# Hitenze/Preconditioned_Additive_Gaussian_Processes_with_Fourier_Acceleration

Hardware: AMD Instinct MI355X
Metric: kernel matvecs/sec + PCG wall-time to 1e-6, n=1e6 d=32 additive, 1/2/4/8 GPU (higher is better)
Workload: dtype f64; 1 GPU; additive NFFT matvec, n=1000000, d=32, 32 x 1-D windows, Gaussian f=1 l=1 mu=0.01 (BASELINE configs[2]); n=1000000, d=32, nwindows=32, parallelism=single

## Files before the change

include/nfft4gp_amd.h:

```cpp
#ifndef NFFT4GP_AMD_H
#define NFFT4GP_AMD_H

#include <stddef.h>

#ifdef __cplusplus
extern "C" {
#endif

#ifndef NFFT4GP_DOUBLE
#define NFFT4GP_DOUBLE double
#endif

#ifndef NFFT4GP_KERNEL_MAX_PARAMS
#define NFFT4GP_KERNEL_MAX_PARAMS 5
#endif

typedef int (*func_kernel)(void *str, NFFT4GP_DOUBLE *data, int n, int ldim, int d, int *permr, int kr,
                           int *permc, int kc, NFFT4GP_DOUBLE **Kp, NFFT4GP_DOUBLE **dKp);
typedef int (*func_solve)(void *precond, int n, NFFT4GP_DOUBLE *x, NFFT4GP_DOUBLE *rhs);
typedef int (*func_symmatvec)(void *matrix, int n, NFFT4GP_DOUBLE alpha, NFFT4GP_DOUBLE *x,
                              NFFT4GP_DOUBLE beta, NFFT4GP_DOUBLE *y);
typedef void (*func_free)(void *str);
typedef int (*func_trace)(void *str, NFFT4GP_DOUBLE **tracesp);
typedef NFFT4GP_DOUBLE (*func_logdet)(void *str);
// ... 158 lines not shown
typedef struct NFFT4GP_PRECOND_NYS_STRUCT
{
   int _k_setup;
   int _own_perm;
   int *_perm;
   int _n;
   int _tits;
   NFFT4GP_DOUBLE _titt;
   NFFT4GP_DOUBLE _tset;
   NFFT4GP_DOUBLE _tlogdet;
   NFFT4GP_DOUBLE _tdvp;
   int _nys_opt;
   int _k;
   NFFT4GP_DOUBLE _eta;
   NFFT4GP_DOUBLE _f2;
   NFFT4GP_DOUBLE *_U;
   NFFT4GP_DOUBLE *_s;
   NFFT4GP_DOUBLE *_work;
   NFFT4GP_DOUBLE *_K;
   NFFT4GP_DOUBLE *_dU;
   NFFT4GP_DOUBLE *_dK;
   pprecond_chol _chol_K11;
   int _dvp_nosolve;
} precond_nys, *pprecond_nys;
int Nfft4GPPrecondNysSolve(void *vnys_mat, int n, NFFT4GP_DOUBLE *x, NFFT4GP_DOUBLE *rhs);
int Nfft4GPAmdPrecondNysMirrorRelease(void *vnys_mat);

void *Nfft4GPAmdPrecondFsaiCreate(void);
void Nfft4GPAmdPrecondFsaiFree(void *str);
void Nfft4GPAmdPrecondFsaiReset(void *str);
void Nfft4GPAmdPrecondFsaiSetLfil(void *str, int lfil);
void Nfft4GPAmdPrecondFsaiSetKernel(void *str, int kernel);
int Nfft4GPAmdPrecondFsaiSetupWithKernel(NFFT4GP_DOUBLE *data, int n, int ldim, int d, func_kernel fkernel,
                                         void *fkernel_params, int require_grad, void *vfsai_mat);
int Nfft4GPAmdPrecondFsaiSetCsr(void *vfsai_mat, int n, const int *ia, const int *ja, const NFFT4GP_DOUBLE *aa,
                                const NFFT4GP_DOUBLE *da);
int Nfft4GPAmdPrecondFsaiCsr(void *vfsai_mat, int *ia, int *ja, NFFT4GP_DOUBLE *aa, NFFT4GP_DOUBLE *da);
int Nfft4GPAmdPrecondFsaiSolve(void *vfsai_mat, int n, NFFT4GP_DOUBLE *x, NFFT4GP_DOUBLE *rhs);
int Nfft4GPAmdPrecondFsaiInvL(void *vfsai_mat, int n, NFFT4GP_DOUBLE *x, NFFT4GP_DOUBLE *rhs);
int Nfft4GPAmdPrecondFsaiInvLT(void *vfsai_mat, int n, NFFT4GP_DOUBLE *x, NFFT4GP_DOUBLE *rhs);
int Nfft4GPAmdPrecondFsaiDvp(void *vfsai_mat, int n, int *mask, NFFT4GP_DOUBLE *x, NFFT4GP_DOUBLE **yp);
int Nfft4GPAmdPrecondFsaiTrace(void *vfsai_mat, NFFT4GP_DOUBLE **tracesp);
NFFT4GP_DOUBLE Nfft4GPAmdPrecondFsaiLogdet(void *vfsai_mat);

void *Nfft4GPAmdFsaiCreate(int n, const int *L_i, const int *L_j, const NFFT4GP_DOUBLE *L_a);
int Nfft4GPAmdFsaiSolve(void *fsai, int n, NFFT4GP_DOUBLE *x, NFFT4GP_DOUBLE *rhs);
void Nfft4GPAmdFsaiFree(void *fsai);

void *Nfft4GPAmdAfnCreate(int n, int k, const int *perm, const NFFT4GP_DOUBLE *L11, const NFFT4GP_DOUBLE *K12,
                          void *fsai_schur);
int Nfft4GPAmdAfnSolve(void *afn, int n, NFFT4GP_DOUBLE *x, NFFT4GP_DOUBLE *rhs);
void Nfft4GPAmdAfnFree(void *afn);
void *Nfft4GPAmdAfnSetup(const NFFT4GP_DOUBLE *data, int n, int ldim, int d, int k, int perm_opt, const int *perm,
                         int schur_lfil, int kernel, void *fkernel_params);
void *Nfft4GPAmdAfnSetupSchur(const NFFT4GP_DOUBLE *data, int n, int ldim, int d, int k, int perm_opt,
                              const int *perm, int schur_opt, int schur_lfil, int kernel, void *fkernel_params);
int Nfft4GPAmdAfnSetOperator(void *afn, void *op);
int Nfft4GPAmdAfnInfo(void *afn, int *k, int *perm, int *ia, int *ja, NFFT4GP_DOUBLE *aa);

int Nfft4GPAmdRankestNysScaled(const NFFT4GP_DOUBLE *data, int n, int ldim, int d, int kernel, void *fkernel_params,
                               int max_rank, int nsample, int nsample_r);
int Nfft4GPAmdRankestDefault(const NFFT4GP_DOUBLE *data, int n, int ldim, int d, int kernel, void *fkernel_params,
                             int max_rank, int nsample, int nsample_r, NFFT4GP_DOUBLE full_tol, int *perm);
int Nfft4GPAmdAfnRankEstimate(const NFFT4GP_DOUBLE *data, int n, int ldim, int d, int max_k, int perm_opt,
                              int nsamples, int kernel, void *fkernel_params, int *perm);
void *Nfft4GPAmdPrecondAFNSetup(const NFFT4GP_DOUBLE *data, int n, int ldim, int d, int max_k, int perm_opt,
                                int schur_opt, int schur_lfil, int nsamples, int kernel, void *fkernel_params,
                                int require_grad);
int Nfft4GPAmdPrecondAFNSolve(void *pre, int n, NFFT4GP_DOUBLE *x, NFFT4GP_DOUBLE *rhs);
int Nfft4GPAmdPrecondAFNInfo(void *pre, int *kind, int *k, void **afn, void **nys);
void Nfft4GPAmdPrecondAFNFree(void *pre);
void *Nfft4GPAmdPrecondAFNCreate(int max_k, int perm_opt, int schur_opt, int schur_lfil, int nsamples);
int Nfft4GPAmdPrecondAFNSetupWithKernel(NFFT4GP_DOUBLE *data, int n, int ldim, int d, func_kernel fkernel,
                                        void *fkernel_params, int require_grad, void *pre);
int Nfft4GPAmdPrecondAFNDvp(void *pre, int n, int *mask, NFFT4GP_DOUBLE *x, NFFT4GP_DOUBLE **yp);
int Nfft4GPAmdPrecondAFNTrace(void *pre, NFFT4GP_DOUBLE **tracesp);
NFFT4GP_DOUBLE Nfft4GPAmdPrecondAFNLogdet(void *pre);
void Nfft4GPAmdPrecondAFNReset(void *pre);

int Nfft4GPAmdSortFps(const NFFT4GP_DOUBLE *data, int n, int ldim, int d, int *k, NFFT4GP_DOUBLE tol, int *perm,
                      NFFT4GP_DOUBLE *dist);

void Nfft4GPAmdSetStream(void *hip_stream);
void *Nfft4GPAmdGetStream(void);
int Nfft4GPAmdDeviceAvailable(void);
const char *Nfft4GPAmdVersion(void);

int Nfft4GPAmdAdditiveLayoutInfo(void *str, long long *out, int nout);

int Nfft4GPAmdTimingEnable(void *str, int enable);
int Nfft4GPAmdSetDeterministic(void *str, int on);
int Nfft4GPAmdSetPrecision(void *str, int bits);
int Nfft4GPAmdTimingQuery(void *str, double *ms, long long *cnt);
int Nfft4GPAmdKernelBench(void *str, int which, int grad, int reps, const NFFT4GP_DOUBLE *x, NFFT4GP_DOUBLE *y,
                          double *ms_avg);

void *Nfft4GPAmdAdditiveShardCreate(NFFT4GP_DOUBLE *data, int n_global, int ldim, int d, int *windows,
                                    int nwindows, int dwindows, int row_begin, int row_end);
int Nfft4GPAmdShardSpread(void *str, const NFFT4GP_DOUBLE *x_local, NFFT4GP_DOUBLE *grid);
int Nfft4GPAmdShardFinish(void *str, const NFFT4GP_DOUBLE *grid, int grad, NFFT4GP_DOUBLE alpha,
                          const NFFT4GP_DOUBLE *x_local, NFFT4GP_DOUBLE beta, NFFT4GP_DOUBLE *y_local);
long long Nfft4GPAmdShardGridSize(void *str);

typedef int (*Nfft4GPAmdAllreduceFn)(void *ctx, NFFT4GP_DOUBLE *d_buf, long long count);
int Nfft4GPAmdCommRcclAvailable(void);
int Nfft4GPAmdCommUniqueId(void *id128);
void *Nfft4GPAmdCommCreateRccl(int rank, int world, const void *id128);
void *Nfft4GPAmdCommCreateCallback(int rank, int world, Nfft4GPAmdAllreduceFn fn, void *ctx,
                                   NFFT4GP_DOUBLE *d_stage, long long capacity);
int Nfft4GPAmdCommAllreduce(void *comm, NFFT4GP_DOUBLE *d_buf, long long count);
void Nfft4GPAmdCommFree(void *comm);
int Nfft4GPAmdCommRanks(void *comm);

int Nfft4GPAmdAdditiveComponentShard(void *str, int nw_global, int own_diag);
void *Nfft4GPAmdDistCreate(void *handle, int kind, void *comm);
void Nfft4GPAmdDistFree(void *dop);
int Nfft4GPAmdDistMatSymv(void *dop, int n, NFFT4GP_DOUBLE alpha, NFFT4GP_DOUBLE *x, NFFT4GP_DOUBLE beta,
                          NFFT4GP_DOUBLE *y);
int Nfft4GPAmdDistCheck(void *dop);
int Nfft4GPAmdDistSetChunks(void *dop, int chunks);
int Nfft4GPAmdDistPeerEnable(void *dop);
int Nfft4GPAmdDistPeerDisable(void *dop);
int Nfft4GPAmdDistPeerActive(void *dop);
int Nfft4GPAmdDistTimingEnable(void *dop, int enable);
int Nfft4GPAmdDistTimingQuery(void *dop, double *ms, long long *cnt);
int Nfft4GPAmdDistGradMatSymv(void *dop, int n, NFFT4GP_DOUBLE alpha, NFFT4GP_DOUBLE *x, NFFT4GP_DOUBLE beta,
                              NFFT4GP_DOUBLE *y);
int Nfft4GPAmdDistGaussianKernel(void *dop, NFFT4GP_DOUBLE *data, int n, int ldim, int d, int *permr, int kr,
                                 int *permc, int kc, NFFT4GP_DOUBLE **Kp, NFFT4GP_DOUBLE **dKp);
int Nfft4GPAmdDistMatern12Kernel(void *dop, NFFT4GP_DOUBLE *data, int n, int ldim, int d, int *permr, int kr,
                                 int *permc, int kc, NFFT4GP_DOUBLE **Kp, NFFT4GP_DOUBLE **dKp);
void *Nfft4GPAmdNysShard(void *nys, int row_begin, int row_end, void *comm);
void *Nfft4GPAmdNysShardSetupAdditive(void *dop, const int *perm, int k, int k11_mode);
int Nfft4GPAmdDistNysSolve(void *dnys, int n, NFFT4GP_DOUBLE *x, NFFT4GP_DOUBLE *rhs);
void Nfft4GPAmdDistNysFree(void *dnys);
int Nfft4GPAmdAfnSetStorage(void *afn, int bits);
int Nfft4GPAmdPrecondAFNSetStorage(void *pre, int bits);
void *Nfft4GPAmdAfnShard(void *afn, int row_begin, int row_end, void *comm);
void *Nfft4GPAmdAfnShardSetup(const NFFT4GP_DOUBLE *data, int n, int ldim, int d, int k, int perm_opt,
                              const int *perm, int schur_opt, int schur_lfil, int kernel, void *fkernel_params,
                              int row_begin, int row_end, void *comm);
int Nfft4GPAmdAfnShardInfo(void *dafn, int *m1, int *m2, long long *k12_doubles, long long *g_nnz);
int Nfft4GPAmdDistAfnSolve(void *dafn, int n, NFFT4GP_DOUBLE *x, NFFT4GP_DOUBLE *rhs);
void Nfft4GPAmdDistAfnFree(void *dafn);

typedef int (*func_matvec)(void *matrix, char trans, int m, int n, NFFT4GP_DOUBLE alpha, NFFT4GP_DOUBLE *x,
                           NFFT4GP_DOUBLE beta, NFFT4GP_DOUBLE *y);
typedef enum
{
   NFFT4GP_OPTIMIZER_UNDEFINED = 0,
   NFFT4GP_OPTIMIZER_ADAM,
   NFFT4GP_OPTIMIZER_NLTGCR
} nfft4gp_optimizer_type;
typedef int (*func_loss)(void *problem, NFFT4GP_DOUBLE *x, NFFT4GP_DOUBLE *lossp, NFFT4GP_DOUBLE *dloss);
typedef int (*func_optimization_step)(void *optimizer);

typedef struct NFFT4GP_OPTIMIZER_ADAM_STRUCT
{
   int _maxits;
   NFFT4GP_DOUBLE _tol;
   func_loss _floss;
   void *_fdata;
   int _n;
   NFFT4GP_DOUBLE _beta1;
   NFFT4GP_DOUBLE _beta2;
   NFFT4GP_DOUBLE _epsilon;
   NFFT4GP_DOUBLE _alpha;
   NFFT4GP_DOUBLE *_m;
   NFFT4GP_DOUBLE *_v;
   NFFT4GP_DOUBLE *_m_hat;
   NFFT4GP_DOUBLE *_v_hat;
   int _nits;
   NFFT4GP_DOUBLE *_loss_history;
   NFFT4GP_DOUBLE *_x_history;
   NFFT4GP_DOUBLE *_grad_history;
   NFFT4GP_DOUBLE *_grad_norm_history;
} optimizer_adam, *poptimizer_adam;

void *Nfft4GPOptimizationAdamCreate(void);
void Nfft4GPOptimizationAdamFree(void *optimizer);
int Nfft4GPOptimizationAdamSetProblem(void *optimizer, func_loss floss, void *fdata, int n);
int Nfft4GPOptimizationAdamSetOptions(void *optimizer, int maxits, NFFT4GP_DOUBLE tol, NFFT4GP_DOUBLE beta1,
                                      NFFT4GP_DOUBLE beta2, NFFT4GP_DOUBLE epsilon, NFFT4GP_DOUBLE alpha);
int Nfft4GPOptimizationAdamInit(void *optimizer, NFFT4GP_DOUBLE *x);
int Nfft4GPOptimizationAdamStep(void *optimizer);

typedef struct NFFT4GP_GP_OPTIMIZER_STRUCT
{
   nfft4gp_optimizer_type _type;
   func_optimization_step _fstep;
   void *_optimizer;
   NFFT4GP_DOUBLE *_dwork;
   NFFT4GP_DOUBLE *_data_train;
   int _data_train_n;
   int _data_train_ldim;
   int _data_train_d;
   NFFT4GP_DOUBLE *_label_train;
   func_kernel _fkernel;
   void *_vfkernel_data;
   func_free _kernel_data_free;
   func_symmatvec _matvec;
   func_symmatvec _dmatvec;
   func_kernel _precond_fkernel;
   void *_precond_vfkernel_data;
   func_free _precond_kernel_data_free;
   precond_kernel_setup _precond_setup;
   func_solve _precond_solve;
   func_trace _precond_trace;
   func_logdet _precond_logdet;
   func_dvp _precond_dvp;
   func_free _precond_reset;
   void *_precond_data;
   int _atol_loss;
   NFFT4GP_DOUBLE _tol_loss;
   int _wsize_loss;
   int _maxits_loss;
   int _nvecs_loss;
   NFFT4GP_DOUBLE *_radamacher_loss;
   nfft4gp_transform_type _transform;
   int *_mask;
   int _print_level_loss;
   NFFT4GP_DOUBLE *_data_predict;
   int _data_predict_n;
   int _data_predict_ldim;
   int _data_predict_d;
   NFFT4GP_DOUBLE *_label_predict;
   func_matvec _matvec_predict;
   int _atol_predict;
   NFFT4GP_DOUBLE _tol_predict;
   int _wsize_predict;
   int _maxits_predict;
   int _print_level_predict;
   int _retuire_std;
} nfft4gp_gp_problem, *pnfft4gp_gp_problem;

void *Nfft4GPGPProblemCreate(void);
void Nfft4GPGPProblemFree(void *gp_problem);
int Nfft4GPGpProblemSetup(void *gp_problem, nfft4gp_optimizer_type type, func_optimization_step fstep, void *optimizer,
                          NFFT4GP_DOUBLE *data_train, int data_train_n, int data_train_ldim, int data_train_d,
                          NFFT4GP_DOUBLE *label_train, func_kernel fkernel, void *vfkernel_data,
                          func_free kernel_data_free, func_symmatvec matvec, func_symmatvec dmatvec,
                          func_kernel precond_fkernel, void *precond_vfkernel_data,
                          func_free precond_kernel_data_free, precond_kernel_setup precond_setup,
                          func_solve precond_solve, func_trace precond_trace, func_logdet precond_logdet,
                          func_dvp precond_dvp, func_free precond_reset, void *precond_data, int atol_loss,
                          NFFT4GP_DOUBLE tol_loss, int wsize_loss, int maxits_loss, int nvecs_loss,
                          NFFT4GP_DOUBLE *radamacher_loss, nfft4gp_transform_type transform, int *mask,
                          int print_level_loss, NFFT4GP_DOUBLE *data_predict, int data_predict_n,
                          int data_predict_ldim, int data_predict_d, NFFT4GP_DOUBLE *label_predict,
                          func_matvec matvec_predict, int atol_predict, NFFT4GP_DOUBLE tol_predict, int wsize_predict,
                          int maxits_predict, int print_level_predict, int retuire_std);
int Nfft4GPGpProblemLoss(void *problem, NFFT4GP_DOUBLE *x, NFFT4GP_DOUBLE *lossp, NFFT4GP_DOUBLE *dloss);

void *Nfft4GPAmdModelCreate(void *additive_handle, const NFFT4GP_DOUBLE *alpha, int n);
int Nfft4GPAmdModelPredict(void *model, const NFFT4GP_DOUBLE *Xnew, int n_new, int ldim, int d, NFFT4GP_DOUBLE *mean,
                           long long *n_outside);
int Nfft4GPAmdModelInfo(void *model, int *nw, int *d, int *kernel, NFFT4GP_DOUBLE *hyper3);
int Nfft4GPAmdModelCoefficients(void *model, NFFT4GP_DOUBLE *H, NFFT4GP_DOUBLE *centre, NFFT4GP_DOUBLE *scale,
                                int *feature);
void *Nfft4GPAmdModelFromCoefficients(int nw, int d, int kernel, const NFFT4GP_DOUBLE *hyper3,
                                      const NFFT4GP_DOUBLE *H, const NFFT4GP_DOUBLE *centre,
                                      const NFFT4GP_DOUBLE *scale, const int *feature);
int Nfft4GPAmdModelFitVariance(void *model, const NFFT4GP_DOUBLE *X, int n, int ldim, int d);
int Nfft4GPAmdModelPredictStd(void *model, const NFFT4GP_DOUBLE *Xnew, int n_new, int ldim, int d,
                              NFFT4GP_DOUBLE *std, int with_noise, long long *n_outside);
int Nfft4GPAmdModelFitTimes(void *model, NFFT4GP_DOUBLE *ms3);
int Nfft4GPAmdModelVarianceInfo(void *model, int *R);
int Nfft4GPAmdModelVariance(void *model, NFFT4GP_DOUBLE *S);
int Nfft4GPAmdModelSetVariance(void *model, const NFFT4GP_DOUBLE *S, int R);
int Nfft4GPAmdModelFeatureWeights(int kernel, NFFT4GP_DOUBLE l, NFFT4GP_DOUBLE scale, int nw, NFFT4GP_DOUBLE *w33);
int Nfft4GPAmdModelFeatureWeightsGrad(int kernel, NFFT4GP_DOUBLE l, NFFT4GP_DOUBLE scale, int nw,
                                      NFFT4GP_DOUBLE *dw33);
void Nfft4GPAmdModelFree(void *model);

void *Nfft4GPAmdFeatureGpCreate(void *additive_handle, const NFFT4GP_DOUBLE *X, int n, int ldim, int d,
                                const NFFT4GP_DOUBLE *y);
int Nfft4GPAmdFeatureGpSetOptions(void *fgp, nfft4gp_transform_type transform, const int *mask);
int Nfft4GPAmdFeatureGpLoss(void *fgp, NFFT4GP_DOUBLE *x, NFFT4GP_DOUBLE *lossp, NFFT4GP_DOUBLE *dloss);
int Nfft4GPAmdFeatureGpSolve(void *fgp, const NFFT4GP_DOUBLE *X, int n, int ldim, int d, const NFFT4GP_DOUBLE *y,
                             NFFT4GP_DOUBLE f, NFFT4GP_DOUBLE l, NFFT4GP_DOUBLE mu, NFFT4GP_DOUBLE *alpha);
int Nfft4GPAmdFeatureGpSolveRhs(void *fgp, const NFFT4GP_DOUBLE *X, int n, int ldim, int d, const NFFT4GP_DOUBLE *r,
                                NFFT4GP_DOUBLE f, NFFT4GP_DOUBLE l, NFFT4GP_DOUBLE mu, NFFT4GP_DOUBLE *alpha);
int Nfft4GPAmdFeatureGpVariance(void *fgp, NFFT4GP_DOUBLE f, NFFT4GP_DOUBLE l, NFFT4GP_DOUBLE mu, NFFT4GP_DOUBLE *S);
int Nfft4GPAmdFeatureGpPredict(void *fgp, NFFT4GP_DOUBLE f, NFFT4GP_DOUBLE l, NFFT4GP_DOUBLE mu,
                               const NFFT4GP_DOUBLE *Xnew, int n_new, int ldim, int d, NFFT4GP_DOUBLE *mean,
                               long long *n_outside);
int Nfft4GPAmdFeatureGpMoments(void *fgp, NFFT4GP_DOUBLE *G, NFFT4GP_DOUBLE *b, NFFT4GP_DOUBLE *yy);
int Nfft4GPAmdFeatureGpInfo(void *fgp, int *n, int *nw, int *R, int *kernel);
int Nfft4GPAmdFeatureGpStatus(void *fgp, int *det_sign, NFFT4GP_DOUBLE *logabsdet);
void Nfft4GPAmdFeatureGpFree(void *fgp);

int Nfft4GPAmdHostTapPoly(NFFT4GP_DOUBLE *C);
int Nfft4GPAmdHostCirculant(int kind, NFFT4GP_DOUBLE c, NFFT4GP_DOUBLE weight, NFFT4GP_DOUBLE *bhat,
                            NFFT4GP_DOUBLE *w);
NFFT4GP_DOUBLE Nfft4GPAmdHostPrepare(const NFFT4GP_DOUBLE *col, int n, unsigned int *q);
int Nfft4GPAmdHostLayout(const unsigned int *qc, int n, int nw, int B, int CG, long long *counts,
                         unsigned short *meta, unsigned int *lo, unsigned int *q, int *tile_off);
int Nfft4GPAmdHostLayoutRec(const unsigned int *qc, int n, int nw, int B, int CG, int rec, long long *counts,
                            unsigned short *meta, unsigned int *lo, unsigned int *q, int *tile_off);
int Nfft4GPAmdDeviceLayout(const unsigned int *qc, int n, int nw, int B, int CG, long long *counts,
                           unsigned short *meta, unsigned int *lo, unsigned int *q, int *tile_off);
int Nfft4GPAmdDeviceLayoutRec(const unsigned int *qc, int n, int nw, int B, int CG, int rec, long long *counts,
                              unsigned short *meta, unsigned int *lo, unsigned int *q, int *tile_off);
int Nfft4GPAmdHostSymEig(const NFFT4GP_DOUBLE *A, int n, NFFT4GP_DOUBLE *w, NFFT4GP_DOUBLE *V);
int Nfft4GPAmdHostCholInverse(const NFFT4GP_DOUBLE *A, int k, NFFT4GP_DOUBLE shift, NFFT4GP_DOUBLE *G);
int Nfft4GPAmdHostLuSolve(const NFFT4GP_DOUBLE *A, int n, NFFT4GP_DOUBLE *B, int nrhs);
int Nfft4GPAmdHostLuLogdet(const NFFT4GP_DOUBLE *A, int n, NFFT4GP_DOUBLE *logabsdet, int *sign);

#ifdef __cplusplus
}
#endif

#endif
```

preconditioned_additive_gaussian_processes_with_fourier_acceleration_amd/csrc/internal.h:

```cpp
#pragma once

#include <hip/hip_runtime.h>

#include <cstdint>
#include <memory>
#include <utility>
#include <string>
#include <vector>

#include "../../include/nfft4gp_amd.h"

namespace nfft4gp_amd {

constexpr int kNos = 64;
constexpr int kBand = 32;
constexpr int kM = 4;
constexpr int kTaps = 2 * kM + 2;
constexpr int kDeg = 7;
constexpr int kNC = kDeg + 1;
constexpr int kR = 16;
constexpr int kWave = 64;
constexpr int kPad = 32;
constexpr int kMaxBlock = 4096 - kPad;

#define NFFT4GP_HIP_CHECK(expr)                                                                    \
   do {                                                                                            \
      hipError_t _e = (expr);                                                                      \
      if (_e != hipSuccess) {                                                                      \
         fprintf(stderr, "nfft4gp_amd: HIP error %s at %s:%d (%s)\n", hipGetErrorString(_e),      \
                 __FILE__, __LINE__, #expr);                                                       \
         return -1;                                                                                \
      }                                                                                            \
   } while (0)

double kb_phi(double t);
double kb_phi_hut(int k);
const std::vector<double>& tap_poly_coeffs();
void bhat_1d(int kind, double c, double* bhat);
void circulant_1d(const double* bhat, double weight, double* w);

__host__ __device__ inline size_t quad_index(long long t, int w, int lane, int nwords)
{
   return (((size_t)t * (size_t)(nwords / 4) + (size_t)(w >> 2)) * kWave + (size_t)lane) * 4 + (size_t)(w & 3);
}

template <class T>
struct DefaultInitAlloc : std::allocator<T> {
   template <class U>
   struct rebind {
      using other = DefaultInitAlloc<U>;
   };
   DefaultInitAlloc() = default;
   template <class U>
   DefaultInitAlloc(const DefaultInitAlloc<U>&) noexcept {}
   template <class U>
   void construct(U* p) noexcept
   {
      ::new ((void*)p) U;
   }
   template <class U, class... A>
   void construct(U* p, A&&... a)
   {
      ::new ((void*)p) U(std::forward<A>(a)...);
   }
};
template <class T>
using RawVec = std::vector<T, DefaultInitAlloc<T>>;

__host__ __device__ inline uint32_t slot_word(uint32_t loc, uint32_t frac)
{
   const uint32_t lo4 = loc & 15u, e = (frac & 0x3FFFFFFu) << 6;
   return ((lo4 >= 8u && e != 0u) ? e - 16u + lo4 : e + lo4) ^ 0x80000000u;
}
__host__ __device__ inline uint32_t lo_byte(uint32_t loc) { return (loc >> 4) & 255u; }
__host__ __device__ inline uint32_t slot_word4(uint32_t loc, uint32_t frac)
{
   const uint32_t e = (frac & 0x3FFFFFFu) << 6, L = loc & 4095u;
   const uint32_t v = (e & ~4095u) | L;
   const int32_t dv = (int32_t)(v - e);
   const uint32_t down = (dv > 2048 && v >= 4096u) ? 4096u : 0u;
   const uint32_t up = (dv < -2048 && v <= 0xFFFFEFFFu) ? 4096u : 0u;
   return (v - down + up) ^ 0x80000000u;
}

struct Layout {
   int n = 0;
   int nw = 0;
   int B = kMaxBlock;
   int CG = 8;
   int rec = 5;
   int ngroups = 0;
   int nblocks = 0;
   long long ntiles = 0;
   RawVec<uint16_t> meta;
   RawVec<uint32_t> lo;
   RawVec<uint32_t> q;
   std::vector<int> tile_off;
   std::vector<int> cmax;
};
void build_layout(const uint32_t* qc, int n, int nw, int B, int CG, Layout& L, int rec = 5);
struct AdditivePlan;
int build_layout_dev(const uint32_t* d_qc, int n, int nw, int B, int CG, AdditivePlan& P, hipStream_t s, int rec = 5);

struct DevLayout {
   uint16_t* meta = nullptr;
   uint32_t* lo = nullptr;
   uint32_t* q = nullptr;
   int* tile_off = nullptr;
   int* cmax = nullptr;
   long long ntiles = 0;
   size_t bytes = 0;
};

constexpr int kMdMaxDim = 5;
constexpr int kMdTiledMaxDim = 3;
struct MdComp {
   int d = 0;
   int hicount = 1;
   long long u_off = 0;
};
struct MdPlan {
   bool on = false;
   bool gfix_per_window = false;
   int maxd = 1;
   long long G = 0;
   long long Cmax = 0;
   long long M = 0;
   std::vector<MdComp> comps;
   MdComp* d_comps = nullptr;
   int* d_u = nullptr;
   double* d_psi = nullptr;
   double* d_grid = nullptr;
   double2* d_F[2] = {nullptr, nullptr};
   double2* d_Mo[2] = {nullptr, nullptr};
   double2* d_B[4] = {nullptr, nullptr, nullptr, nullptr};
   double* d_h[2] = {nullptr, nullptr};
   double* d_bh = nullptr;
   double* d_bhd = nullptr;
   double* d_dot_part = nullptr;
   unsigned int* d_dot_ticket = nullptr;
   int* d_perm = nullptr;
   int4* d_items = nullptr;
   int nitems = 0;
   bool lines = false;
   double* d_part = nullptr;
   unsigned long long* d_gfix = nullptr;
   unsigned long long* d_xmax = nullptr;
   double psi_max = 0.0;
};

struct AdditivePlan {
   int n_global = 0, row_begin = 0, row_end = 0, n = 0;
   int nw = 0, dw = 0, skip_last = 0;
   std::vector<int> comp_dims;
   int d = 0;
   std::vector<int> comp_feature;
   bool points_ready = false;
   std::vector<double> comp_scale;
   std::vector<double> comp_centre;
   std::vector<double> comp_sigma;
   int kernel = 0;
   double f = 1.0, l = 1.0, mu = 0.0;
   double weight = 1.0;
   double diag = 1.0;
   int B = kMaxBlock, CG = 3, ngroups = 0, nblocks = 0;
   int rec = 5;
   int spread_variant = -1;
   int spread_fold = 1;
   bool det = false;
   double* d_hb = nullptr;
   int nparts = 0;
   DevLayout dl;
   double* d_part = nullptr;
   double* d_w = nullptr;
   double* d_wd = nullptr;
   double* d_H = nullptr;
   double* d_Hd = nullptr;
   double* d_C = nullptr;
   double* d_dot_part = nullptr;
   unsigned int* d_dot_ticket = nullptr;
   double* d_part2 = nullptr;
   double* d_gsum = nullptr;
   int fused_grid = -1;
   bool cells33 = false;
   double* d_hsum = nullptr;
   int hsum_par = 0;
   double* d_H2 = nullptr;
   double* d_xs = nullptr;
   double* d_ys = nullptr;
   MdPlan md;
   bool timing = false;
   hipEvent_t* kev = nullptr;
   double ms[3] = {0, 0, 0};
   long long cnt[3] = {0, 0, 0};
};

int upload_tap_coeffs();
int launch_spread(const AdditivePlan& P, const double* d_x, double* d_part, hipStream_t stream);
int launch_grid(const AdditivePlan& P, const double* d_part, int nparts, int grad, hipStream_t stream);
int launch_spread_grid(AdditivePlan& P, const double* d_x, int grad, hipStream_t stream);
int launch_grid_from_sum(const AdditivePlan& P, const double* d_gridsum, int grad, hipStream_t stream);
constexpr int kPeerInline = 8;
struct PeerArgs {
   char* const* bufs = nullptr;
   char* inl[kPeerInline] = {};
   char* own = nullptr;
   int world = 0;
   unsigned int epoch = 0;
   unsigned int* err = nullptr;
   long long slot_doubles = 0;
   long long spin = 0;
};
int launch_reduce_parts(const AdditivePlan& P, const double* d_part, double* d_gridsum, hipStream_t stream,
                        const PeerArgs* A = nullptr);
int launch_shard_finish_split(const AdditivePlan& P, const double* d_gridsum, double alpha, const double* d_x,
                              double beta, double* d_y, int S, hipStream_t stream, const PeerArgs* A = nullptr,
                              const double* d_part = nullptr);
int launch_peer_grid(const AdditivePlan& P, const PeerArgs& A, const double* d_part, hipStream_t stream);
int launch_peer_sum(const AdditivePlan& P, const PeerArgs& A, double* d_grid, hipStream_t stream);
int launch_interp(const AdditivePlan& P, int grad, double alpha, const double* d_x, double beta, double* d_y,
                  hipStream_t stream, double* d_dot = nullptr);
int launch_interp_blocks(const AdditivePlan& P, double alpha, const double* d_x, double beta, double* d_y, int b0,
                         int b1, hipStream_t stream);
int launch_matvec2(AdditivePlan& P, double alpha, const double* x0, const double* x1, double beta, double* y0,
                   double* y1, hipStream_t stream);
int pick_spread_variant(const AdditivePlan& P);
bool grid_atomic(const AdditivePlan& P);
int pick_interp_threads(const AdditivePlan& P);
bool pick_interp_hl(const AdditivePlan& P);
int pick_hl_slots(const AdditivePlan& P);
int pick_interp2_threads();
bool pick_fused_grid(const AdditivePlan& P);
int launch_matvec_fused(AdditivePlan& P, double alpha, const double* d_x, double beta, double* d_y, hipStream_t stream,
                        double* d_dot = nullptr);
int additive_matvec_multi(void* str, int nv, double alpha, const double* const* X, double beta, double* const* Y);
int additive_matvec_dot(void* str, const double* d_x, double* d_y, double* d_dot);
AdditivePlan* additive_plan_of(void* str);
bool additive_fused_dot_ok(void* str);

struct NysDev {
   int n = 0, k = 0;
   double eta = 0.0;
   double* U = nullptr;
   float* Uf = nullptr;
   double* s = nullptr;
   double* w = nullptr;
   double* part = nullptr;
   int nblk = 0;
   double setup_ms[4] = {0.0, 0.0, 0.0, 0.0};
   std::vector<double> hs;
   bool grad = false;
   double f2 = 0.0;
   double *Kall = nullptr, *dU = nullptr, *G = nullptr, *Gt = nullptr, *GdKG = nullptr, *D = nullptr;
   double *vk = nullptr, *vn = nullptr;
};
void nys_free(NysDev* N);
constexpr int kNysRows = 2048;
int nys_alloc_scratch(NysDev* N);
int gemm_f64(bool transA, int M, int N, int K, const double* A, long long lda, const double* B, long long ldb,
             double* C, long long ldc, hipStream_t s);
int sym_eig_host(const std::vector<double>& A, int n, std::vector<double>& w, std::vector<double>& V);
int chol_inverse_host(std::vector<double>& A, int k);
int lu_solve_host(std::vector<double>& A, int n, std::vector<double>& B, int nrhs, double* logabsdet = nullptr,
                  int* sign = nullptr, std::vector<int>* piv_out = nullptr);
void lu_subst_host(const std::vector<double>& A, int n, const std::vector<int>& piv, std::vector<double>& B, int nrhs);
int lu_solve_dev(double* A, int n, double* B, int nrhs, hipStream_t s, double* logabsdet = nullptr,
                 int* sign = nullptr, int* piv_keep = nullptr);
int lu_resolve_dev(const double* A, int n, const int* piv, double* B, int nrhs, hipStream_t s);
struct Comm;
struct NysShard {
   Comm* comm = nullptr;
   int row_begin = 0, n_global = 0;
};
NysDev* nys_setup_additive(const double* xw_host, int n, int nw, int dw, int skip_last, int kernel, double f,
                           double l, double mu, const int* perm, int k, int k11_mode, bool with_grad = false,
                           const NysShard* shard = nullptr);

int md_build_points(AdditivePlan& P, const std::vector<std::vector<double>>& xs);
int md_setup(AdditivePlan& P);
int md_spread(const AdditivePlan& P, const double* d_x, double* d_grid, hipStream_t s);
int md_grid(const AdditivePlan& P, const double* d_grid, int grad, hipStream_t s);
int md_interp(const AdditivePlan& P, int grad, double alpha, const double* d_x, double beta, double* d_y,
              hipStream_t s, double* d_dot = nullptr);
void md_free(AdditivePlan& P);
void bhat_nd(int kind, int d, double c, std::vector<double>& bhat);

int chol_inverse_dev(double* A, int k, double shift, double* G, double* Gt, int* d_info, hipStream_t s);
int gram_tn(int M, int N, int K, const double* A, long long lda, const double* B, long long ldb, double* C, int sym,
            hipStream_t s);
int sym_eigvals_dev(double* A, int n, std::vector<double>& w, hipStream_t s);
struct KernelSpec {
   int kernel = 0;
   double f = 1.0, l = 1.0, mu = 0.0;
   const double* Xk = nullptr;
   long long ldk = 0;
   int nw = 1, dw = 0, last_dw = 0;
};
int fsai_kernel_csr(const double* dX, int n, int ldim, int d, int lfil, const KernelSpec& K, const double* dW, int kw,
                    int require_grad, std::vector<int>& ia, std::vector<int>& ja, std::vector<double>& aa,
                    std::vector<double>& da, hipStream_t s, const double* dGB = nullptr,
                    const double* dGC = nullptr, void** keep = nullptr);
void* fsai_create_from_device(int n, int* dia, int* dja, double* daa, const std::vector<int>& hia, hipStream_t s);
long long count_nonfinite(const double* d, size_t count, hipStream_t s);
int fsai_pattern_rows(const double* dX, int n, int ldim, int d, int lfil, const std::vector<int>& rows,
                      std::vector<int>& hia, std::vector<int>& hja, hipStream_t s);
int fsai_values_rows(const KernelSpec& Ks, const double* dX, long long ldim, int d, int lfil, const int* dia,
                     const int* dja, int nrows, const double* dW, int kw, const int* dwcol, double* daa, hipStream_t s);
void* afn_shard_from_parts(int n_local, int k, int n2, Comm* comm, const std::vector<int>& lm_idx,
                           const std::vector<int>& lm_row, const std::vector<int>& nl_pos,
                           const std::vector<int>& nl_row, double* d_Linv, double* d_LinvT, double* d_K12, bool fsai,
                           double schur_scale, const std::vector<int>& gia, const std::vector<int>& gja,
                           const std::vector<double>& gaa);
void* fsai_grad_create(int n, const int* ia, const int* ja, const double* aa, const double* da);
void fsai_grad_free(void* F);
int fsai_grad_op(void* F, int op, int g, const double* x, double* y, hipStream_t s);
double fsai_grad_diag(void* F, int g, hipStream_t s);
int chol_factor_dev(double* A, int k, int* d_info, hipStream_t s);
int kernel_spec_of(void* fkernel_params, func_kernel fkernel, int kernel, int n, KernelSpec& K, double** owned);
struct AfnGrad {
   int n = 0, k = 0, n2 = 0;
   int* perm = nullptr;
   double *L = nullptr, *Linv = nullptr, *LinvT = nullptr;
   double* dL = nullptr;
   const double* K12 = nullptr;
   double* dK12 = nullptr;
   void* S = nullptr;
   void* afn = nullptr;
   double trace[3] = {0.0, 0.0, 0.0};
   double logdet = 0.0;
   double* work = nullptr;
};
void afn_grad_free(AfnGrad* G);
int afn_grad_dvp(AfnGrad* G, const int* mask, const double* x, double* y, hipStream_t s);

void* afn_create_device(int n, int k, int* d_perm, double* d_Linv, double* d_LinvT, double* d_K12, void* S,
                        double schur_scale = 0.0);

hipStream_t current_stream();
bool is_device_ptr(const void* p);
int device_ok();

constexpr int kMvFeat = 33, kMvPad = 36, kMvMaxNw = 128;
constexpr double kMpLimit = 0.25 + 1.0 / 8589934592.0;
inline int mv_order(int nw) { return kMvPad * ((nw + 3) / 4 * 4); }

__device__ inline bool mv_angle(double x, double ctr, double sc, double& c1, double& s1)
{
   const double xs = (x - ctr) * sc;
   const bool in = fabs(xs) <= kMpLimit;
   const double xq = in ? xs : 0.0;
   const uint32_t q = (uint32_t)(unsigned long long)llround(xq * 4294967296.0);
   sincospi((double)(int)q * (1.0 / 2147483648.0), &s1, &c1);
   return in;
}

__device__ inline void mv_rotate(double& ck, double& sk, double c1, double s1)
{
   const double c = ck * c1 - sk * s1;
   sk = sk * c1 + ck * s1;
   ck = c;
}

struct WindowMap {
   int nw = 0, d = 0;
   const double* centre = nullptr;
   const double* scale = nullptr;
   const int* feature = nullptr;
};
void feature_weights(int kernel, double l, double scale, int nw, double* w33);
void feature_weights_grad(int kernel, double l, double scale, int nw, double* dw33);
int window_count_outside(const WindowMap& W, const double* dX, long long ld, int n, hipStream_t s, long long* outside);
int window_moments(const WindowMap& W, const double* dX, long long ld, int n, const double* dy, double* G, double* b,
                   double* yy, double* ms2, hipStream_t s);

struct RandScope {
   RandScope();
   ~RandScope();
};
struct CallerRandBatch {
   char* prev = nullptr;
   CallerRandBatch();
   ~CallerRandBatch();
};

struct Comm {
   int rank = 0, world = 1;
   virtual ~Comm() {}
   virtual int allreduce(double* d_buf, size_t count, hipStream_t s) = 0;
   virtual int ranks() { return world; }
};
int additive_rows(void* str, int* n_local, int* n_global, int* row_begin);
int dist_failed(void* dop);
bool shard_fused_dot_ok(void* str);
int shard_finish_dot(void* str, const double* grid, const double* x_local, double* y_local, double* d_dot);
bool shard_peer_ok(void* str);
int shard_spread_peer(void* str, const double* x_local, const PeerArgs& A);
int shard_peer_sum(void* str, const PeerArgs& A, double* d_grid);
int shard_finish_dot_peer(void* str, const PeerArgs& A, double* d_grid, const double* x_local, double* y_local,
                          double* d_dot);
int shard_finish_peer(void* str, const PeerArgs& A, double* d_grid, int grad, double alpha, const double* x_local,
                      double beta, double* y_local);
struct DistPcgInfo {
   Comm* dot_comm = nullptr;
   int n_global = 0;
   int row_begin = 0;
   bool fused_dot = false;
};
int dist_pcg_info(void* dop, DistPcgInfo& info);
NysDev* nys_setup_shard(void* str, const int* perm, int k, int k11_mode, Comm* comm);
int additive_matvec_chunked(void* str, double alpha, const double* d_x, double* d_y, int nchunks,
                            int (*done)(void* ctx, size_t r0, size_t r1), void* ctx);
int dist_matvec_dot(void* dop, const double* d_p, double* d_q, double* d_dot);

}
```

preconditioned_additive_gaussian_processes_with_fourier_acceleration_amd/csrc/layout_gpu.hip:

```cpp
#include <hip/hip_runtime.h>

#include <algorithm>
#include <cstdio>
#include <vector>

#include "callbacks.hpp"
#include "internal.h"

namespace nfft4gp_amd {

namespace {

constexpr int kLT = 256;
constexpr int kLWaves = kLT / 64;

__global__ __launch_bounds__(kLT) void k_lay_count(const uint32_t* __restrict__ qc, int n, int nw, int B, int CG,
                                                   int ngroups, int* __restrict__ tiles, int* __restrict__ cmax)
{
   __shared__ int hist[kNos];
   __shared__ int nch, mx;
   const int bg = blockIdx.x, b = bg / ngroups, g = bg % ngroups;
   const int base = b * B, nloc = min(B, n - base);
   const int c0 = g * CG, c1 = min(nw, c0 + CG);
   const int tid = threadIdx.x;
   if (tid == 0) nch = mx = 0;
   for (int c = c0; c < c1; c++) {
      const uint32_t* qq = qc + (size_t)c * n + base;
      if (tid < kNos) hist[tid] = 0;
      __syncthreads();
      for (int j = tid; j < nloc; j += kLT) atomicAdd(&hist[qq[j] >> 26], 1);
      __syncthreads();
      if (tid < 64) {
         int v = (hist[tid] + kR - 1) / kR, m = hist[tid];
         for (int off = 32; off > 0; off >>= 1) {
            v += __shfl_xor(v, off, 64);
            m = max(m, __shfl_xor(m, off, 64));
         }
         if (tid == 0) {
            nch += v;
            mx = max(mx, m);
         }
      }
      __syncthreads();
   }
   if (tid == 0) {
      tiles[bg] = (nch + kWave - 1) / kWave;
      cmax[bg] = mx;
   }
}

struct EmitLds {
   size_t off, run, cbase, sorted, sloc, sfr, smeta, cnt, total;
   __host__ __device__ EmitLds(int CG, int B, int Tmax)
   {
      size_t p = 0;
      auto take = [&](size_t bytes) {
         const size_t at = p;
         p += (bytes + 15) & ~(size_t)15;
         return at;
      };
      off = take(sizeof(int) * CG * (kNos + 1));
      run = take(sizeof(int) * CG * kNos);
      cbase = take(sizeof(int) * (CG * kNos + 1));
      const size_t sorted_bytes = sizeof(uint16_t) * CG * B, cnt_bytes = sizeof(int) * Tmax * (2 * 32 + 4 * 16);
      sorted = take(sorted_bytes > cnt_bytes ? sorted_bytes : cnt_bytes);
      cnt = sorted;
      sloc = take(sizeof(uint16_t) * Tmax * kWave * kR);
      sfr = take(sizeof(uint32_t) * Tmax * kWave * kR);
      smeta = take(sizeof(uint16_t) * Tmax * kWave);
      total = p;
   }
};

template <int REC>
__global__ __launch_bounds__(kLT) void k_lay_emit(const uint32_t* __restrict__ qc, int n, int nw, int B, int CG,
                                                  int ngroups, int Tmax, const int* __restrict__ tile_off,
                                                  uint16_t* __restrict__ meta, uint32_t* __restrict__ lo,
                                                  uint32_t* __restrict__ q)
{
   extern __shared__ __attribute__((aligned(16))) unsigned char lds[];
   const EmitLds E(CG, B, Tmax);
   int* s_off = reinterpret_cast<int*>(lds + E.off);
   int* s_run = reinterpret_cast<int*>(lds + E.run);
   int* s_cbase = reinterpret_cast<int*>(lds + E.cbase);
   uint16_t* s_sorted = reinterpret_cast<uint16_t*>(lds + E.sorted);
   uint16_t* s_loc = reinterpret_cast<uint16_t*>(lds + E.sloc);
   uint32_t* s_fr = reinterpret_cast<uint32_t*>(lds + E.sfr);
   uint16_t* s_meta = reinterpret_cast<uint16_t*>(lds + E.smeta);
   int* s_cnt = reinterpret_cast<int*>(lds + E.cnt);

   const int bg = blockIdx.x, b = bg / ngroups, g = bg % ngroups;
   const int base = b * B, nloc = min(B, n - base);
   const int c0 = g * CG, c1 = min(nw, c0 + CG), ncomp = c1 - c0;
   const int t0 = tile_off[bg], T = tile_off[bg + 1] - t0;
   const int tid = threadIdx.x, lane = tid & 63, wave = tid >> 6;

   for (int ci0 = 0; ci0 < ncomp; ci0 += kLWaves) {
      const int ci = ci0 + wave;
      const bool act = ci < ncomp;
      const uint32_t* qq = qc + (size_t)(c0 + (act ? ci : 0)) * n + base;
      int* off = s_off + (act ? ci : 0) * (kNos + 1);
      int* run = s_run + (act ? ci : 0) * kNos;
      uint16_t* sorted = s_sorted + (size_t)(act ? ci : 0) * B;
      if (act) run[lane] = 0;
      __syncthreads();
      if (act)
         for (int j = lane; j < nloc; j += 64) atomicAdd(&run[qq[j] >> 26], 1);
      __syncthreads();
      if (act) {
         const int v = run[lane];
         int incl = v;
         for (int d = 1; d < 64; d <<= 1) {
            const int t = __shfl_up(incl, d, 64);
            if (lane >= d) incl += t;
         }
         off[lane] = incl - v;
         if (lane == 63) off[kNos] = incl;
         run[lane] = incl - v;
      }
      __syncthreads();
      for (int jb = 0; jb < nloc; jb += 64) {
         const int j = jb + lane;
         const bool valid = act && j < nloc;
         const int cell = valid ? (int)(qq[j] >> 26) : 0;
         unsigned long long peers = __ballot(valid);
#pragma unroll
         for (int bit = 0; bit < 6; bit++) {
            const unsigned long long set = __ballot(valid && ((cell >> bit) & 1));
            peers &= ((cell >> bit) & 1) ? set : ~set;
         }
         const int rank = __popcll(peers & ((1ull << lane) - 1ull));
         const int start = valid ? run[cell] : 0;
         __syncthreads();
         if (valid) {
            sorted[start + rank] = (uint16_t)j;
            if (lane == 63 - __clzll(peers)) run[cell] = start + __popcll(peers);
         }
         __syncthreads();
      }
   }
   if (tid == 0) {
      int acc = 0;
      for (int i = 0; i < ncomp * kNos; i++) {
         s_cbase[i] = acc;
         const int* off = s_off + (i / kNos) * (kNos + 1);
         const int cnt = off[i % kNos + 1] - off[i % kNos];
         acc += (cnt + kR - 1) / kR;
      }
      s_cbase[ncomp * kNos] = acc;
   }
   for (int i = tid; i < T * kWave * kR; i += kLT) {
      s_loc[i] = (uint16_t)(B + ((i / kR) % kWave & 31));
      s_fr[i] = 0u;
   }
   for (int i = tid; i < T * kWave; i += kLT) s_meta[i] = (uint16_t)(c0 << 6);
   __syncthreads();
   const int nchunks = s_cbase[ncomp * kNos];
   for (int k = tid; k < nchunks; k += kLT) {
      int lo_i = 0, hi_i = ncomp * kNos;
      while (hi_i - lo_i > 1) {
         const int mid = (lo_i + hi_i) >> 1;
         if (s_cbase[mid] <= k) lo_i = mid;
         else hi_i = mid;
      }
      const int ci = lo_i / kNos, cell = lo_i % kNos;
      const int* off = s_off + ci * (kNos + 1);
      const int s = off[cell] + (k - s_cbase[lo_i]) * kR;
      const int tile = k % T, ln = k / T;
      s_meta[tile * kWave + ln] = (uint16_t)(((c0 + ci) << 6) | cell);
      const uint32_t* qq = qc + (size_t)(c0 + ci) * n + base;
      const uint16_t* sorted = s_sorted + (size_t)ci * B;
      for (int r = 0; r < kR; r++) {
         const int sidx = s + r;
         if (sidx < off[cell + 1]) {
            const int loc = sorted[sidx];
            s_loc[(tile * kWave + ln) * kR + r] = (uint16_t)loc;
            s_fr[(tile * kWave + ln) * kR + r] = qq[loc] & 0x3FFFFFFu;
         }
      }
   }
   __syncthreads();
   if (tid < T) {
      uint16_t* L = s_loc + (size_t)tid * kWave * kR;
      uint32_t* F = s_fr + (size_t)tid * kWave * kR;
      int* c32 = s_cnt + tid * 128;
      int* c16 = c32 + 64;
      for (int r = 0; r < kR; r++) {
         for (int i = 0; i < 128; i++) c32[i] = 0;
         for (int ln = 0; ln < kWave; ln++) {
            int best = r, best_cost = 1 << 30;
            for (int k = r; k < kR; k++) {
               const int v = L[ln * kR + k];
               const int cost = 2 * c32[(ln >> 5) * 32 + (v & 31)] + c16[(ln >> 4) * 16 + (v & 15)];
               if (cost < best_cost) {
                  best_cost = cost;
                  best = k;
                  if (cost == 0) break;
               }
            }
            const uint16_t tl = L[ln * kR + r];
            L[ln * kR + r] = L[ln * kR + best];
            L[ln * kR + best] = tl;
            const uint32_t tf = F[ln * kR + r];
            F[ln * kR + r] = F[ln * kR + best];
            F[ln * kR + best] = tf;
            const int v = L[ln * kR + r];
            c32[(ln >> 5) * 32 + (v & 31)]++;
            c16[(ln >> 4) * 16 + (v & 15)]++;
         }
      }
   }
   __syncthreads();
   for (int i = tid; i < T * kWave; i += kLT) meta[(size_t)(t0 + i / kWave) * kWave + i % kWave] = s_meta[i];
   for (int i = tid; i < T * kWave * kR; i += kLT) {
      const int tile = i / (kWave * kR), ln = (i / kR) % kWave, r = i % kR;
      const uint32_t loc = s_loc[i];
      q[quad_index(t0 + tile, r, ln, kR)] = REC == 5 ? slot_word(loc, s_fr[i]) : slot_word4(loc, s_fr[i]);
   }
   if (REC != 5) return;
   for (int i = tid; i < T * kWave * (kR / 4); i += kLT) {
      const int tile = i / (kWave * (kR / 4)), ln = (i / (kR / 4)) % kWave, r4 = i % (kR / 4);
      const uint16_t* l4 = s_loc + ((size_t)tile * kWave + ln) * kR + 4 * r4;
      lo[quad_index(t0 + tile, r4, ln, kR / 4)] =
          lo_byte(l4[0]) | (lo_byte(l4[1]) << 8) | (lo_byte(l4[2]) << 16) | (lo_byte(l4[3]) << 24);
   }
}

}

int build_layout_dev(const uint32_t* d_qc, int n, int nw, int B, int CG, AdditivePlan& P, hipStream_t s, int rec)
{
   const int ngroups = (nw + CG - 1) / CG, nblocks = (n + B - 1) / B, nbg = ngroups * nblocks;
   const int Tmax_bound = (CG * (B / kR + kNos) + kWave - 1) / kWave + 1;
   if (EmitLds(CG, B, (CG * ((B + kR - 1) / kR) + kWave - 1) / kWave).total > 160 * 1024) return -1;
   int* d_tiles = nullptr;
   int* d_cmax = nullptr;
   NFFT4GP_HIP_CHECK(hipMalloc((void**)&d_tiles, sizeof(int) * (nbg + 1)));
   NFFT4GP_HIP_CHECK(hipMalloc((void**)&d_cmax, sizeof(int) * std::max(1, nbg)));
   hipLaunchKernelGGL(k_lay_count, dim3(std::max(1, nbg)), dim3(kLT), 0, s, d_qc, n, nw, B, CG, ngroups, d_tiles,
                      d_cmax);
   NFFT4GP_HIP_CHECK(hipGetLastError());
   std::vector<int> tiles(nbg);
   NFFT4GP_HIP_CHECK(hipMemcpyAsync(tiles.data(), d_tiles, sizeof(int) * nbg, hipMemcpyDeviceToHost, s));
   NFFT4GP_HIP_CHECK(hipStreamSynchronize(s));
   std::vector<int> toff(nbg + 1, 0);
   long long acc = 0;
   int Tmax = 1;
   for (int i = 0; i < nbg; i++) {
      toff[i] = (int)acc;
      acc += tiles[i];
      Tmax = std::max(Tmax, tiles[i]);
   }
   toff[nbg] = (int)acc;
   if (Tmax > Tmax_bound || EmitLds(CG, B, Tmax).total > 160 * 1024) {
      (void)hipFree(d_tiles);
      (void)hipFree(d_cmax);
      return -1;
   }
   P.ngroups = ngroups;
   P.nblocks = nblocks;
   P.dl = DevLayout();
   P.dl.cmax = d_cmax;
   NFFT4GP_HIP_CHECK(hipMalloc((void**)&P.dl.tile_off, sizeof(int) * (nbg + 1)));
   NFFT4GP_HIP_CHECK(hipMemcpyAsync(P.dl.tile_off, toff.data(), sizeof(int) * (nbg + 1), hipMemcpyHostToDevice, s));
   const size_t nt = (size_t)std::max<long long>(acc, 1);
   NFFT4GP_HIP_CHECK(hipMalloc((void**)&P.dl.meta, sizeof(uint16_t) * nt * kWave));
   if (rec == 5) NFFT4GP_HIP_CHECK(hipMalloc((void**)&P.dl.lo, sizeof(uint32_t) * nt * (kR / 4) * kWave));
   NFFT4GP_HIP_CHECK(hipMalloc((void**)&P.dl.q, sizeof(uint32_t) * nt * kR * kWave));
   const size_t lds = EmitLds(CG, B, Tmax).total;
   static const bool attr = []() {
      (void)hipFuncSetAttribute((const void*)k_lay_emit<5>, hipFuncAttributeMaxDynamicSharedMemorySize, 160 * 1024);
      (void)hipFuncSetAttribute((const void*)k_lay_emit<4>, hipFuncAttributeMaxDynamicSharedMemorySize, 160 * 1024);
      (void)hipGetLastError();
      return true;
   }();
   (void)attr;
   if (nbg > 0)
      hipLaunchKernelGGL(rec == 5 ? k_lay_emit<5> : k_lay_emit<4>, dim3(nbg), dim3(kLT), lds, s, d_qc, n, nw, B, CG,
                         ngroups, Tmax, P.dl.tile_off, P.dl.meta, P.dl.lo, P.dl.q);
   NFFT4GP_HIP_CHECK(hipGetLastError());
   NFFT4GP_HIP_CHECK(hipStreamSynchronize(s));
   (void)hipFree(d_tiles);
   P.dl.ntiles = acc;
   P.dl.bytes = (size_t)acc * kWave * (2 + (rec == 5 ? 4 * (kR / 4) : 0) + 4 * kR) + sizeof(int) * (nbg + 1);
   return 0;
}

}

extern "C" int Nfft4GPAmdDeviceLayoutRec(const unsigned int* qc, int n, int nw, int B, int CG, int rec,
                                         long long* counts, unsigned short* meta, unsigned int* lo, unsigned int* q,
                                         int* tile_off);
extern "C" int Nfft4GPAmdDeviceLayout(const unsigned int* qc, int n, int nw, int B, int CG, long long* counts,
                                      unsigned short* meta, unsigned int* lo, unsigned int* q, int* tile_off)
{
   return Nfft4GPAmdDeviceLayoutRec(qc, n, nw, B, CG, 5, counts, meta, lo, q, tile_off);
}

extern "C" int Nfft4GPAmdDeviceLayoutRec(const unsigned int* qc, int n, int nw, int B, int CG, int rec,
                                         long long* counts, unsigned short* meta, unsigned int* lo, unsigned int* q,
                                         int* tile_off)
{
   using namespace nfft4gp_amd;
   if (B <= 0 || B > kMaxBlock || CG <= 0 || n < 0 || nw <= 0 || nw > 1023 || !counts || (rec != 4 && rec != 5))
      return -1;
   if (!need_device("Nfft4GPAmdDeviceLayout")) return -1;
   hipStream_t s = current_stream();
   uint32_t* d_qc = nullptr;
   NFFT4GP_HIP_CHECK(hipMalloc((void**)&d_qc, sizeof(uint32_t) * std::max<size_t>(1, (size_t)n * nw)));
   NFFT4GP_HIP_CHECK(hipMemcpy(d_qc, qc, sizeof(uint32_t) * (size_t)n * nw, hipMemcpyHostToDevice));
   AdditivePlan P;
   const int rc = build_layout_dev(d_qc, n, nw, B, CG, P, s, rec);
   (void)hipFree(d_qc);
   if (rc) return -1;
   const int nbg = P.ngroups * P.nblocks;
   counts[0] = P.dl.ntiles;
   counts[1] = P.ngroups;
   counts[2] = P.nblocks;
   const size_t nt = (size_t)P.dl.ntiles;
   int err = 0;
   if (meta && hipMemcpy(meta, P.dl.meta, sizeof(uint16_t) * nt * kWave, hipMemcpyDeviceToHost) != hipSuccess) err = 1;
   if (lo && rec == 5 &&
       hipMemcpy(lo, P.dl.lo, sizeof(uint32_t) * nt * (kR / 4) * kWave, hipMemcpyDeviceToHost) != hipSuccess)
      err = 1;
   if (q && hipMemcpy(q, P.dl.q, sizeof(uint32_t) * nt * kR * kWave, hipMemcpyDeviceToHost) != hipSuccess) err = 1;
   if (tile_off && hipMemcpy(tile_off, P.dl.tile_off, sizeof(int) * (nbg + 1), hipMemcpyDeviceToHost) != hipSuccess)
      err = 1;
   for (void* p : {(void*)P.dl.meta, (void*)P.dl.lo, (void*)P.dl.q, (void*)P.dl.tile_off, (void*)P.dl.cmax})
      (void)hipFree(p);
   return err ? -1 : 0;
}
```

preconditioned_additive_gaussian_processes_with_fourier_acceleration_amd/csrc/nfft_api.cpp:

```cpp
#include <dlfcn.h>
#include <hip/hip_runtime.h>

#include <array>
#include <algorithm>
#include <atomic>
#include <chrono>
#include <thread>
#include <cmath>
#include <cstdio>
#include <cstdlib>
#include <cstring>
#include <mutex>
#include <vector>

#include "internal.h"
#include "reduce.hpp"

using namespace nfft4gp_amd;

namespace nfft4gp_amd {

namespace {
std::recursive_mutex g_rand_mu;
int g_rand_depth = 0;
char* g_caller_rand = nullptr;
char g_private_rand[256];
bool g_private_ready = false;
}

RandScope::RandScope()
{
   g_rand_mu.lock();
   if (g_rand_depth++ == 0) {
      if (!g_private_ready) {
         g_caller_rand = initstate(20240807u, g_private_rand, sizeof(g_private_rand));
         g_private_ready = true;
      } else {
         g_caller_rand = setstate(g_private_rand);
      }
   }
}

RandScope::~RandScope()
{
   if (--g_rand_depth == 0) {
      setstate(g_caller_rand);
      g_caller_rand = nullptr;
   }
   g_rand_mu.unlock();
}

CallerRandBatch::CallerRandBatch()
{
   if (g_rand_depth > 0) prev = setstate(g_caller_rand);
}

CallerRandBatch::~CallerRandBatch()
{
   if (prev) g_caller_rand = setstate(prev);
}

static hipStream_t g_stream = nullptr;

hipStream_t current_stream() { return g_stream; }

int device_ok()
{
   static int ok = 0;
   if (!ok) {
      int cnt = 0;
      const hipError_t e = hipGetDeviceCount(&cnt);
      if (e != hipSuccess) {
         fprintf(stderr, "nfft4gp_amd: hipGetDeviceCount failed: %s\n", hipGetErrorString(e));
         cnt = 0;
      }
      (void)hipGetLastError();
      ok = cnt > 0 ? 1 : 0;
   }
   return ok;
}

bool is_device_ptr(const void* p)
{
   if (!p) return false;
   hipPointerAttribute_t attr;
   hipError_t e = hipPointerGetAttributes(&attr, p);
   if (e != hipSuccess) {
      (void)hipGetLastError();
      return false;
   }
   return attr.type == hipMemoryTypeDevice || attr.type == hipMemoryTypeManaged;
}

}

namespace {

struct TimingRec {
   std::array<hipEvent_t, 6> ev;
   bool grid = true;
};

struct PlanExt {
   AdditivePlan P;
   std::vector<TimingRec> pending;
   std::vector<TimingRec> pool;
};

struct SingleAdj {
   str_adj pub{};
   double sigma_pub = 0.0;
   nfft4gp_kernel* owner = nullptr;
   int dim = 1;
   int max_n = 0;
   std::vector<double> data;
   PlanExt* plan = nullptr;
};

void dfree(void* p)
{
   if (p) (void)hipFree(p);
}

void free_layout(AdditivePlan& P)
{
   dfree(P.dl.meta);
   dfree(P.dl.lo);
   dfree(P.dl.q);
   dfree(P.dl.tile_off);
   dfree(P.dl.cmax);
   P.dl = DevLayout();
   dfree(P.d_part);
   dfree(P.d_part2);
   dfree(P.d_H2);
   dfree(P.d_dot_part);
   dfree(P.d_dot_ticket);
   P.d_part2 = P.d_H2 = nullptr;
   P.d_part = nullptr;
   P.d_dot_part = nullptr;
   P.d_dot_ticket = nullptr;
}

void free_plan(PlanExt* E)
{
   if (!E) return;
   AdditivePlan& P = E->P;
   free_layout(P);
   md_free(P);
   dfree(P.d_w);
   dfree(P.d_wd);
   dfree(P.d_H);
   dfree(P.d_Hd);
   dfree(P.d_hb);
   dfree(P.d_gsum);
   dfree(P.d_hsum);
   dfree(P.d_C);
   dfree(P.d_xs);
   dfree(P.d_ys);
   for (auto& r : E->pending)
      for (auto e : r.ev) (void)hipEventDestroy(e);
   for (auto& r : E->pool)
      for (auto e : r.ev) (void)hipEventDestroy(e);
   delete E;
}

template <class T, class A>
int upload(T** dptr, const std::vector<T, A>& h)
{
   if (*dptr) {
      (void)hipFree(*dptr);
      *dptr = nullptr;
   }
   if (h.empty()) return 0;
   NFFT4GP_HIP_CHECK(hipMalloc((void**)dptr, sizeof(T) * h.size()));
   NFFT4GP_HIP_CHECK(hipMemcpy(*dptr, h.data(), sizeof(T) * h.size(), hipMemcpyHostToDevice));
   return 0;
}

double centre_and_scale(const double* col, int n_global, int d, std::vector<double>& xs, double* centre = nullptr)
{
   xs.assign(col, col + (size_t)n_global * d);
   for (int i = 0; i < d; i++) {
      double c = 0.0;
      for (int j = 0; j < n_global; j++) c += xs[(size_t)i * n_global + j];
      c /= (double)n_global;
      if (centre) centre[i] = c;
      for (int j = 0; j < n_global; j++) xs[(size_t)i * n_global + j] -= c;
   }
   double radius = 0.0;
   for (int j = 0; j < n_global; j++) {
      double r = 0.0;
      for (int i = 0; i < d; i++) r += xs[(size_t)i * n_global + j] * xs[(size_t)i * n_global + j];
      r = std::sqrt(r);
      if (r > radius) radius = r;
   }
   double scale;
   if (radius == 0.0) return -1.0;
   if (radius > 0.25 || radius < 0.125) {
      scale = 0.25 / radius;
      for (auto& v : xs) v *= scale;
   } else {
      scale = 1.0;
   }
   return scale;
}

uint32_t quantize(double x)
{
   const long long v = std::llround(x * 4294967296.0);
   return (uint32_t)(unsigned long long)v;
}

int plan_build_points(AdditivePlan& P, const double* buffer)
{
   const int ng = P.n_global;
   RawVec<uint32_t> qc((size_t)P.nw * P.n);
   P.comp_scale.assign(P.nw, 1.0);
   P.comp_centre.assign(P.nw, 0.0);
   std::vector<double> xs;
   if (std::any_of(P.comp_dims.begin(), P.comp_dims.end(), [](int d) { return d != 1; })) {
      std::vector<std::vector<double>> xsc(P.nw);
      for (int c = 0; c < P.nw; c++) {
         const double* col = buffer + (size_t)c * ng * P.dw;
         P.comp_scale[c] = centre_and_scale(col, ng, P.comp_dims[c], xsc[c]);
         if (P.comp_scale[c] < 0.0) {
            fprintf(stderr, "nfft4gp_amd: all points of window %d coincide (radius 0); the reference's scaling "
                            "0.25/radius (nfft_interface.c:190) is undefined there.\n", c);
            return -1;
         }
      }
      if (md_build_points(P, xsc)) return -1;
      P.points_ready = true;
      return 0;
   }
   const auto t0 = std::chrono::steady_clock::now();
   std::atomic<int> next{0};
   std::atomic<int> outside33{0};
   auto work = [&]() {
      std::vector<double> xw;
      for (int c = next++; c < P.nw; c = next++) {
         const double* col = buffer + (size_t)c * ng * P.dw;
         P.comp_scale[c] = centre_and_scale(col, ng, 1, xw, &P.comp_centre[c]);
         if (P.comp_scale[c] < 0.0) continue;
         uint32_t cimax = 0;
         for (int j = 0; j < P.n; j++) {
            const uint32_t q = quantize(xw[(size_t)P.row_begin + j]);
            qc[(size_t)c * P.n + j] = q;
            cimax = std::max(cimax, (q + 0x40000000u) >> 26);
         }
         if (cimax > 32u) outside33 = 1;
      }
   };
   {
      const int nt = std::max(1, std::min({16, P.nw, (int)std::thread::hardware_concurrency()}));
      std::vector<std::thread> th;
      for (int t = 1; t < nt; t++) th.emplace_back(work);
      work();
      for (auto& t : th) t.join();
   }
   for (int c = 0; c < P.nw; c++)
      if (P.comp_scale[c] < 0.0) {
         fprintf(stderr,
                 "nfft4gp_amd: all points of window %d coincide (radius 0); the reference's scaling "
                 "0.25/radius (nfft_interface.c:190) is undefined there.\n", c);
         return -1;
      }
   P.cells33 = outside33 == 0;
   const auto t1 = std::chrono::steady_clock::now();
   free_layout(P);
   hipStream_t s = current_stream();
   uint32_t* d_qc = nullptr;
   NFFT4GP_HIP_CHECK(hipMalloc((void**)&d_qc, sizeof(uint32_t) * std::max<size_t>(1, qc.size())));
   NFFT4GP_HIP_CHECK(hipMemcpyAsync(d_qc, qc.data(), sizeof(uint32_t) * qc.size(), hipMemcpyHostToDevice, s));
   const auto t2 = std::chrono::steady_clock::now();
   const int rc_dev = build_layout_dev(d_qc, P.n, P.nw, P.B, P.CG, P, s, P.rec);
   (void)hipStreamSynchronize(s);
   (void)hipFree(d_qc);
   if (rc_dev) {
      Layout L;
      build_layout(qc.data(), P.n, P.nw, P.B, P.CG, L, P.rec);
      P.ngroups = L.ngroups;
      P.nblocks = L.nblocks;
      free_layout(P);
      if (upload(&P.dl.meta, L.meta) || upload(&P.dl.lo, L.lo) || upload(&P.dl.q, L.q) ||
          upload(&P.dl.tile_off, L.tile_off) || upload(&P.dl.cmax, L.cmax))
         return -1;
      P.dl.ntiles = L.ntiles;
      P.dl.bytes = L.meta.size() * 2 + L.lo.size() * 4 + L.q.size() * 4 + L.tile_off.size() * 4;
   }
   if (getenv("NFFT4GP_AMD_VERBOSE")) {
      const auto t3 = std::chrono::steady_clock::now();
      auto ms = [](auto a, auto b) { return std::chrono::duration<double, std::milli>(b - a).count(); };
      fprintf(stderr, "nfft4gp_amd: layout setup: centre/scale/quantize %.1f ms, coordinate upload %.1f ms, "
                      "layout (%s) %.1f ms\n", ms(t0, t1), ms(t1, t2), rc_dev ? "host" : "GPU", ms(t2, t3));
   }
   P.nparts = P.nblocks;
   NFFT4GP_HIP_CHECK(hipMalloc((void**)&P.d_part, sizeof(double) * (size_t)std::max(1, P.nparts) * P.nw * kNos));

   dfree(P.d_dot_part);
   NFFT4GP_HIP_CHECK(hipMalloc((void**)&P.d_dot_part, sizeof(double) * (size_t)std::max(1, P.nblocks)));
   if (!P.d_dot_ticket) {
      NFFT4GP_HIP_CHECK(hipMalloc((void**)&P.d_dot_ticket, sizeof(unsigned int) * kTicketWords));
      NFFT4GP_HIP_CHECK(hipMemset(P.d_dot_ticket, 0, sizeof(unsigned int) * kTicketWords));
   }

   if (!P.d_H) NFFT4GP_HIP_CHECK(hipMalloc((void**)&P.d_H, sizeof(double) * (size_t)P.nw * kNos * kNC));
   if (!P.d_Hd) NFFT4GP_HIP_CHECK(hipMalloc((void**)&P.d_Hd, sizeof(double) * (size_t)P.nw * kNos * kNC));
   if (!P.d_hb) NFFT4GP_HIP_CHECK(hipMalloc((void**)&P.d_hb, sizeof(double) * 4 * (size_t)std::max(1, P.nw)));
   if (upload_tap_coeffs()) return -1;
   P.points_ready = true;
   return 0;
}

int plan_setup(AdditivePlan& P, const double* buffer, int kernel, double f, double l, double mu)
{
   if (!device_ok()) {
      fprintf(stderr, "nfft4gp_amd: no HIP device visible; the operator has no CPU fallback.\n");
      return -1;
   }
   if (!P.points_ready && plan_build_points(P, buffer)) return -1;
   P.kernel = kernel;
   P.f = f;
   P.l = l;
   P.mu = mu;
   P.comp_sigma.assign(P.nw, 0.0);
   if (P.md.on) {
      for (int c = 0; c < P.nw; c++)
         P.comp_sigma[c] = (kernel == 0) ? l * P.comp_scale[c] * std::sqrt(2.0) : l * P.comp_scale[c];
      return md_setup(P);
   }
   std::vector<double> w((size_t)P.nw * kNos), wd((size_t)P.nw * kNos);
   double bh[kBand], bhd[kBand];
   for (int c = 0; c < P.nw; c++) {
      const double sc = P.comp_scale[c];
      const double sig = (kernel == 0) ? l * sc * std::sqrt(2.0) : l * sc;
      P.comp_sigma[c] = sig;
      bhat_1d(kernel == 0 ? 0 : 2, sig, bh);
      bhat_1d(kernel == 0 ? 1 : 3, sig, bhd);
      const double dscale = (kernel == 0) ? 2.0 * sc * std::sqrt(2.0) / sig : sc / sig;
      circulant_1d(bh, P.weight, w.data() + (size_t)c * kNos);
      circulant_1d(bhd, P.weight * dscale, wd.data() + (size_t)c * kNos);
   }
   if (upload(&P.d_w, w) || upload(&P.d_wd, wd)) return -1;
   return 0;
}

TimingRec get_rec(PlanExt* E)
{
   if (!E->pool.empty()) {
      TimingRec r = E->pool.back();
      E->pool.pop_back();
      return r;
   }
   TimingRec r;
   for (auto& e : r.ev) (void)hipEventCreate(&e);
   return r;
}

bool use_fused(const AdditivePlan& P, hipStream_t s)
{
   if (!pick_fused_grid(P)) return false;
   hipStreamCaptureStatus st = hipStreamCaptureStatusNone;
   if (hipStreamIsCapturing(s, &st) != hipSuccess) {
      (void)hipGetLastError();
      return false;
   }
   return st == hipStreamCaptureStatusNone;
}

int plan_apply_dev(PlanExt* E, int grad, double alpha, const double* d_x, double beta, double* d_y)
{
   AdditivePlan& P = E->P;
   hipStream_t s = current_stream();
   TimingRec rec;
   if (P.timing) {
      rec = get_rec(E);
      if (!P.md.on) P.kev = rec.ev.data();
   }
   const bool mdt = P.timing && P.md.on;
   int rc = 0;
   if (mdt) (void)hipEventRecord(rec.ev[0], s);
   const bool fused = !grad && use_fused(P, s);
   rec.grid = !fused;
   if (P.md.on) {
      rc = md_spread(P, d_x, P.md.d_grid, s);
      if (mdt) {
         (void)hipEventRecord(rec.ev[1], s);
         (void)hipEventRecord(rec.ev[2], s);
      }
      if (!rc) rc = md_grid(P, P.md.d_grid, grad, s);
   } else if (fused) {
      rc = launch_matvec_fused(P, alpha, d_x, beta, d_y, s);
   } else {
      rc = launch_spread_grid(P, d_x, grad, s);
   }
   if (mdt) {
      (void)hipEventRecord(rec.ev[3], s);
      (void)hipEventRecord(rec.ev[4], s);
   }
   if (!rc && !fused)
      rc = P.md.on ? md_interp(P, grad, alpha, d_x, beta, d_y, s) : launch_interp(P, grad, alpha, d_x, beta, d_y, s);
   if (mdt) (void)hipEventRecord(rec.ev[5], s);
   P.kev = nullptr;
   if (P.timing) {
      if (rc)
         E->pool.push_back(rec);
      else
         E->pending.push_back(rec);
   }
   return rc ? -1 : 0;
}

int plan_apply(PlanExt* E, int n, int grad, double alpha, const double* x, double beta, double* y)
{
   AdditivePlan& P = E->P;
   if (!P.points_ready) {
      fprintf(stderr, "nfft4gp_amd: matvec called before the kernel setup (func_kernel) call.\n");
      return -1;
   }
   if (n != P.n) {
      fprintf(stderr, "nfft4gp_amd: matvec size %d does not match the handle (%d).\n", n, P.n);
      return -1;
   }
   if (P.row_begin != 0 || P.row_end != P.n_global) {
      fprintf(stderr, "nfft4gp_amd: rows [%d, %d) of %d form a row shard; use Nfft4GPAmdShardSpread/ShardFinish.\n",
              P.row_begin, P.row_end, P.n_global);
      return -1;
   }
   const size_t ny = (size_t)n * (grad ? 3 : 1);
   const bool dx = is_device_ptr(x), dy = is_device_ptr(y);
   if (dx && dy) return plan_apply_dev(E, grad, alpha, x, beta, y);
   hipStream_t s = current_stream();
   if (!P.d_xs) NFFT4GP_HIP_CHECK(hipMalloc((void**)&P.d_xs, sizeof(double) * (size_t)n));
   if (!P.d_ys) NFFT4GP_HIP_CHECK(hipMalloc((void**)&P.d_ys, sizeof(double) * (size_t)n * 3));
   const double* xd = x;
   double* yd = y;
   if (!dx) {
      NFFT4GP_HIP_CHECK(hipMemcpyAsync(P.d_xs, x, sizeof(double) * n, hipMemcpyHostToDevice, s));
      xd = P.d_xs;
   }
   if (!dy) {
      yd = P.d_ys;
      if (beta != 0.0) NFFT4GP_HIP_CHECK(hipMemcpyAsync(yd, y, sizeof(double) * ny, hipMemcpyHostToDevice, s));
   }
   if (plan_apply_dev(E, grad, alpha, xd, beta, yd)) return -1;
   if (!dy) NFFT4GP_HIP_CHECK(hipMemcpyAsync(y, yd, sizeof(double) * ny, hipMemcpyDeviceToHost, s));
   NFFT4GP_HIP_CHECK(hipStreamSynchronize(s));
   return 0;
}

PlanExt* additive_plan(void* str)
{
   if (!str) return nullptr;
   return (PlanExt*)((nfft4gp_kernel*)str)->_external;
}


int omp_threads_in_process()
{
   using fn_t = int (*)();
   static fn_t f = (fn_t)dlsym(RTLD_DEFAULT, "omp_get_max_threads");
   return f ? std::max(1, f()) : 1;
}

nfft4gp_kernel* kernel_struct_create(int max_n, int omp = 0)
{
   nfft4gp_kernel* k = (nfft4gp_kernel*)calloc(1, sizeof(nfft4gp_kernel));
   k->_max_n = max_n;
   k->_omp = omp;
   k->_ldwork = (size_t)max_n * (size_t)(omp ? omp_threads_in_process() : 1);
   k->_dwork = (double*)malloc(sizeof(double) * std::max<size_t>(1, k->_ldwork));
   return k;
}

int setup_common(void* str, int kernel, int n, int ldim, double** Kp, double** dKp)
{
   if (Kp == NULL || dKp == NULL) {
      printf("Error: NFFT kernel requires Kp and dKp to be not NULL.\n");
      return -1;
   }
   nfft4gp_kernel* kd = (nfft4gp_kernel*)str;
   PlanExt* E = additive_plan(str);
   if (!E) return -1;
   (void)n;
   (void)ldim;
   if (plan_setup(E->P, kd->_buffer, kernel, kd->_params[0], kd->_params[1], kd->_noise_level)) return -1;
   *Kp = (double*)str;
   *dKp = (double*)str;
   return 0;
}

int default_block(int n)
{
   if (n >= 200 * kMaxBlock) return kMaxBlock;
   if (n >= 40 * 2032) return 2032;
   return 1024;
}

void env_layout(AdditivePlan& P)
{
   P.B = default_block(P.n);
   {
      const int nw = std::max(P.nw, 1), nblocks = std::max(1, (P.n + P.B - 1) / P.B);
      auto pick = [&](int cgmax) {
         const int ngroups = (nw + cgmax - 1) / cgmax;
         P.CG = (nw + ngroups - 1) / ngroups;
         return ngroups;
      };
      if ((long long)pick(4) * nblocks < 384) pick(3);
   }
   if (const char* e = getenv("NFFT4GP_AMD_BLOCK")) {
      const int v = atoi(e);
      if (v >= 256) P.B = std::min(v, kMaxBlock) & ~15;
   }
   if (const char* e = getenv("NFFT4GP_AMD_CG")) {
      const int v = atoi(e);
      if (v >= 1 && v <= 64) P.CG = v;
   }
   if (const char* e = getenv("NFFT4GP_AMD_SPREAD_VARIANT")) P.spread_variant = atoi(e);
   if (const char* e = getenv("NFFT4GP_AMD_SPREAD_FOLD")) P.spread_fold = atoi(e) != 0;
   if (const char* e = getenv("NFFT4GP_AMD_DET")) P.det = atoi(e) != 0;
   if (const char* e = getenv("NFFT4GP_AMD_PRECISION")) P.rec = atoi(e) == 32 ? 4 : 5;
   if (const char* e = getenv("NFFT4GP_AMD_FUSED_GRID")) P.fused_grid = atoi(e) != 0;
}

void* additive_create(double* data, int n_global, int ldim, int d, int* windows, int nwindows, int dwindows, int rb,
                      int re)
{
   nfft4gp_kernel* kd = kernel_struct_create(3 * n_global);
   kd->_iparams[0] = nwindows;
   kd->_iparams[1] = dwindows;
   int skip_window = 1;
   kd->_iparams[2] = 0;
   while (skip_window < dwindows && windows[nwindows * dwindows - skip_window] < 0) {
      skip_window++;
      kd->_iparams[2]++;
   }
   kd->_ibufferp = (int**)malloc(sizeof(int*));
   kd->_ibufferp[0] = windows;
   kd->_buffer = (double*)malloc(sizeof(double) * (size_t)n_global * nwindows * dwindows);
   kd->_own_buffer = 1;
   PlanExt* E = new PlanExt();
   AdditivePlan& P = E->P;
   P.n_global = n_global;
   P.row_begin = rb;
   P.row_end = re;
   P.n = re - rb;
   P.nw = nwindows;
   P.dw = dwindows;
   P.d = d;
   P.skip_last = kd->_iparams[2];
   P.weight = 1.0 / (double)nwindows;
   env_layout(P);
   double* dst = kd->_buffer;
   const int* fw = windows;
   for (int i = 0; i < nwindows; i++) {
      int actual = 0;
      for (int j = 0; j < dwindows; j++) {
         if (fw[0] >= 0) {
            memcpy(dst, data + (size_t)fw[0] * ldim, sizeof(double) * n_global);
            if (actual == 0) P.comp_feature.push_back(fw[0]);
            fw++;
            dst += n_global;
            actual++;
         }
      }
      if (actual == 0) P.comp_feature.push_back(-1);
      P.comp_dims.push_back(actual);
   }
   kd->_external = E;
   return kd;
}

}

namespace nfft4gp_amd {
bool additive_fused_dot_ok(void* str)
{
   PlanExt* E = additive_plan(str);
   if (!E || !E->P.points_ready) return false;
   const AdditivePlan& P = E->P;
   if (P.row_begin != 0 || P.row_end != P.n_global) return false;
   return P.md.on || P.nblocks <= kRedMaxBlocks;
}

int additive_matvec_dot(void* str, const double* d_x, double* d_y, double* d_dot)
{
   PlanExt* E = additive_plan(str);
   if (!E || !E->P.points_ready) return -1;
   AdditivePlan& P = E->P;
   hipStream_t s = current_stream();
   if (P.md.on) {
      if (md_spread(P, d_x, P.md.d_grid, s) || md_grid(P, P.md.d_grid, 0, s)) return -1;
      return md_interp(P, 0, 1.0, d_x, 0.0, d_y, s, d_dot);
   }
   if (use_fused(P, s)) return launch_matvec_fused(P, 1.0, d_x, 0.0, d_y, s, d_dot);
   if (launch_spread_grid(P, d_x, 0, s)) return -1;
   return launch_interp(P, 0, 1.0, d_x, 0.0, d_y, s, d_dot);
}
}

namespace nfft4gp_amd {
int additive_matvec_multi(void* str, int nv, double alpha, const double* const* X, double beta, double* const* Y)
{
   PlanExt* E = additive_plan(str);
   if (!E || !E->P.points_ready) return -1;
   AdditivePlan& P = E->P;
   if (P.row_begin != 0 || P.row_end != P.n_global) return -1;
   hipStream_t s = current_stream();
   int v = 0;
   if (!P.md.on && !P.timing)
      for (; v + 1 < nv; v += 2)
         if (launch_matvec2(P, alpha, X[v], X[v + 1], beta, Y[v], Y[v + 1], s)) return -1;
   for (; v < nv; v++)
      if (plan_apply_dev(E, 0, alpha, X[v], beta, Y[v])) return -1;
   return 0;
}

int additive_matvec_chunked(void* str, double alpha, const double* d_x, double* d_y, int nchunks,
                            int (*done)(void* ctx, size_t r0, size_t r1), void* ctx)
{
   PlanExt* E = additive_plan(str);
   if (!E || !E->P.points_ready) return -1;
   AdditivePlan& P = E->P;
   if (P.md.on || P.timing || P.row_begin != 0 || P.row_end != P.n_global || P.nblocks == 0) return -1;
   hipStream_t s = current_stream();
   if (launch_spread_grid(P, d_x, 0, s)) return -1;
   nchunks = std::max(1, std::min(nchunks, P.nblocks));
   for (int c = 0; c < nchunks; c++) {
      const int b0 = (int)((long long)P.nblocks * c / nchunks), b1 = (int)((long long)P.nblocks * (c + 1) / nchunks);
      if (launch_interp_blocks(P, alpha, d_x, 0.0, d_y, b0, b1, s)) return -1;
      if (done(ctx, (size_t)b0 * P.B, std::min((size_t)b1 * P.B, (size_t)P.n))) return -1;
   }
   return 0;
}

AdditivePlan* additive_plan_of(void* str)
{
   PlanExt* E = additive_plan(str);
   return E ? &E->P : nullptr;
}

int additive_rows(void* str, int* n_local, int* n_global, int* row_begin)
{
   PlanExt* E = additive_plan(str);
   if (!E) return -1;
   *n_local = E->P.n;
   *n_global = E->P.n_global;
   if (row_begin) *row_begin = E->P.row_begin;
   return 0;
}

static int shard_split(const AdditivePlan& P)
{
   int S = (P.nblocks <= 64 && !P.det) ? 4 : 1;
   if (const char* e = getenv("NFFT4GP_AMD_SHARD_SPLIT")) S = std::max(1, std::min(16, atoi(e)));
   return std::min(S, std::max(1, P.ngroups));
}

bool shard_fused_dot_ok(void* str)
{
   PlanExt* E = additive_plan(str);
   if (!E || !E->P.points_ready) return false;
   return E->P.md.on || E->P.nblocks <= kRedMaxBlocks;
}

bool shard_peer_ok(void* str)
{
   PlanExt* E = additive_plan(str);
   return E && E->P.points_ready && !E->P.md.on;
}

int shard_spread_peer(void* str, const double* x_local, const PeerArgs& A)
{
   (void)A;
   PlanExt* E = additive_plan(str);
   if (!E || !E->P.points_ready || E->P.md.on) return -1;
   AdditivePlan& P = E->P;
   hipStream_t s = current_stream();
   return (P.nblocks > 0 && launch_spread(P, x_local, P.d_part, s)) ? -1 : 0;
}

int shard_peer_sum(void* str, const PeerArgs& A, double* d_grid)
{
   PlanExt* E = additive_plan(str);
   if (!E || !E->P.points_ready || E->P.md.on) return -1;
   hipStream_t s = current_stream();
   if (launch_reduce_parts(E->P, E->P.d_part, nullptr, s, &A)) return -1;
   return launch_peer_sum(E->P, A, d_grid, s);
}

int shard_finish_peer(void* str, const PeerArgs& A, double* d_grid, int grad, double alpha, const double* x_local,
                      double beta, double* y_local)
{
   PlanExt* E = additive_plan(str);
   if (!E || !E->P.points_ready || E->P.md.on) return -1;
   AdditivePlan& P = E->P;
   hipStream_t s = current_stream();
   const int S = shard_split(P);
   if (!grad && S > 1 && !P.timing)
      return launch_shard_finish_split(P, nullptr, alpha, x_local, beta, y_local, S, s, &A, P.d_part);
   if (!grad && !P.timing && !P.det)
      return (launch_peer_grid(P, A, P.d_part, s) || launch_interp(P, 0, alpha, x_local, beta, y_local, s)) ? -1 : 0;
   if (shard_peer_sum(str, A, d_grid) || launch_grid_from_sum(P, d_grid, grad, s)) return -1;
   return launch_interp(P, grad, alpha, x_local, beta, y_local, s);
}

int shard_finish_dot(void* str, const double* grid, const double* x_local, double* y_local, double* d_dot)
{
   PlanExt* E = additive_plan(str);
   if (!E || !E->P.points_ready) return -1;
   AdditivePlan& P = E->P;
   hipStream_t s = current_stream();
   if (P.n == 0) {
      NFFT4GP_HIP_CHECK(hipMemsetAsync(d_dot, 0, sizeof(double), s));
      return 0;
   }
   if (P.md.on) {
      if (md_grid(P, grid, 0, s)) return -1;
      return md_interp(P, 0, 1.0, x_local, 0.0, y_local, s, d_dot);
   }
   if (launch_grid_from_sum(P, grid, 0, s)) return -1;
   return launch_interp(P, 0, 1.0, x_local, 0.0, y_local, s, d_dot);
}

int shard_finish_dot_peer(void* str, const PeerArgs& A, double* d_grid, const double* x_local, double* y_local,
                          double* d_dot)
{
   PlanExt* E = additive_plan(str);
   if (!E || !E->P.points_ready || E->P.md.on) return -1;
   AdditivePlan& P = E->P;
   hipStream_t s = current_stream();
   if (P.n > 0 && !P.det && !P.timing)
      return (launch_peer_grid(P, A, P.d_part, s) || launch_interp(P, 0, 1.0, x_local, 0.0, y_local, s, d_dot)) ? -1
                                                                                                            : 0;
   if (shard_peer_sum(str, A, d_grid)) return -1;
   return shard_finish_dot(str, d_grid, x_local, y_local, d_dot);
}
}

namespace nfft4gp_amd {
int additive_buffer_info(void* str, const double** xw, int* n, int* nw, int* dw, int* skip_last, int* kernel)
{
   nfft4gp_kernel* kd = (nfft4gp_kernel*)str;
   PlanExt* E = additive_plan(str);
   if (!kd || !E || !kd->_buffer) return -1;
   const AdditivePlan& P = E->P;
   if (P.row_begin != 0 || P.row_end != P.n_global) return -1;
   *xw = kd->_buffer;
   *n = P.n_global;
   *nw = kd->_iparams[0];
   *dw = kd->_iparams[1];
   *skip_last = kd->_iparams[2];
   *kernel = P.points_ready ? P.kernel : -1;
   return 0;
}
}

extern "C" {

static const char* kVersion = "nfft4gp_amd 0.1.0 (gfx950)";

const char* Nfft4GPAmdVersion(void) { return kVersion; }
int Nfft4GPAmdDeviceAvailable(void) { return device_ok(); }
void Nfft4GPAmdSetStream(void* s) { g_stream = (hipStream_t)s; }
void* Nfft4GPAmdGetStream(void) { return (void*)g_stream; }

void* Nfft4GPKernelParamCreate(int max_n, int omp) { return kernel_struct_create(max_n, omp); }

void Nfft4GPKernelParamFree(void* str)
{
   nfft4gp_kernel* k = (nfft4gp_kernel*)str;
   if (!k) return;
   free(k->_dwork);
   if (k->_own_buffer) free(k->_buffer);
   if (k->_own_dbuffer) free(k->_dbuffer);
   free(k->_ibufferp);
   if (k->_own_fkernel_buffer_params) Nfft4GPKernelParamFree(k->_fkernel_buffer_params);
   free(k);
}

void* Nfft4GPNFFTAdditiveKernelParamCreate(double* data, int n, int ldim, int d, int* windows, int nwindows,
                                           int dwindows)
{
   RandScope rand_scope;
   return additive_create(data, n, ldim, d, windows, nwindows, dwindows, 0, n);
}

void* Nfft4GPAmdAdditiveShardCreate(double* data, int n_global, int ldim, int d, int* windows, int nwindows,
                                    int dwindows, int row_begin, int row_end)
{
   if (row_begin < 0 || row_end > n_global || row_begin > row_end) {
      fprintf(stderr, "nfft4gp_amd: invalid shard rows [%d, %d) of %d\n", row_begin, row_end, n_global);
      return NULL;
   }
   return additive_create(data, n_global, ldim, d, windows, nwindows, dwindows, row_begin, row_end);
}

int Nfft4GPNFFTAdditiveKernelGaussianKernel(void* str, double* data, int n, int ldim, int d, int* permr, int kr,
                                            int* permc, int kc, double** Kp, double** dKp)
{
   (void)data, (void)d, (void)permr, (void)kr, (void)permc, (void)kc;
   RandScope rand_scope;
   return setup_common(str, 0, n, ldim, Kp, dKp);
}

int Nfft4GPNFFTAdditiveKernelMatern12Kernel(void* str, double* data, int n, int ldim, int d, int* permr, int kr,
                                            int* permc, int kc, double** Kp, double** dKp)
{
   (void)data, (void)d, (void)permr, (void)kr, (void)permc, (void)kc;
   RandScope rand_scope;
   return setup_common(str, 1, n, ldim, Kp, dKp);
}

int Nfft4GPAdditiveNFFTMatSymv(void* data, int n, double alpha, double* x, double beta, double* y)
{
   PlanExt* E = additive_plan(data);
   if (!E) return -1;
   return plan_apply(E, n, 0, alpha, x, beta, y);
}

int Nfft4GPAmdAdditiveMatSymvMulti(void* data, int n, int nrhs, double alpha, const double* X, long long ldx,
                                   double beta, double* Y, long long ldy)
{
   PlanExt* E = additive_plan(data);
   if (!E || !E->P.points_ready || n != E->P.n || nrhs < 0 || ldx < n || ldy < n) {
      fprintf(stderr, "nfft4gp_amd: Nfft4GPAmdAdditiveMatSymvMulti: handle not set up, or n / ld mismatch\n");
      return -1;
   }
   if (nrhs == 0) return 0;
   if (!is_device_ptr(X) || !is_device_ptr(Y)) {
      fprintf(stderr, "nfft4gp_amd: Nfft4GPAmdAdditiveMatSymvMulti takes device arrays\n");
      return -1;
   }
   std::vector<const double*> xs(nrhs);
   std::vector<double*> ys(nrhs);
   for (int v = 0; v < nrhs; v++) {
      xs[v] = X + (size_t)v * ldx;
      ys[v] = Y + (size_t)v * ldy;
   }
   return additive_matvec_multi(data, nrhs, alpha, xs.data(), beta, ys.data());
}

int Nfft4GPAdditiveNFFTGradMatSymv(void* data, int n, double alpha, double* x, double beta, double* y)
{
   PlanExt* E = additive_plan(data);
   if (!E) return -1;
   return plan_apply(E, n, 1, alpha, x, beta, y);
}

void Nfft4GPAdditiveNFFTKernelFree(void* str)
{
   if (!str) return;
   free_plan(additive_plan(str));
   ((nfft4gp_kernel*)str)->_external = NULL;
   Nfft4GPKernelParamFree(str);
}

double* Nfft4GPNFFTAppendData(double* X1, int n1, int ldim1, int d, double* X2, int n2, int ldim2)
{
   double* X = (double*)malloc(sizeof(double) * (size_t)(n1 + n2) * d);
   for (int i = 0; i < d; i++) {
      memcpy(X + (size_t)i * (n1 + n2), X1 + (size_t)i * ldim1, sizeof(double) * n1);
      memcpy(X + (size_t)i * (n1 + n2) + n1, X2 + (size_t)i * ldim2, sizeof(double) * n2);
   }
   return X;
}

int Nfft4GPAmdAdditiveLayoutInfo(void* str, long long* out, int nout)
{
   PlanExt* E = additive_plan(str);
   if (!E || !out) return -1;
   const AdditivePlan& P = E->P;
   long long v[18] = {P.n, P.nw, P.B, P.nblocks, P.dl.ntiles, P.dl.ntiles * kWave * kR, kR, P.CG, P.ngroups,
                      (long long)P.dl.bytes, pick_spread_variant(P), grid_atomic(P), pick_interp_threads(P),
                      pick_interp_hl(P), pick_hl_slots(P), pick_interp2_threads(), pick_fused_grid(P), shard_split(P)};
   for (int i = 0; i < nout && i < 18; i++) out[i] = v[i];
   return 0;
}

int Nfft4GPAmdSetPrecision(void* str, int bits)
{
   PlanExt* E = additive_plan(str);
   if (!E || (bits != 32 && bits != 64)) {
      fprintf(stderr, "nfft4gp_amd: Nfft4GPAmdSetPrecision needs an additive handle and bits 32 or 64\n");
      return -1;
   }
   AdditivePlan& P = E->P;
   const int rec = bits == 32 ? 4 : 5;
   if (rec == P.rec) return 0;
   (void)hipStreamSynchronize(current_stream());
   P.rec = rec;
   if (!P.points_ready || P.md.on) return 0;
   const double* buffer = ((nfft4gp_kernel*)str)->_buffer;
   P.points_ready = false;
   if (plan_build_points(P, buffer)) return -1;
   return plan_setup(P, buffer, P.kernel, P.f, P.l, P.mu);
}

int Nfft4GPAmdSetDeterministic(void* str, int on)
{
   PlanExt* E = additive_plan(str);
   if (!E) return -1;
   (void)hipStreamSynchronize(current_stream());
   E->P.det = on != 0;
   return 0;
}

int Nfft4GPAmdTimingEnable(void* str, int enable)
{
   PlanExt* E = additive_plan(str);
   if (!E) return -1;
   E->P.timing = enable != 0;
   if (enable) {
      (void)hipStreamSynchronize(current_stream());
      for (auto& r : E->pending) E->pool.push_back(r);
      E->pending.clear();
      for (int i = 0; i < 3; i++) {
         E->P.ms[i] = 0;
         E->P.cnt[i] = 0;
      }
   }
   return 0;
}

int Nfft4GPAmdTimingQuery(void* str, double* ms, long long* cnt)
{
   PlanExt* E = additive_plan(str);
   if (!E) return -1;
   AdditivePlan& P = E->P;
   for (auto& r : E->pending) {
      NFFT4GP_HIP_CHECK(hipEventSynchronize(r.ev[5]));
      for (int i = 0; i < 3; i++) {
         if (i == 1 && !r.grid) continue;
         float t = 0.f;
         NFFT4GP_HIP_CHECK(hipEventElapsedTime(&t, r.ev[2 * i], r.ev[2 * i + 1]));
         P.ms[i] += t;
         P.cnt[i]++;
      }
      E->pool.push_back(r);
   }
   E->pending.clear();
   for (int i = 0; i < 3; i++) {
      if (ms) ms[i] = P.ms[i];
      if (cnt) cnt[i] = P.cnt[i];
   }
   return 0;
}

int Nfft4GPAmdKernelBench(void* str, int which, int grad, int reps, const double* x, double* y, double* ms_avg)
{
   PlanExt* E = additive_plan(str);
   if (!E || !E->P.points_ready || reps <= 0 || !ms_avg) return -1;
   AdditivePlan& P = E->P;
   if (!is_device_ptr(x) || !is_device_ptr(y)) {
      fprintf(stderr, "nfft4gp_amd: Nfft4GPAmdKernelBench needs device vectors\n");
      return -1;
   }
   hipStream_t s = current_stream();
   hipEvent_t e0, e1;
   NFFT4GP_HIP_CHECK(hipEventCreate(&e0));
   NFFT4GP_HIP_CHECK(hipEventCreate(&e1));
   for (int rep = -1; rep < reps; rep++) {
      if (rep == 0) NFFT4GP_HIP_CHECK(hipEventRecord(e0, s));
      int rc = 0;
      if (P.md.on)
         rc = which == 0 ? md_spread(P, x, P.md.d_grid, s)
              : which == 1 ? md_grid(P, P.md.d_grid, grad, s)
                           : md_interp(P, grad, 1.0, x, 0.0, y, s);
      else if (which == 0)
         rc = launch_spread(P, x, P.d_part, s);
      else if (which == 1)
         rc = launch_grid(P, P.d_part, P.nparts, grad, s);
      else
         rc = launch_interp(P, grad, 1.0, x, 0.0, y, s);
      if (rc) return -1;
   }
   NFFT4GP_HIP_CHECK(hipEventRecord(e1, s));
   NFFT4GP_HIP_CHECK(hipEventSynchronize(e1));
   float t = 0.f;
   NFFT4GP_HIP_CHECK(hipEventElapsedTime(&t, e0, e1));
   *ms_avg = (double)t / reps;
   (void)hipEventDestroy(e0);
   (void)hipEventDestroy(e1);
   return 0;
}


void* Nfft4GPAmdNysSetupAdditive(void* str, const int* perm, int k, int k11_mode)
{
   if (!device_ok()) {
      fprintf(stderr, "nfft4gp_amd: Nfft4GPAmdNysSetupAdditive: no HIP device visible (no CPU fallback).\n");
      return nullptr;
   }
   nfft4gp_kernel* kd = (nfft4gp_kernel*)str;
   PlanExt* E = additive_plan(str);
   if (!E || !E->P.points_ready || !perm) {
      fprintf(stderr, "nfft4gp_amd: Nfft4GPAmdNysSetupAdditive needs an additive handle after its kernel setup\n");
      return nullptr;
   }
   const AdditivePlan& P = E->P;
   if (P.row_begin != 0 || P.row_end != P.n_global) {
      fprintf(stderr, "nfft4gp_amd: Nfft4GPAmdNysSetupAdditive: row-sharded handles are not supported\n");
      return nullptr;
   }
   return nys_setup_additive(kd->_buffer, P.n_global, P.nw, P.dw, P.skip_last, P.kernel, kd->_params[0],
                             kd->_params[1], kd->_noise_level, perm, k, k11_mode);
}

}

namespace nfft4gp_amd {
NysDev* nys_setup_shard(void* str, const int* perm, int k, int k11_mode, Comm* comm)
{
   nfft4gp_kernel* kd = (nfft4gp_kernel*)str;
   PlanExt* E = additive_plan(str);
   if (!E || !E->P.points_ready || !perm || !comm) {
      fprintf(stderr, "nfft4gp_amd: the sharded Nystrom setup needs a row-shard handle after its kernel setup\n");
      return nullptr;
   }
   const AdditivePlan& P = E->P;
   NysShard sh;
   sh.comm = comm;
   sh.row_begin = P.row_begin;
   sh.n_global = P.n_global;
   return nys_setup_additive(kd->_buffer, P.n, P.nw, P.dw, P.skip_last, P.kernel, kd->_params[0], kd->_params[1],
                             kd->_noise_level, perm, k, k11_mode, false, &sh);
}
}

extern "C" {

int Nfft4GPAmdAdditiveComponentShard(void* str, int nw_global, int own_diag)
{
   PlanExt* E = additive_plan(str);
   if (!E || nw_global < E->P.nw || E->P.row_begin != 0 || E->P.row_end != E->P.n_global) {
      fprintf(stderr, "nfft4gp_amd: Nfft4GPAmdAdditiveComponentShard needs a whole-row additive handle and "
                      "nw_global >= its %d windows\n", E ? E->P.nw : 0);
      return -1;
   }
   E->P.weight = 1.0 / (double)nw_global;
   E->P.diag = own_diag ? 1.0 : 0.0;
   AdditivePlan& P = E->P;
   if (P.points_ready) return plan_setup(P, ((nfft4gp_kernel*)str)->_buffer, P.kernel, P.f, P.l, P.mu);
   return 0;
}

int Nfft4GPAmdShardSpread(void* str, const double* x_local, double* grid)
{
   PlanExt* E = additive_plan(str);
   if (!E || !E->P.points_ready) return -1;
   AdditivePlan& P = E->P;
   hipStream_t s = current_stream();
   if (P.md.on) return md_spread(P, x_local, grid, s);
   if (P.nblocks == 0) {
      NFFT4GP_HIP_CHECK(hipMemsetAsync(grid, 0, sizeof(double) * P.nw * kNos, s));
      return 0;
   }
   if (launch_spread(P, x_local, P.d_part, s)) return -1;
   return launch_reduce_parts(P, P.d_part, grid, s);
}

int Nfft4GPAmdShardFinish(void* str, const double* grid, int grad, double alpha, const double* x_local, double beta,
                          double* y_local)
{
   PlanExt* E = additive_plan(str);
   if (!E || !E->P.points_ready) return -1;
   AdditivePlan& P = E->P;
   hipStream_t s = current_stream();
   if (P.md.on) {
      if (md_grid(P, grid, grad, s)) return -1;
      return md_interp(P, grad, alpha, x_local, beta, y_local, s);
   }
   const int S = shard_split(P);
   if (!grad && S > 1 && !P.timing) return launch_shard_finish_split(P, grid, alpha, x_local, beta, y_local, S, s);
   if (launch_grid_from_sum(P, grid, grad, s)) return -1;
   return launch_interp(P, grad, alpha, x_local, beta, y_local, s);
}

long long Nfft4GPAmdDebugShardH(void* str, double* out, long long count)
{
   PlanExt* E = additive_plan(str);
   if (!E || !E->P.points_ready || E->P.md.on || !out || !E->P.d_H) return -1;
   const long long m = std::min(count, (long long)E->P.nw * kNos * kNC);
   if (hipStreamSynchronize(current_stream()) != hipSuccess ||
       hipMemcpy(out, E->P.d_H, sizeof(double) * (size_t)m, hipMemcpyDeviceToHost) != hipSuccess)
      return -1;
   return m;
}

long long Nfft4GPAmdShardGridSize(void* str)
{
   PlanExt* E = additive_plan(str);
   if (!E || !E->P.points_ready) return -1;
   const AdditivePlan& P = E->P;
   return P.md.on ? (long long)P.nw * P.md.G : (long long)P.nw * kNos;
}

int Nfft4GPAmdHostTapPoly(double* C)
{
   if (C) {
      const std::vector<double>& T = tap_poly_coeffs();
      memcpy(C, T.data(), sizeof(double) * T.size());
   }
   return kNC;
}

int Nfft4GPAmdHostCirculant(int kind, double c, double weight, double* bhat, double* w)
{
   double bh[kBand];
   bhat_1d(kind, c, bh);
   if (bhat) memcpy(bhat, bh, sizeof(bh));
   if (w) circulant_1d(bh, weight, w);
   return 0;
}

double Nfft4GPAmdHostPrepare(const double* col, int n, unsigned int* q)
{
   std::vector<double> xs;
   const double sc = centre_and_scale(col, n, 1, xs);
   if (sc < 0.0) return sc;
   for (int j = 0; j < n; j++) q[j] = quantize(xs[j]);
   return sc;
}

int Nfft4GPAmdHostLayout(const unsigned int* qc, int n, int nw, int B, int CG, long long* counts,
                         unsigned short* meta, unsigned int* lo, unsigned int* q, int* tile_off)
{
   return Nfft4GPAmdHostLayoutRec(qc, n, nw, B, CG, 5, counts, meta, lo, q, tile_off);
}

int Nfft4GPAmdHostLayoutRec(const unsigned int* qc, int n, int nw, int B, int CG, int rec, long long* counts,
                            unsigned short* meta, unsigned int* lo, unsigned int* q, int* tile_off)
{
   if (B <= 0 || B > kMaxBlock || CG <= 0 || n < 0 || nw <= 0 || nw > 1023 || (rec != 4 && rec != 5)) return -1;
   Layout L;
   build_layout(qc, n, nw, B, CG, L, rec);
   counts[0] = L.ntiles;
   counts[1] = L.ngroups;
   counts[2] = L.nblocks;
   if (meta) memcpy(meta, L.meta.data(), L.meta.size() * sizeof(uint16_t));
   if (lo && !L.lo.empty()) memcpy(lo, L.lo.data(), L.lo.size() * sizeof(uint32_t));
   if (q) memcpy(q, L.q.data(), L.q.size() * sizeof(uint32_t));
   if (tile_off) memcpy(tile_off, L.tile_off.data(), L.tile_off.size() * sizeof(int));
   return 0;
}

void* Nfft4GPNFFTKernelParamCreate(int max_n, int dim)
{
   nfft4gp_kernel* kd = kernel_struct_create(max_n);
   SingleAdj* adj = new SingleAdj();
   adj->owner = kd;
   adj->dim = dim;
   adj->max_n = max_n;
   kd->_external = adj;
   return kd;
}

int Nfft4GPNFFTKernelParamRemovePoints(void* kernel)
{
   nfft4gp_kernel* kd = (nfft4gp_kernel*)kernel;
   SingleAdj* adj = kd ? (SingleAdj*)kd->_external : nullptr;
   if (adj && adj->plan) {
      free_layout(adj->plan->P);
      adj->plan->P.points_ready = false;
   }
   return 0;
}

int Nfft4GPNFFTKernelParamFreeNFFTKernel(void* kernel) { return Nfft4GPNFFTKernelParamRemovePoints(kernel); }

void Nfft4GPNFFTKernelParamFree(void* kernel)
{
   nfft4gp_kernel* kd = (nfft4gp_kernel*)kernel;
   if (!kd) return;
   SingleAdj* adj = (SingleAdj*)kd->_external;
   if (adj) {
      free_plan(adj->plan);
      delete adj;
   }
// ... 88 lines not shown
```

preconditioned_additive_gaussian_processes_with_fourier_acceleration_amd/csrc/nfft_kernels.hip:

```cpp
#include <hip/hip_ext.h>
#include <hip/hip_runtime.h>

#include <algorithm>
#include <cmath>
#include <cstdio>
#include <vector>

#include "internal.h"
#include "reduce.hpp"

namespace nfft4gp_amd {

constexpr int kGridThreads = 1024;
constexpr int kMomStride = kNC + 1;
constexpr int kMomWin = kNC * kNos + 4;
template <int MOMT>
__host__ __device__ constexpr int mom_doubles_per_window()
{
   return MOMT ? kMomWin : kNos * kMomStride;
}
template <int MOMT>
__device__ __forceinline__ int mom_index(int cl, int cell, int d)
{
   return MOMT ? cl * kMomWin + d * kNos + cell : (cl * kNos + cell) * kMomStride + d;
}

__device__ __forceinline__ double q_to_s(uint32_t q) { return (double)(int)q; }

__constant__ double c_taps[kTaps * kNC];
__constant__ double c_taps_u[kTaps * kNC];
typedef float f32x2 __attribute__((ext_vector_type(2)));

constexpr int kMaxStampWG = 16384;
__device__ unsigned long long g_stamps[kMaxStampWG * 4];

__device__ __forceinline__ void stamp(int slot)
{
   if (threadIdx.x == 0 && blockIdx.x < kMaxStampWG)
      g_stamps[blockIdx.x * 4 + slot] = __builtin_amdgcn_s_memrealtime();
}

struct TileRegs {
   uint32_t mt;
   uint32_t lo[kR / 4];
   uint32_t qq[kR];
};

template <int REC = 5>
__device__ __forceinline__ void load_tile(TileRegs& T, const uint16_t* __restrict__ meta,
                                          const uint32_t* __restrict__ lo, const uint32_t* __restrict__ qarr,
                                          int t, int lane)
{
   T.mt = meta[(size_t)t * 64 + lane];
   const uint4* l4 = reinterpret_cast<const uint4*>(lo) + (size_t)t * (kR / 16) * 64 + lane;
   const uint4* q4 = reinterpret_cast<const uint4*>(qarr) + (size_t)t * (kR / 4) * 64 + lane;
#pragma unroll
   for (int k = 0; k < (REC == 5 ? kR / 16 : 0); k++) {
      const uint4 v = l4[k * 64];
      T.lo[4 * k + 0] = v.x;
      T.lo[4 * k + 1] = v.y;
      T.lo[4 * k + 2] = v.z;
      T.lo[4 * k + 3] = v.w;
   }
#pragma unroll
   for (int k = 0; k < kR / 4; k++) {
      const uint4 v = q4[k * 64];
      T.qq[4 * k + 0] = v.x;
      T.qq[4 * k + 1] = v.y;
      T.qq[4 * k + 2] = v.z;
      T.qq[4 * k + 3] = v.w;
   }
}

template <int REC = 5>
__device__ __forceinline__ uint32_t slot_off(const TileRegs& T, int r)
{
   if (REC == 4) return (T.qq[r] << 3) & 0x7FF8u;
   const uint32_t hi = ((T.lo[r >> 2] >> (8 * (r & 3))) & 255u) << 7;
   uint32_t off;
   asm("v_and_or_b32 %0, %1, %2, %3" : "=v"(off) : "v"(T.qq[r] << 3), "s"(0x78u), "v"(hi));
   return off;
}

template <class V>
__device__ __forceinline__ V* at_off(V* base, uint32_t byte_off)
{
   return reinterpret_cast<V*>(reinterpret_cast<char*>(base) + byte_off);
}

typedef __attribute__((address_space(3))) double lds_f64;
__device__ __forceinline__ lds_f64* lds_at(uint32_t byte_off) { return (lds_f64*)(size_t)byte_off; }
__device__ __forceinline__ void lds_add(uint32_t byte_off, double v)
{
   (void)__hip_atomic_fetch_add(lds_at(byte_off), v, __ATOMIC_RELAXED, __HIP_MEMORY_SCOPE_WORKGROUP);
}

template <int THREADS>
__device__ __forceinline__ void stage_block_glds(double* __restrict__ s, const double* __restrict__ x, int base,
                                                 int nloc, int B)
{
   const int tid = threadIdx.x, lane = tid & 63, wave = tid >> 6;
   const double* src = x + base;
   const int nfull = ((reinterpret_cast<uintptr_t>(src) & 15) == 0) ? nloc / 128 : 0;
   for (int p = wave; p < nfull; p += THREADS / 64)
      __builtin_amdgcn_global_load_lds((const __attribute__((address_space(1))) void*)(src + 128 * p + 2 * lane),
                                       (__attribute__((address_space(3))) void*)(s + 128 * p), 16, 0, 0);
   for (int e = 128 * nfull + tid; e < B + kPad; e += THREADS) s[e] = e < nloc ? src[e] : 0.0;
}

__device__ __forceinline__ double det_grid(uint32_t bexp)
{
   return __hiloint2double((int)((bexp << 20) | 0x80000u), 0);
}
__device__ __forceinline__ double det_round(double v, double C) { return (v + C) - C; }

template <int THREADS>
__device__ __forceinline__ void det_max_publish(const double* s_alpha, int nloc, uint32_t* s_red)
{
   constexpr int nwaves = THREADS / 64;
   const int wave = threadIdx.x >> 6, lane = threadIdx.x & 63;
   const int per = (nloc + nwaves - 1) / nwaves;
   const uint32_t* hw = reinterpret_cast<const uint32_t*>(s_alpha);
   uint32_t m = 0;
   for (int e = wave * per + lane; e < min(nloc, (wave + 1) * per); e += 64) m = max(m, hw[2 * e + 1] & 0x7FFFFFFFu);
   for (int off = 32; off > 0; off >>= 1) m = max(m, (uint32_t)__shfl_xor((int)m, off, 64));
   if (lane == 0) {
      s_red[wave] = m;
      __hip_atomic_fetch_add(s_red + nwaves, 1u, __ATOMIC_RELEASE, __HIP_MEMORY_SCOPE_WORKGROUP);
   }
}
template <int THREADS>
__device__ __forceinline__ uint32_t det_max_wait(uint32_t* s_red)
{
   constexpr int nwaves = THREADS / 64;
   while (__hip_atomic_load(s_red + nwaves, __ATOMIC_ACQUIRE, __HIP_MEMORY_SCOPE_WORKGROUP) < (uint32_t)nwaves)
      __builtin_amdgcn_s_sleep(1);
   uint32_t m = 0;
#pragma unroll
   for (int w = 0; w < nwaves; w++) m = max(m, s_red[w]);
   return (uint32_t)__builtin_amdgcn_readfirstlane((int)m) >> 20;
}

__device__ __forceinline__ uint32_t det_interp_exp(const double* __restrict__ hb, int nw)
{
   double Y = 0.0;
   for (int c = 0; c < nw; c++) Y += hb[c];
   const uint32_t bY = ((uint32_t)__double2hiint(Y) >> 20) & 0x7FFu;
   return min(bY + 2u, 2046u);
}

template <int REC>
__device__ __forceinline__ int tile_at(TileRegs& cur, const uint16_t* __restrict__ meta,
                                       const uint32_t* __restrict__ lo, const uint32_t* __restrict__ qarr, int t, int t1)
{
   if (t < t1) load_tile<REC>(cur, meta, lo, qarr, t, threadIdx.x & 63);
   return t;
}

__device__ __forceinline__ void gather_h(double (&h)[kNC], const double* __restrict__ H, uint32_t mt)
{
   const double2* src = reinterpret_cast<const double2*>(H + (size_t)mt * kNC);
#pragma unroll
   for (int d = 0; d < kNC; d += 2) {
      const double2 v = src[d / 2];
      h[d] = v.x;
      h[d + 1] = v.y;
   }
}
__device__ __forceinline__ void gather_h_lds(double (&h)[kNC], const double* row, int stride)
{
#pragma unroll
   for (int d = 0; d < kNC; d++) h[d] = row[d * stride];
}

template <int REC, bool DET>
__device__ __forceinline__ void interp_run(const TileRegs& cur, const double (&h)[kNC], double C)
{
#pragma unroll
   for (int r = 0; r < kR; r++) {
      const uint32_t off = slot_off<REC>(cur, r);
      const double u = q_to_s(cur.qq[r]);
      double v = h[kNC - 1];
#pragma unroll
      for (int d = kNC - 2; d >= 0; d--) v = fma(v, u, h[d]);
      lds_add(off, DET ? det_round(v, C) : v);
   }
}

constexpr int kEpMax = 8;

template <int THREADS>
__device__ __forceinline__ void ep_prefetch(double (&xe)[kEpMax], double (&ye)[kEpMax], const double* __restrict__ x,
                                            const double* __restrict__ y, int base, int nloc, double beta)
{
   static_assert(kMaxBlock <= kEpMax * THREADS, "a block's epilogue values fit the threads' registers");
#pragma unroll
   for (int k = 0; k < kEpMax; k++) {
      const int j = threadIdx.x + k * THREADS;
      xe[k] = (j < nloc) ? x[(size_t)base + j] : 0.0;
      ye[k] = (beta != 0.0 && j < nloc) ? y[(size_t)base + j] : 0.0;
   }
}

template <int THREADS, bool DOT>
__device__ __forceinline__ double ep_plain(const double (&xe)[kEpMax], const double (&ye)[kEpMax], const double* s_y,
                                           double* __restrict__ y, int base, int nloc, double alpha, double beta,
                                           double f, double mu)
{
   const double ff = f * f;
   double dacc = 0.0;
#pragma unroll
   for (int k = 0; k < kEpMax; k++) {
      const int j = threadIdx.x + k * THREADS;
      if (j >= nloc) break;
      const double v = ff * (s_y[j] + mu * xe[k]);
      const double yo = (beta == 0.0) ? alpha * v : fma(beta, ye[k], alpha * v);
      y[(size_t)base + j] = yo;
      if (DOT) dacc = fma(yo, xe[k], dacc);
   }
   return dacc;
}

template <int THREADS>
__device__ __forceinline__ void ep_dot_finish(double dacc, double* s_scr, double* __restrict__ dot_part,
                                              unsigned int* __restrict__ dot_ticket, double* __restrict__ dot_out)
{
   dacc = block_sum0_s<THREADS>(dacc, s_scr);
   double tot;
   if (grid_total_s<THREADS>(dacc, dot_part, dot_ticket, &tot, reinterpret_cast<int*>(s_scr + 2 * (THREADS / 64)),
                             s_scr + THREADS / 64) &&
       threadIdx.x == 0)
      *dot_out = tot;
}

constexpr bool kFoldMfmaOk = kNC == 8 && kTaps <= 12 && kNos == 64;
template <int REC>
__device__ __forceinline__ void fold_tap_operand(double (&a)[2], int lane)
{
   const int i = lane & 15, k = lane >> 4;
   const double* ct = REC == 4 ? c_taps_u : c_taps;
#pragma unroll
   for (int ks = 0; ks < 2; ks++) a[ks] = i < kTaps ? ct[i * kNC + 4 * ks + k] : 0.0;
}
__device__ __forceinline__ double fold_window_mfma(const double (&a)[2], double* mrow, double* grow89, int lane)
{
   typedef double f64x4 __attribute__((ext_vector_type(4)));
   const int i = lane & 15, k = lane >> 4;
   double bm[2][4];
#pragma unroll
   for (int ks = 0; ks < 2; ks++)
#pragma unroll
      for (int cb = 0; cb < 4; cb++) bm[ks][cb] = mrow[(4 * ks + k) * kNos + 16 * cb + i];
#pragma unroll
   for (int cb = 0; cb < 4; cb++) {
      f64x4 acc = {0.0, 0.0, 0.0, 0.0};
      acc = __builtin_amdgcn_mfma_f64_16x16x4f64(a[0], bm[0][cb], acc, 0, 0, 0);
      acc = __builtin_amdgcn_mfma_f64_16x16x4f64(a[1], bm[1][cb], acc, 0, 0, 0);
      mrow[k * kNos + 16 * cb + i] = acc[0];
      mrow[(4 + k) * kNos + 16 * cb + i] = acc[1];
      if (k < kTaps - 8) grow89[k * kNos + 16 * cb + i] = acc[2];
   }
   __builtin_amdgcn_fence(__ATOMIC_RELEASE, "wavefront");
   __builtin_amdgcn_wave_barrier();
   __builtin_amdgcn_fence(__ATOMIC_ACQUIRE, "wavefront");
   double v = 0.0;
#pragma unroll
   for (int tp = 0; tp < kTaps; tp++) {
      const int cell = (lane + kM - tp) & (kNos - 1);
      v += tp < 8 ? mrow[tp * kNos + cell] : grow89[(tp - 8) * kNos + cell];
   }
   return v;
}

constexpr int kFgCells = 33;
constexpr int kFgSpan = kFgCells + kTaps - 1;
constexpr int kFgSpan0 = (kNos - 16 - kM) & (kNos - 1);

template <int THREADS, bool TIMELINE = false, int MOMT = 1, bool DET = false, int REC = 5, bool PIPE = false>
__global__ __launch_bounds__(THREADS, 6) void k_spread(const uint16_t* __restrict__ meta,
                                                      const uint32_t* __restrict__ lo,
                                                      const uint32_t* __restrict__ qarr,
                                                      const int* __restrict__ tile_off, const int* __restrict__ cmax,
                                                      const double* __restrict__ x, int n, int B, int nblocks,
                                                      int ngroups, int CG, int nw, double* __restrict__ part,
                                                      double* __restrict__ gsum, int fold)
{
   extern __shared__ __attribute__((aligned(16))) double smem[];
   const int Bp = B + kPad;
   double* s_alpha = smem;
   double* s_mom = smem + Bp;
   uint32_t* s_red = reinterpret_cast<uint32_t*>(s_mom + CG * mom_doubles_per_window<MOMT>());

   const int xcd = blockIdx.x & 7;
   const int rest = blockIdx.x >> 3;
   const int g = rest % ngroups;
   const int b = (rest / ngroups) * 8 + xcd;
   if (b >= nblocks) return;
   if (TIMELINE) stamp(0);

   const int tid = threadIdx.x;
   const int lane = tid & 63;
   const int wave = tid >> 6;
   constexpr int nwaves = THREADS / 64;

   TileRegs cur, nxt;
   const int t1 = tile_off[b * ngroups + g + 1];
   int t = tile_off[b * ngroups + g] + wave;
   if (t < t1) load_tile<REC>(cur, meta, lo, qarr, t, lane);
   const int base = b * B;
   stage_block_glds<THREADS>(s_alpha, x, base, min(B, n - base), B);
   for (int i = tid; i < CG * mom_doubles_per_window<MOMT>(); i += THREADS) s_mom[i] = 0.0;
   if (DET && tid == 0) s_red[nwaves] = 0u;
   asm volatile("s_waitcnt vmcnt(0)" ::: "memory");
   __syncthreads();
   if (TIMELINE) stamp(1);
   double Cd[kNC];
   if (DET) {
      det_max_publish<THREADS>(s_alpha, min(B, n - base), s_red);
      const int cm = cmax[b * ngroups + g];
      const uint32_t lcm = max(cm > 1 ? 32u - (uint32_t)__clz(cm - 1) : 0u, 6u) + 1u;
      const uint32_t bC0 = det_max_wait<THREADS>(s_red) + lcm;
#pragma unroll
      for (int d = 0; d < kNC; d++) Cd[d] = det_grid(REC == 4 ? bC0 : bC0 + 31u * d);
   }

   const int c0 = g * CG;
   for (; t < t1; t += nwaves) {
      if (PIPE && t + nwaves < t1) load_tile<REC>(nxt, meta, lo, qarr, t + nwaves, lane);
      double acc[kNC];
      if constexpr (REC == 4) {
         static_assert(kNC == 8, "the packed moment chain is written for degree 7");
         f32x2 m01 = {0.f, 0.f}, m23 = {0.f, 0.f}, m45 = {0.f, 0.f}, m67 = {0.f, 0.f};
#pragma unroll
         for (int r = 0; r < kR; r++) {
            const float u = (float)(int)cur.qq[r] * 0x1p-32f;
            const float al = (float)*lds_at(slot_off<REC>(cur, r));
            const float u2 = u * u;
            f32x2 p = {al, al * u};
            m01 += p;
            p *= u2;
            m23 += p;
            p *= u2;
            m45 += p;
            p *= u2;
            m67 += p;
         }
         acc[0] = m01.x, acc[1] = m01.y, acc[2] = m23.x, acc[3] = m23.y;
         acc[4] = m45.x, acc[5] = m45.y, acc[6] = m67.x, acc[7] = m67.y;
      } else {
#pragma unroll
         for (int d = 0; d < kNC; d++) acc[d] = 0.0;
#pragma unroll
         for (int r = 0; r < kR; r++) {
            const double u = q_to_s(cur.qq[r]);
            double tpow = *lds_at(slot_off<REC>(cur, r));
            acc[0] += tpow;
#pragma unroll
            for (int d = 1; d < kNC; d++) {
               tpow *= u;
               acc[d] += tpow;
            }
         }
      }
      const int comp_local = (int)(cur.mt >> 6) - c0;
      const int cell = (int)(cur.mt & 63u);
      double* dst = s_mom + mom_index<MOMT>(comp_local, cell, 0);
#pragma unroll
      for (int d = 0; d < kNC; d++) {
         const double a = DET ? det_round(acc[d], Cd[d]) : acc[d];
         atomicAdd(dst + mom_index<MOMT>(0, 0, d), a);
      }
      if (PIPE)
         cur = nxt;
      else if (t + nwaves < t1)
         load_tile<REC>(cur, meta, lo, qarr, t + nwaves, lane);
   }
   const int ncomp = min(CG, nw - c0);
   constexpr bool kMfold = MOMT == 1 && kFoldMfmaOk;
   const bool mfold = kMfold && fold && 128 * ncomp <= Bp;
   double tapa[2] = {0.0, 0.0};
   if (mfold && wave < ncomp) fold_tap_operand<REC>(tapa, lane);
   __syncthreads();
   if (TIMELINE) stamp(2);

   for (int cl = wave; kMfold && mfold && cl < ncomp; cl += nwaves) {
      const double v = fold_window_mfma(tapa, s_mom + mom_index<1>(cl, 0, 0), s_alpha + cl * 128, lane);
      if (gsum)
         atomicAdd(gsum + (size_t)(c0 + cl) * kNos + lane, v);
      else
         part[((size_t)(c0 + cl) * nblocks + b) * kNos + lane] = v;
   }
   for (int idx = tid; !mfold && idx < ncomp * kNos; idx += THREADS) {
      const int cl = idx / kNos;
      const int gi = idx % kNos;
      double v = 0.0;
#pragma unroll 1
      for (int tp = 0; tp < kTaps; tp++) {
         const double* mrow = s_mom + mom_index<MOMT>(cl, (gi + kM - tp) & (kNos - 1), 0);
#pragma unroll
         for (int d = 0; d < kNC; d++)
            v = fma((REC == 4 ? c_taps_u : c_taps)[tp * kNC + d], mrow[mom_index<MOMT>(0, 0, d)], v);
      }
      if (gsum)
         atomicAdd(gsum + (size_t)(c0 + cl) * kNos + gi, v);
      else
         part[((size_t)(c0 + cl) * nblocks + b) * kNos + gi] = v;
   }
   if (TIMELINE) {
      __syncthreads();
      stamp(3);
   }
}

extern "C" int Nfft4GPAmdDebugStamps(unsigned long long* out, int nwg)
{
   if (nwg > kMaxStampWG) nwg = kMaxStampWG;
   NFFT4GP_HIP_CHECK(hipDeviceSynchronize());
   NFFT4GP_HIP_CHECK(hipMemcpyFromSymbol(out, HIP_SYMBOL(g_stamps), sizeof(unsigned long long) * 4 * nwg));
   return nwg;
}

__device__ __forceinline__ void grid_tail_coeffs(double (&ct)[kTaps])
{
   const int tid = threadIdx.x;
   const int d = tid % kNC;
#pragma unroll
   for (int tp = 0; tp < kTaps; tp++) ct[tp] = tid < kNos * kNC ? c_taps[tp * kNC + d] : 0.0;
}

__device__ void grid_tail(int comp, const double* __restrict__ s_g, double wreg, const double (&ct)[kTaps],
                          double* __restrict__ H, double* s_w, double* s_h, double* __restrict__ hb = nullptr,
                          double* s_scr = nullptr)
{
   static_assert(kGridThreads >= kNos * kNC, "one H entry per thread");
   const int tid = threadIdx.x;
   if (tid < kNos) s_w[tid] = wreg;
   __syncthreads();
   {
      const int o = tid >> 4, st = tid & 15;
      double h = 0.0;
      if (o < kNos) {
#pragma unroll
         for (int k = 0; k < 4; k++) {
            const int l2 = st * 4 + k;
            h = fma(s_w[(o - l2) & (kNos - 1)], s_g[l2], h);
         }
      }
      for (int off = 8; off > 0; off >>= 1) h += __shfl_xor(h, off, 64);
      if (o < kNos && st == 0) s_h[o] = h;
   }
   __syncthreads();
   if (tid < kNos * kNC) {
      const int cell = tid / kNC;
      const int d = tid % kNC;
      double v = 0.0;
#pragma unroll
      for (int tp = 0; tp < kTaps; tp++) v = fma(s_h[(cell - kM + tp) & (kNos - 1)], ct[tp], v);
      H[((size_t)comp * kNos + cell) * kNC + d] = v;
      if (hb) s_scr[tid] = ldexp(fabs(v), 31 * d);
   }
   if (hb) {
      __syncthreads();
      if (tid < kNos) {
         double m = 0.0;
#pragma unroll
         for (int d = 0; d < kNC; d++) m += s_scr[tid * kNC + d];
         for (int off = 32; off > 0; off >>= 1) m = fmax(m, __shfl_xor(m, off, 64));
         if (tid == 0) hb[comp] = m;
      }
   }
   __syncthreads();
}

__global__ __launch_bounds__(kGridThreads) void k_grid(const double* __restrict__ part, int nparts,
                                                      const double* __restrict__ w, const double* __restrict__ wd,
                                                      double* __restrict__ H, double* __restrict__ Hd, int grad,
                                                      int from_sum, long long part_rs = 0, long long h_rs = 0,
                                                      double* __restrict__ hb = nullptr, int clear_sum = 0)
{
   __shared__ double s_red[kGridThreads];
   __shared__ double s_g[kNos];
   __shared__ double s_h[kNos];
   __shared__ double s_w[kNos];
   const int comp = blockIdx.x;
   part += blockIdx.y * part_rs;
   H += blockIdx.y * h_rs;
   const int tid = threadIdx.x;
   const double wv = tid < kNos ? w[(size_t)comp * kNos + tid] : 0.0;
   const double wdv = (grad && tid < kNos) ? wd[(size_t)comp * kNos + tid] : 0.0;
   double ct[kTaps];
   grid_tail_coeffs(ct);
   if (from_sum) {
      if (tid < kNos) {
         s_g[tid] = part[(size_t)comp * kNos + tid];
         if (clear_sum) const_cast<double*>(part)[(size_t)comp * kNos + tid] = 0.0;
      }
   } else {
      constexpr int kPer = 16;
      const int cell = tid & 63;
      const int strand = tid >> 6;
      constexpr int nstr = kGridThreads / 64;
      const double* src = part + (size_t)comp * nparts * kNos + cell;
      double acc = 0.0;
      for (int p0 = strand; p0 < nparts; p0 += kPer * nstr) {
         double v[kPer];
#pragma unroll
         for (int k = 0; k < kPer; k++) {
            const int p = p0 + k * nstr;
            v[k] = p < nparts ? src[(size_t)p * kNos] : 0.0;
         }
#pragma unroll
         for (int k = 0; k < kPer; k++) acc += v[k];
      }
      s_red[tid] = acc;
      __syncthreads();
      if (tid < kNos) {
         double v = 0.0;
         for (int k = 0; k < nstr; k++) v += s_red[k * 64 + tid];
         s_g[tid] = v;
      }
   }
   __syncthreads();
   if (hb) hb += 2 * (size_t)gridDim.x * blockIdx.y;
   grid_tail(comp, s_g, wv, ct, H, s_w, s_h, hb, s_red);
   if (grad) grid_tail(comp, s_g, wdv, ct, Hd, s_w, s_h, hb ? hb + gridDim.x : nullptr, s_red);
}

constexpr int kPeerLanes = kGridThreads / 64;

__device__ __forceinline__ unsigned long long* peer_slot(char* buf, const PeerArgs& A)
{
   return (unsigned long long*)(buf + (A.epoch & 1u) * A.slot_doubles * 16);
}

__device__ __forceinline__ char* peer_buf(const PeerArgs& A, int r)
{
   char* b = A.inl[0];
#pragma unroll
   for (int k = 1; k < kPeerInline; k++)
      if (r == k) b = A.inl[k];
   return r < kPeerInline ? b : A.bufs[r];
}

__device__ __forceinline__ void peer_put(const PeerArgs& A, int comp, int cell, double v)
{
   unsigned long long* p = peer_slot(A.own, A) + 2 * ((size_t)comp * kNos + cell);
   const unsigned long long bits = (unsigned long long)__double_as_longlong(v);
   const unsigned long long e = (unsigned long long)A.epoch << 32;
   __hip_atomic_store(p, (bits & 0xffffffffull) | e, __ATOMIC_RELAXED, __HIP_MEMORY_SCOPE_SYSTEM);
   __hip_atomic_store(p + 1, (bits >> 32) | e, __ATOMIC_RELAXED, __HIP_MEMORY_SCOPE_SYSTEM);
}

__device__ __forceinline__ void peer_gather(const PeerArgs& A, int comp, double* s_g)
{
   __shared__ double s_v[kPeerLanes][kNos];
   const int tid = threadIdx.x, cell = tid & (kNos - 1), lr = tid / kNos;
   double v = 0.0;
   for (int r0 = 0; r0 < A.world; r0 += kPeerLanes) {
      const int r = r0 + lr;
      if (r < A.world) {
         const unsigned long long* p = peer_slot(peer_buf(A, r), A) + 2 * ((size_t)comp * kNos + cell);
         unsigned long long w0, w1;
         for (long long it = 0;; it++) {
            w0 = __hip_atomic_load(p, __ATOMIC_RELAXED, __HIP_MEMORY_SCOPE_SYSTEM);
            w1 = __hip_atomic_load(p + 1, __ATOMIC_RELAXED, __HIP_MEMORY_SCOPE_SYSTEM);
            if ((unsigned int)(w0 >> 32) == A.epoch && (unsigned int)(w1 >> 32) == A.epoch) break;
            if (it >= A.spin) {
               __hip_atomic_store(A.err, 1u, __ATOMIC_RELAXED, __HIP_MEMORY_SCOPE_SYSTEM);
               break;
            }
            __builtin_amdgcn_s_sleep(2);
         }
         s_v[lr][cell] = __longlong_as_double((long long)((w0 & 0xffffffffull) | (w1 << 32)));
      }
      __syncthreads();
      if (tid < kNos)
         for (int k = 0; k < kPeerLanes && r0 + k < A.world; k++) v = (r0 + k == 0) ? s_v[k][tid] : v + s_v[k][tid];
      __syncthreads();
   }
   if (tid < kNos) s_g[tid] = v;
}

__device__ __forceinline__ double parts_sum(const double* __restrict__ part, int nparts, int comp, double* s_red)
{
   const int tid = threadIdx.x;
   constexpr int kPer = 16;
   const int cell = tid & 63;
   const int strand = tid >> 6;
   constexpr int nstr = kGridThreads / 64;
   const double* src = part + (size_t)comp * nparts * kNos + cell;
   double acc = 0.0;
   for (int p0 = strand; p0 < nparts; p0 += kPer * nstr) {
      double v[kPer];
#pragma unroll
      for (int k = 0; k < kPer; k++) {
         const int p = p0 + k * nstr;
         v[k] = p < nparts ? src[(size_t)p * kNos] : 0.0;
      }
#pragma unroll
      for (int k = 0; k < kPer; k++) acc += v[k];
   }
   s_red[tid] = acc;
   __syncthreads();
   double v = 0.0;
   if (tid < kNos)
      for (int k = 0; k < nstr; k++) v += s_red[k * 64 + tid];
   return v;
}

__global__ __launch_bounds__(kGridThreads) void k_peer_sum(PeerArgs A, double* __restrict__ grid)
{
   __shared__ double s_g[kNos];
   peer_gather(A, blockIdx.x, s_g);
   if (threadIdx.x < kNos) grid[(size_t)blockIdx.x * kNos + threadIdx.x] = s_g[threadIdx.x];
}

__global__ __launch_bounds__(kGridThreads) void k_grid_sum_yinit(const double* __restrict__ gsum,
                                                                const double* __restrict__ w, double* __restrict__ H,
                                                                double* __restrict__ y, const double* __restrict__ x,
                                                                int n, double beta, double amu, PeerArgs A,
                                                                const double* __restrict__ part, int nparts)
{
   __shared__ double s_g[kNos];
   __shared__ double s_h[kNos];
   __shared__ double s_w[kNos];
   const int comp = blockIdx.x;
   const int tid = threadIdx.x;
   const double wv = tid < kNos ? w[(size_t)comp * kNos + tid] : 0.0;
   double ct[kTaps];
   grid_tail_coeffs(ct);
   if (!A.bufs && tid < kNos) s_g[tid] = gsum[(size_t)comp * kNos + tid];
   if (A.bufs && part) {
      __shared__ double s_red[kGridThreads];
      const double v = parts_sum(part, nparts, comp, s_red);
      if (tid < kNos) peer_put(A, comp, tid, v);
   }
   constexpr int kU = 4;
   const size_t stride = (size_t)gridDim.x * kGridThreads;
   for (size_t j0 = (size_t)blockIdx.x * kGridThreads + tid; j0 < (size_t)n; j0 += kU * stride) {
      double xv[kU], yv[kU];
#pragma unroll
      for (int u = 0; u < kU; u++) {
         const size_t j = j0 + u * stride;
         xv[u] = j < (size_t)n ? x[j] : 0.0;
         yv[u] = (beta != 0.0 && j < (size_t)n) ? y[j] : 0.0;
      }
#pragma unroll
      for (int u = 0; u < kU; u++) {
         const size_t j = j0 + u * stride;
         if (j < (size_t)n) y[j] = (beta == 0.0 ? 0.0 : beta * yv[u]) + amu * xv[u];
      }
   }
   if (A.bufs) peer_gather(A, comp, s_g);
   __syncthreads();
   grid_tail(comp, s_g, wv, ct, H, s_w, s_h);
}

template <int THREADS, int REC = 5>
__global__ __launch_bounds__(THREADS) void k_interp_part(const uint16_t* __restrict__ meta,
                                                        const uint32_t* __restrict__ lo,
                                                        const uint32_t* __restrict__ qarr,
                                                        const int* __restrict__ tile_off, const double* __restrict__ H,
                                                        double* __restrict__ y, int n, int B, int ngroups, int S,
                                                        double scale)
{
   extern __shared__ __attribute__((aligned(16))) double smem[];
   double* s_y = smem;
   const int b = blockIdx.x / S, part = blockIdx.x % S;
   const int g0 = part * ngroups / S, g1 = (part + 1) * ngroups / S;
   const int tid = threadIdx.x;
   const int base = b * B;
   const int nloc = min(B, n - base);
   TileRegs cur;
   const int t1 = tile_off[b * ngroups + g1];
   int t = tile_at<REC>(cur, meta, lo, qarr, tile_off[b * ngroups + g0] + (tid >> 6), t1);
   for (int i = tid; i < B + kPad; i += THREADS) s_y[i] = 0.0;
   __syncthreads();
   for (; t < t1; t = tile_at<REC>(cur, meta, lo, qarr, t + THREADS / 64, t1)) {
      double h[kNC];
      gather_h(h, H, cur.mt);
      interp_run<REC, false>(cur, h, 0.0);
   }
   __syncthreads();
   for (int j = tid; j < nloc; j += THREADS) atomicAdd(y + (size_t)base + j, scale * s_y[j]);
}

__global__ __launch_bounds__(kGridThreads) void k_reduce_parts(const double* __restrict__ part, int nparts, int nw,
                                                              double* __restrict__ gsum, PeerArgs A)
{
   __shared__ double s_red[kGridThreads];
   const int comp = blockIdx.x;
   const int tid = threadIdx.x;
   const double v = parts_sum(part, nparts, comp, s_red);
   if (tid < kNos) {
      if (A.bufs)
         peer_put(A, comp, tid, v);
      else
         gsum[(size_t)comp * kNos + tid] = v;
   }
}

template <bool GRAD, int THREADS, bool DOT = false, bool DET = false, int REC = 5>
__global__ __launch_bounds__(THREADS) void k_interp(
    const uint16_t* __restrict__ meta, const uint32_t* __restrict__ lo, const uint32_t* __restrict__ qarr,
    const int* __restrict__ tile_off, const double* __restrict__ H, const double* __restrict__ Hd,
    const double* __restrict__ x, double* __restrict__ y, int n, int B, int ngroups, double alpha, double beta,
    double f, double mu, double dg, double* __restrict__ dot_part, unsigned int* __restrict__ dot_ticket,
    double* __restrict__ dot_out, const double* __restrict__ hb, int nw)
// ... 112 lines not shown
   ep_prefetch<THREADS>(xe, ye, x, y, base, nloc, beta);
   for (int i = tid; i < Bp; i += THREADS) s_y[i] = 0.0;
   const double Cy = DET ? det_grid(det_interp_exp(hb, nw)) : 0.0;
   __syncthreads();

   for (; t < t1; t = tile_at<REC>(cur, meta, lo, qarr, t + THREADS / 64, t1)) {
      double h[kNC];
      gather_h(h, H, cur.mt);
      interp_run<REC, DET>(cur, h, Cy);
   }
   __syncthreads();

   const double dacc = ep_plain<THREADS, DOT>(xe, ye, s_y, y, base, nloc, alpha, beta, f, mu);
   if (DOT) ep_dot_finish<THREADS>(dacc, smem + Bp, dot_part, dot_ticket, dot_out);
}

constexpr int kHlWin = kNC * kNos + 1;
constexpr size_t kMaxDynamicLds = 160 * 1024;

__host__ __device__ constexpr size_t hl_lds_bytes(int B, int CG, int ngroups, int ns)
{
   return sizeof(double) * ((size_t)B + kPad) + sizeof(double) * (size_t)ns * CG * kHlWin +
          sizeof(int) * (1 + (size_t)ns + 2 * (size_t)ngroups);
}

__device__ __forceinline__ void hl_stage_wave(double* s_H, const double* __restrict__ H, int g, int slot, int CG, int nw,
                                              int lane)
{
   const int c0 = g * CG;
   const int ncomp = min(CG, nw - c0);
   const double2* src = reinterpret_cast<const double2*>(H + (size_t)c0 * kNos * kNC);
   double* dst = s_H + (size_t)slot * CG * kHlWin;
   const int pairs = ncomp * kNos * kNC / 2;
#pragma unroll 4
   for (int i = lane; i < pairs; i += 64) {
      const double2 v = src[i];
      const int e = 2 * i;
      const int cl = e / (kNos * kNC);
      const int cell = (e / kNC) & (kNos - 1);
      const int d = e & (kNC - 1);
      double* row = dst + cl * kHlWin + cell;
      row[d * kNos] = v.x;
      row[(d + 1) * kNos] = v.y;
   }
}

template <int THREADS, bool DET = false, int REC = 5>
__global__ __launch_bounds__(THREADS) void k_interp_hl(const uint16_t* __restrict__ meta, const uint32_t* __restrict__ lo,
                                                       const uint32_t* __restrict__ qarr, const int* __restrict__ tile_off,
                                                       const double* __restrict__ H, const double* __restrict__ x,
                                                       double* __restrict__ y, int n, int B, int ngroups, int CG, int nw,
                                                       double alpha, double beta, double f, double mu,
                                                       const double* __restrict__ hb, int ns)
{
   extern __shared__ __attribute__((aligned(16))) double smem[];
   const int Bp = B + kPad;
   double* s_y = smem;
   double* s_H = smem + Bp;
   int* s_ready = reinterpret_cast<int*>(s_H + (size_t)ns * CG * kHlWin);
   int* s_done = s_ready + ns;
   int* s_toff = s_done + ngroups;
   const int b = blockIdx.x;
   const int tid = threadIdx.x;
   const int base = b * B;
   const int nloc = min(B, n - base);
   const int lane = tid & 63;
   const int wave = tid >> 6;
   constexpr int nwaves = THREADS / 64;
   const int gbase = b * ngroups;
   TileRegs cur;
   const int t1 = tile_off[gbase + ngroups];
   int t = tile_at<REC>(cur, meta, lo, qarr, tile_off[gbase] + wave, t1);
   double xe[kEpMax], ye[kEpMax];
   ep_prefetch<THREADS>(xe, ye, x, y, base, nloc, beta);
   for (int i = tid; i < Bp; i += THREADS) s_y[i] = 0.0;
   for (int i = tid; i < ngroups; i += THREADS) s_done[i] = 0;
   for (int i = tid; i <= ngroups; i += THREADS) s_toff[i] = tile_off[gbase + i];
   if (tid < ns) s_ready[tid] = tid;
   if (wave < ns && wave < ngroups) hl_stage_wave(s_H, H, wave, wave, CG, nw, lane);
   const double Cy = DET ? det_grid(det_interp_exp(hb, nw)) : 0.0;
   __syncthreads();

   int g = 0, gslot = 0;
   int gend = s_toff[1];
   auto leave = [&](int gl) {
      int old = 0;
      if (lane == 0) old = __hip_atomic_fetch_add(s_done + gl, 1, __ATOMIC_ACQ_REL, __HIP_MEMORY_SCOPE_WORKGROUP);
      old = __builtin_amdgcn_readfirstlane(old);
      if (old == nwaves - 1 && gl + ns < ngroups) {
         const int sl = gl % ns;
         hl_stage_wave(s_H, H, gl + ns, sl, CG, nw, lane);
         __builtin_amdgcn_fence(__ATOMIC_RELEASE, "workgroup");
         if (lane == 0) __hip_atomic_store(s_ready + sl, gl + ns, __ATOMIC_RELEASE, __HIP_MEMORY_SCOPE_WORKGROUP);
      }
   };
   for (; t < t1; t = tile_at<REC>(cur, meta, lo, qarr, t + nwaves, t1)) {
      while (t >= gend) {
         leave(g);
         g++;
         gend = s_toff[g + 1];
         gslot = g % ns;
         if (g >= ns) {
            for (long spin = 0; spin < (1l << 24); spin++) {
               if (__hip_atomic_load(s_ready + gslot, __ATOMIC_ACQUIRE, __HIP_MEMORY_SCOPE_WORKGROUP) == g) break;
               __builtin_amdgcn_s_sleep(1);
            }
         }
      }
      const int cl = (int)(cur.mt >> 6) - g * CG;
      const int cell = (int)(cur.mt & 63u);
      double h[kNC];
      gather_h_lds(h, s_H + ((size_t)gslot * CG + cl) * kHlWin + cell, kNos);
      interp_run<REC, DET>(cur, h, Cy);
   }
   for (; g < ngroups; g++) leave(g);
   __syncthreads();

   ep_plain<THREADS, false>(xe, ye, s_y, y, base, nloc, alpha, beta, f, mu);
}

constexpr int kFgWin = kNC * kFgCells + 1;
constexpr int kFgRow = kNos + 1;
constexpr int kFgQuads = (kFgSpan + 3) / 4;
constexpr int kFgHs = 4 * kFgQuads + 1;
constexpr int kFgLdsWin = kFgWin + kFgHs + 2 * kFgRow;

template <int THREADS, bool DOT = false, int REC = 5>
__global__ __launch_bounds__(THREADS) void k_interp_fg(
    const uint16_t* __restrict__ meta, const uint32_t* __restrict__ lo, const uint32_t* __restrict__ qarr,
    const int* __restrict__ tile_off, const double* __restrict__ gsum, double* __restrict__ gclear,
    const double* __restrict__ wcirc, const double* __restrict__ x, double* __restrict__ y, int n, int B, int ngroups,
    double alpha, double beta, double f, double mu, double* __restrict__ dot_part,
    unsigned int* __restrict__ dot_ticket, double* __restrict__ dot_out, int nw)
{
   static_assert(THREADS % (4 * kNC) == 0 && kNC == 8, "a thread keeps its degree and cell quarter over the build");
   static_assert(kFgSpan % 6 == 0, "the circulant's steps go six per trip");
   extern __shared__ __attribute__((aligned(16))) double smem[];
   const int Bp = B + kPad;
   double* s_y = smem;
   double* s_H = smem + Bp;
   double* s_h = s_H + (size_t)nw * kFgWin;
   double* s_g = s_h + (size_t)nw * kFgHs;
   double* s_w = s_g + (size_t)nw * kFgRow;
   double* s_scr = s_w + (size_t)nw * kFgRow;
   const int b = blockIdx.x;
   const int tid = threadIdx.x;
   const int base = b * B;
   const int nloc = min(B, n - base);
   TileRegs cur;
   const int t1 = tile_off[(b + 1) * ngroups];
   int t = tile_at<REC>(cur, meta, lo, qarr, tile_off[b * ngroups] + (tid >> 6), t1);
   double ct[kTaps];
#pragma unroll
   for (int tp = 0; tp < kTaps; tp++) ct[tp] = c_taps[tp * kNC + (tid & (kNC - 1))];
   for (int i = tid; i < nw * kNos; i += THREADS) {
      const int o = (i >> 6) * kFgRow + (i & (kNos - 1));
      s_g[o] = gsum[i];
      s_w[o] = wcirc[i];
   }
   if (b == 0)
      for (int i = tid; i < nw * kNos; i += THREADS) gclear[i] = 0.0;
   for (int i = tid; i < Bp; i += THREADS) s_y[i] = 0.0;
   __syncthreads();
   for (int it = tid; it < nw * kFgQuads; it += THREADS) {
      const int w = it / kFgQuads, k0 = 4 * (it % kFgQuads);
      const double* gw = s_g + w * kFgRow;
      const double* ww = s_w + w * kFgRow;
      double r3 = ww[(k0 + 3) & (kNos - 1)], r2 = ww[(k0 + 2) & (kNos - 1)], r1 = ww[(k0 + 1) & (kNos - 1)], r0 = ww[k0];
      double a0 = 0.0, a1 = 0.0, a2 = 0.0, a3 = 0.0;
#pragma unroll 6
      for (int j = 0; j < kFgSpan; j++) {
         const double gj = gw[(kFgSpan0 + j) & (kNos - 1)];
         a0 = fma(r0, gj, a0);
         a1 = fma(r1, gj, a1);
         a2 = fma(r2, gj, a2);
         a3 = fma(r3, gj, a3);
         r3 = r2, r2 = r1, r1 = r0;
         r0 = ww[(k0 - j - 1) & (kNos - 1)];
      }
      double* hw = s_h + w * kFgHs + k0;
      hw[0] = a0, hw[1] = a1, hw[2] = a2, hw[3] = a3;
   }
   __syncthreads();
   {
      const int d = tid & (kNC - 1), seg = (tid >> 3) & 3;
      const int c0 = seg ? 8 * seg + 1 : 0, c1 = 8 * seg + 9;
      for (int w = tid >> 5; w < nw; w += THREADS / 32) {
         const double* hw = s_h + w * kFgHs + c0;
         double hv[kTaps + 8];
#pragma unroll
         for (int j = 0; j < kTaps + 8; j++) hv[j] = hw[j];
         double acc[9];
#pragma unroll
         for (int k = 0; k < 9; k++) acc[k] = 0.0;
#pragma unroll
         for (int tp = 0; tp < kTaps; tp++) {
#pragma unroll
            for (int k = 0; k < 9; k++) acc[k] = fma(hv[k + tp], ct[tp], acc[k]);
         }
         double* dst = s_H + (size_t)w * kFgWin + d * kFgCells + c0;
#pragma unroll
         for (int k = 0; k < 9; k++)
            if (c0 + k < c1) dst[k] = acc[k];
      }
   }
   __syncthreads();
   double xe[kEpMax], ye[kEpMax];
   ep_prefetch<THREADS>(xe, ye, x, y, base, nloc, beta);

   for (; t < t1; t = tile_at<REC>(cur, meta, lo, qarr, t + THREADS / 64, t1)) {
      const int ci = min((int)((cur.mt + 16u) & 63u), kFgCells - 1);
      double h[kNC];
      gather_h_lds(h, s_H + (size_t)(cur.mt >> 6) * kFgWin + ci, kFgCells);
      interp_run<REC, false>(cur, h, 0.0);
   }
   __syncthreads();

   const double dacc = ep_plain<THREADS, DOT>(xe, ye, s_y, y, base, nloc, alpha, beta, f, mu);
   if (DOT) ep_dot_finish<THREADS>(dacc, s_scr, dot_part, dot_ticket, dot_out);
}


template <int THREADS, bool DET = false, int REC = 5>
__global__ __launch_bounds__(THREADS) void k_interp2(const uint16_t* __restrict__ meta,
                                                     const uint32_t* __restrict__ lo,
                                                     const uint32_t* __restrict__ qarr,
                                                     const int* __restrict__ tile_off, const double* __restrict__ H,
                                                     size_t h_rs, const double* __restrict__ x0,
                                                     const double* __restrict__ x1, double* __restrict__ y0,
                                                     double* __restrict__ y1, int n, int B, int ngroups, double alpha,
                                                     double beta, double f, double mu, const double* __restrict__ hb,
                                                     int nw)
{
   extern __shared__ __attribute__((aligned(16))) double smem[];
   const int Bp = B + kPad;
   double* s_y0 = smem;
   double* s_y1 = smem + Bp;
   const int b = blockIdx.x;
   const int tid = threadIdx.x;
   const int base = b * B;
   const int nloc = min(B, n - base);
   const int lane = tid & 63;
   const int wave = tid >> 6;
   constexpr int nwaves = THREADS / 64;
   const int t0 = tile_off[b * ngroups];
   const int t1 = tile_off[(b + 1) * ngroups];
   TileRegs cur;
   int t = tile_at<REC>(cur, meta, lo, qarr, t0 + wave, t1);
   for (int i = tid; i < Bp; i += THREADS) s_y0[i] = s_y1[i] = 0.0;
   double C0 = 0.0, C1 = 0.0;
   if (DET) {
      C0 = det_grid(det_interp_exp(hb, nw));
      C1 = det_grid(det_interp_exp(hb + 2 * nw, nw));
   }
   __syncthreads();
   const double* H1 = H + h_rs;
   for (; t < t1; t += nwaves) {
      const size_t hoff = (size_t)cur.mt * kNC;
      double h0[kNC], h1[kNC];
#pragma unroll
      for (int d = 0; d < kNC; d += 2) {
         const double2 v0 = *reinterpret_cast<const double2*>(H + hoff + d);
         const double2 v1 = *reinterpret_cast<const double2*>(H1 + hoff + d);
         h0[d] = v0.x;
         h0[d + 1] = v0.y;
         h1[d] = v1.x;
         h1[d + 1] = v1.y;
      }
#pragma unroll
      for (int r = 0; r < kR; r++) {
         const uint32_t off = slot_off<REC>(cur, r);
         const double u = q_to_s(cur.qq[r]);
         double v0 = h0[kNC - 1], v1 = h1[kNC - 1];
#pragma unroll
         for (int d = kNC - 2; d >= 0; d--) {
            v0 = fma(v0, u, h0[d]);
            v1 = fma(v1, u, h1[d]);
         }
         lds_add(off, DET ? det_round(v0, C0) : v0);
         lds_add(off + 8u * (uint32_t)Bp, DET ? det_round(v1, C1) : v1);
      }
      if (t + nwaves < t1) load_tile<REC>(cur, meta, lo, qarr, t + nwaves, lane);
   }
   __syncthreads();
   const double ff = f * f;
   for (int j = tid; j < nloc; j += THREADS) {
      const size_t gj = (size_t)base + j;
      const double v0 = ff * (s_y0[j] + mu * x0[gj]);
      const double v1 = ff * (s_y1[j] + mu * x1[gj]);
      y0[gj] = (beta == 0.0) ? alpha * v0 : fma(beta, y0[gj], alpha * v0);
      y1[gj] = (beta == 0.0) ? alpha * v1 : fma(beta, y1[gj], alpha * v1);
   }
}

template <typename F, typename... A>
static void launch_ev(F fn, dim3 grid, dim3 block, size_t lds, hipStream_t s, const hipEvent_t* ev, A... args)
{
   if (ev)
      hipExtLaunchKernelGGL(fn, grid, block, (std::uint32_t)lds, s, ev[0], ev[1], 0u, args...);
   else
      hipLaunchKernelGGL(fn, grid, block, lds, s, args...);
}

static int spread_momt(const AdditivePlan& P) { return P.spread_variant == 2 ? 0 : 1; }

static size_t spread_lds_bytes(const AdditivePlan& P)
{
   const size_t per = spread_momt(P) ? mom_doubles_per_window<1>() : mom_doubles_per_window<0>();
   return sizeof(double) * ((size_t)P.B + kPad + (size_t)P.CG * per) + (P.det ? 64 : 0);
}

constexpr size_t kRedScratch = sizeof(double) * (2 * (1024 / 64) + 1);

static size_t interp_lds_bytes(const AdditivePlan& P, int grad)
{
   return sizeof(double) * ((size_t)P.B + kPad) * (grad ? 2 : 1) + kRedScratch;
}

int upload_tap_coeffs()
{
   static bool done[64] = {false};
   int dev = 0;
   NFFT4GP_HIP_CHECK(hipGetDevice(&dev));
   if (dev < 0 || dev >= 64) return -1;
   if (!done[dev]) {
      NFFT4GP_HIP_CHECK(hipMemcpyToSymbol(HIP_SYMBOL(c_taps_u), tap_poly_coeffs().data(), sizeof(double) * kTaps * kNC));
      std::vector<double> C = tap_poly_coeffs();
      for (int t = 0; t < kTaps; t++)
         for (int d = 0; d < kNC; d++) C[t * kNC + d] = std::ldexp(C[t * kNC + d], -32 * d);
      NFFT4GP_HIP_CHECK(hipMemcpyToSymbol(HIP_SYMBOL(c_taps), C.data(), sizeof(double) * kTaps * kNC));
      done[dev] = true;
   }
   return 0;
}

typedef void (*SpreadFn)(const uint16_t*, const uint32_t*, const uint32_t*, const int*, const int*, const double*, int,
                         int, int, int, int, int, double*, double*, int);
constexpr int kSpreadThreads = 512;
static const SpreadFn kSpreadFns[2][2][4] = {
    {{k_spread<kSpreadThreads>, k_spread<kSpreadThreads, true>, k_spread<kSpreadThreads, false, 0>,
      k_spread<kSpreadThreads, false, 1, false, 5, true>},
     {k_spread<kSpreadThreads, false, 1, true>, k_spread<kSpreadThreads, true, 1, true>,
      k_spread<kSpreadThreads, false, 0, true>, k_spread<kSpreadThreads, false, 1, true, 5, true>}},
    {{k_spread<kSpreadThreads, false, 1, false, 4>, k_spread<kSpreadThreads, true, 1, false, 4>,
      k_spread<kSpreadThreads, false, 0, false, 4>, k_spread<kSpreadThreads, false, 1, false, 4, true>},
     {k_spread<kSpreadThreads, false, 1, true, 4>, k_spread<kSpreadThreads, true, 1, true, 4>,
      k_spread<kSpreadThreads, false, 0, true, 4>, k_spread<kSpreadThreads, false, 1, true, 4, true>}}};
constexpr int kNumSpreadVariants = 4;
constexpr size_t kInfinityCacheBytes = 256ull << 20;
int pick_spread_variant(const AdditivePlan& P)
{
   int v = P.spread_variant;
   if (v < 0) v = P.dl.bytes > kInfinityCacheBytes ? 3 : 0;
   return std::min(v, kNumSpreadVariants - 1);
}
static SpreadFn spread_fn(const AdditivePlan& P)
{
   return kSpreadFns[P.rec == 4 ? 1 : 0][P.det ? 1 : 0][pick_spread_variant(P)];
}

constexpr int kInterpThreads = 1024;
typedef void (*InterpFn)(const uint16_t*, const uint32_t*, const uint32_t*, const int*, const double*,
                         const double*, const double*, double*, int, int, int, double, double, double, double,
                         double, double*, unsigned int*, double*, const double*, int);

template <int T, int REC>
static InterpFn interp_fn_t(bool grad, bool dot, bool det)
{
   if (grad) return det ? k_interp<true, T, false, true, REC> : k_interp<true, T, false, false, REC>;
   if (dot) return det ? k_interp<false, T, true, true, REC> : k_interp<false, T, true, false, REC>;
   return det ? k_interp<false, T, false, true, REC> : k_interp<false, T, false, false, REC>;
}
static InterpFn interp_fn(bool grad, bool dot, bool small, bool det, int rec)
{
   if (rec == 4) return small ? interp_fn_t<512, 4>(grad, dot, det) : interp_fn_t<kInterpThreads, 4>(grad, dot, det);
   return small ? interp_fn_t<512, 5>(grad, dot, det) : interp_fn_t<kInterpThreads, 5>(grad, dot, det);
}
constexpr int kInterp2Threads = 1024;
typedef void (*Interp2Fn)(const uint16_t*, const uint32_t*, const uint32_t*, const int*, const double*, size_t,
                          const double*, const double*, double*, double*, int, int, int, double, double, double, double,
                          const double*, int);
template <int REC>
static Interp2Fn interp2_fn_t(bool det, bool small)
{
   if (small) return det ? k_interp2<512, true, REC> : k_interp2<512, false, REC>;
   return det ? k_interp2<kInterp2Threads, true, REC> : k_interp2<kInterp2Threads, false, REC>;
}
static Interp2Fn interp2_fn(bool det, bool small, int rec)
{
   return rec == 4 ? interp2_fn_t<4>(det, small) : interp2_fn_t<5>(det, small);
}
typedef void (*InterpPartFn)(const uint16_t*, const uint32_t*, const uint32_t*, const int*, const double*, double*, int,
                             int, int, int, double);
static InterpPartFn interp_part_fn(int rec) { return rec == 4 ? k_interp_part<512, 4> : k_interp_part<512, 5>; }

typedef void (*InterpFgFn)(const uint16_t*, const uint32_t*, const uint32_t*, const int*, const double*, double*,
                           const double*, const double*, double*, int, int, int, double, double, double, double,
                           double*, unsigned int*, double*, int);
static InterpFgFn interp_fg_fn(bool dot, int rec)
{
   if (rec == 4) return dot ? k_interp_fg<kInterpThreads, true, 4> : k_interp_fg<kInterpThreads, false, 4>;
   return dot ? k_interp_fg<kInterpThreads, true, 5> : k_interp_fg<kInterpThreads, false, 5>;
}

typedef void (*InterpHlFn)(const uint16_t*, const uint32_t*, const uint32_t*, const int*, const double*, const double*,
                           double*, int, int, int, int, int, double, double, double, double, const double*, int);
static InterpHlFn interp_hl_fn(bool small, bool det, int rec)
{
   if (rec == 4)
      return small ? (det ? k_interp_hl<512, true, 4> : k_interp_hl<512, false, 4>)
                   : (det ? k_interp_hl<1024, true, 4> : k_interp_hl<1024, false, 4>);
   return small ? (det ? k_interp_hl<512, true, 5> : k_interp_hl<512, false, 5>)
                : (det ? k_interp_hl<1024, true, 5> : k_interp_hl<1024, false, 5>);
}
bool pick_interp_hl(const AdditivePlan& P)
{
   static const int v = getenv("NFFT4GP_AMD_INTERP_HL") ? atoi(getenv("NFFT4GP_AMD_INTERP_HL")) : -1;
   return (v < 0 ? P.dl.bytes > kInfinityCacheBytes : v != 0) && P.ngroups >= 1;
}
int pick_interp_threads(const AdditivePlan& P)
{
   static const int forced = getenv("NFFT4GP_AMD_INTERP_THREADS") ? atoi(getenv("NFFT4GP_AMD_INTERP_THREADS")) : 0;
   return forced == 512 || (forced != 1024 && P.nblocks >= 512) ? 512 : kInterpThreads;
}
int pick_hl_slots(const AdditivePlan& P)
{
   static const int slots_env = getenv("NFFT4GP_AMD_HL_SLOTS") ? atoi(getenv("NFFT4GP_AMD_HL_SLOTS")) : 0;
   int ns = std::max(2, std::min(slots_env > 0 ? slots_env : 2, pick_interp_threads(P) == 512 ? 2 : 6));
   while (ns > 2 && hl_lds_bytes(P.B, P.CG, P.ngroups, ns) > kMaxDynamicLds) ns--;
   return ns;
}
int pick_interp2_threads()
{
   static const int forced = getenv("NFFT4GP_AMD_INTERP2_THREADS") ? atoi(getenv("NFFT4GP_AMD_INTERP2_THREADS")) : 0;
   return forced == 512 ? 512 : kInterp2Threads;
}

static std::vector<const void*> interp_kernels()
{
   std::vector<const void*> v;
   for (int sm = 0; sm < 2; sm++)
      for (int det = 0; det < 2; det++)
         for (int rec = 4; rec <= 5; rec++) v.push_back((const void*)interp_hl_fn(sm, det, rec));
   for (int g = 0; g < 2; g++)
      for (int d = 0; d < 2; d++)
         for (int sm = 0; sm < 2; sm++)
            for (int det = 0; det < 2; det++)
               for (int rec = 4; rec <= 5; rec++) v.push_back((const void*)interp_fn(g, d && !g, sm, det, rec));
   for (int det = 0; det < 2; det++)
      for (int sm = 0; sm < 2; sm++)
         for (int rec = 4; rec <= 5; rec++) v.push_back((const void*)interp2_fn(det, sm, rec));
   for (int rec = 4; rec <= 5; rec++) v.push_back((const void*)interp_part_fn(rec));
   for (int d = 0; d < 2; d++)
      for (int rec = 4; rec <= 5; rec++) v.push_back((const void*)interp_fg_fn(d, rec));
   return v;
}
static std::vector<const void*> spread_kernels()
{
   std::vector<const void*> v;
   for (const auto& byrec : kSpreadFns)
      for (const auto& bydet : byrec)
         for (const SpreadFn f : bydet) v.push_back((const void*)f);
   return v;
}

static bool lds_ready()
{
   static const bool ok = [] {
      std::vector<const void*> v = interp_kernels();
      for (const void* f : spread_kernels()) v.push_back(f);
      for (const void* f : v)
         (void)hipFuncSetAttribute(f, hipFuncAttributeMaxDynamicSharedMemorySize, (int)kMaxDynamicLds);
      (void)hipGetLastError();
      hipFuncAttributes a;
      for (const void* f : v)
         if (hipFuncGetAttributes(&a, f) != hipSuccess || a.sharedSizeBytes != 0) return false;
      return true;
   }();
   if (!ok) fprintf(stderr, "nfft4gp_amd: a matvec kernel has static LDS; its absolute LDS addressing would be wrong\n");
   return ok;
}

static int launch_spread_to(const AdditivePlan& P, const double* d_x, double* d_part, double* d_gsum,
                            hipStream_t stream)
{
   if (P.dl.ntiles == 0 || P.n == 0) return 0;
   if (!lds_ready()) return -1;
   const SpreadFn fn = spread_fn(P);
   const int gridx = ((P.nblocks + 7) / 8) * 8 * P.ngroups;
   launch_ev(fn, dim3(gridx), dim3(kSpreadThreads), spread_lds_bytes(P), stream, P.kev ? P.kev + 0 : nullptr,
             P.dl.meta, P.dl.lo, P.dl.q, P.dl.tile_off, (const int*)P.dl.cmax, d_x, P.n, P.B, P.nblocks, P.ngroups,
             P.CG, P.nw, d_part, d_gsum, P.spread_fold);
   NFFT4GP_HIP_CHECK(hipGetLastError());
   return 0;
}

int launch_spread(const AdditivePlan& P, const double* d_x, double* d_part, hipStream_t stream)
{
   return launch_spread_to(P, d_x, d_part, nullptr, stream);
}

constexpr int kAtomicGridMaxBlocks = 512;
bool grid_atomic(const AdditivePlan& P)
{
   static const int v = getenv("NFFT4GP_AMD_GRID_ATOMIC") ? atoi(getenv("NFFT4GP_AMD_GRID_ATOMIC")) : -1;
   if (P.det || v == 0) return false;
   return v > 0 || P.nblocks <= kAtomicGridMaxBlocks;
}

static int launch_k_grid(const AdditivePlan& P, const double* src, int nparts, int from_sum, int grad, int clear_sum,
                         hipStream_t stream, double* H2 = nullptr, size_t part_rs = 0, size_t h_rs = 0)
{
   launch_ev(k_grid, dim3(P.nw, H2 ? 2 : 1), dim3(kGridThreads), 0, stream, P.kev && !H2 ? P.kev + 2 : nullptr, src,
             nparts, (const double*)P.d_w, (const double*)P.d_wd, H2 ? H2 : P.d_H, P.d_Hd, grad, from_sum,
             (long long)part_rs, (long long)h_rs, P.det ? P.d_hb : (double*)nullptr, clear_sum);
   NFFT4GP_HIP_CHECK(hipGetLastError());
   return 0;
}

int launch_spread_grid(AdditivePlan& P, const double* d_x, int grad, hipStream_t stream)
{
   if (!grid_atomic(P) || P.nblocks == 0) {
      if (launch_spread(P, d_x, P.d_part, stream)) return -1;
      return launch_grid(P, P.d_part, P.nparts, grad, stream);
   }
   if (!P.d_gsum) {
      NFFT4GP_HIP_CHECK(hipMalloc((void**)&P.d_gsum, sizeof(double) * (size_t)P.nw * kNos));
      NFFT4GP_HIP_CHECK(hipMemsetAsync(P.d_gsum, 0, sizeof(double) * (size_t)P.nw * kNos, stream));
   }
   if (launch_spread_to(P, d_x, nullptr, P.d_gsum, stream)) return -1;
   return launch_k_grid(P, P.d_gsum, 1, 1, grad, 1, stream);
}

int launch_grid(const AdditivePlan& P, const double* d_part, int nparts, int grad, hipStream_t stream)
{
   return launch_k_grid(P, d_part, nparts, 0, grad, 0, stream);
}

int launch_grid_from_sum(const AdditivePlan& P, const double* d_gridsum, int grad, hipStream_t stream)
{
   return launch_k_grid(P, d_gridsum, 1, 1, grad, 0, stream);
}

int launch_shard_finish_split(const AdditivePlan& P, const double* d_gridsum, double alpha, const double* d_x,
                              double beta, double* d_y, int S, hipStream_t stream, const PeerArgs* A,
                              const double* d_part)
{
   constexpr int T = 512;
   if (!lds_ready()) return -1;
   if (A && A->slot_doubles != (long long)P.nw * kNos) return -1;
   const double ff = P.f * P.f;
   hipLaunchKernelGGL(k_grid_sum_yinit, dim3(P.nw), dim3(kGridThreads), 0, stream, d_gridsum, (const double*)P.d_w,
                      P.d_H, d_y, d_x, P.n, beta, alpha * ff * P.mu * P.diag, A ? *A : PeerArgs{},
                      A ? (P.nblocks ? d_part : (const double*)P.d_w) : (const double*)nullptr,
                      P.nblocks ? P.nparts : 0);
   if (P.n > 0)
      hipLaunchKernelGGL(interp_part_fn(P.rec), dim3(P.nblocks * S), dim3(T), sizeof(double) * (size_t)(P.B + kPad), stream,
                         P.dl.meta, P.dl.lo, P.dl.q, P.dl.tile_off, (const double*)P.d_H, d_y, P.n, P.B, P.ngroups, S,
                         alpha * ff);
   NFFT4GP_HIP_CHECK(hipGetLastError());
   return 0;
}

int launch_peer_grid(const AdditivePlan& P, const PeerArgs& A, const double* d_part, hipStream_t stream)
{
   if (A.slot_doubles != (long long)P.nw * kNos) return -1;
   hipLaunchKernelGGL(k_grid_sum_yinit, dim3(P.nw), dim3(kGridThreads), 0, stream, (const double*)nullptr,
                      (const double*)P.d_w, P.d_H, (double*)nullptr, (const double*)nullptr, 0, 0.0, 0.0, A,
                      P.nblocks ? d_part : (const double*)P.d_w, P.nblocks ? P.nparts : 0);
   NFFT4GP_HIP_CHECK(hipGetLastError());
   return 0;
}

int launch_reduce_parts(const AdditivePlan& P, const double* d_part, double* d_gridsum, hipStream_t stream,
                        const PeerArgs* A)
{
   PeerArgs a = A ? *A : PeerArgs{};
   if (A && A->slot_doubles != (long long)P.nw * kNos) return -1;
   hipLaunchKernelGGL(k_reduce_parts, dim3(P.nw), dim3(kGridThreads), 0, stream, d_part, P.nblocks ? P.nparts : 0,
                      P.nw, d_gridsum, a);
   NFFT4GP_HIP_CHECK(hipGetLastError());
   return 0;
}

int launch_peer_sum(const AdditivePlan& P, const PeerArgs& A, double* d_grid, hipStream_t stream)
{
   if (A.slot_doubles != (long long)P.nw * kNos) return -1;
   hipLaunchKernelGGL(k_peer_sum, dim3(P.nw), dim3(kGridThreads), 0, stream, A, d_grid);
   NFFT4GP_HIP_CHECK(hipGetLastError());
   return 0;
}

int launch_interp(const AdditivePlan& P, int grad, double alpha, const double* d_x, double beta, double* d_y,
                  hipStream_t stream, double* d_dot)
{
   if (P.n == 0) return 0;
   if (!lds_ready()) return -1;
   if (d_dot && (grad || P.nblocks > kRedMaxBlocks)) {
      fprintf(stderr, "nfft4gp_amd: fused matvec-dot needs a plain matvec and <= %d blocks\n", kRedMaxBlocks);
      return -1;
   }
   const bool small = pick_interp_threads(P) == 512;
   if (!grad && !d_dot && pick_interp_hl(P)) {
      const int ns = pick_hl_slots(P);
      launch_ev(interp_hl_fn(small, P.det, P.rec), dim3(P.nblocks), dim3(small ? 512 : kInterpThreads),
                hl_lds_bytes(P.B, P.CG, P.ngroups, ns), stream, P.kev ? P.kev + 4 : nullptr, P.dl.meta, P.dl.lo,
                P.dl.q, P.dl.tile_off, (const double*)P.d_H, d_x, d_y, P.n, P.B, P.ngroups, P.CG, P.nw, alpha, beta,
                P.f, P.mu * P.diag, (const double*)P.d_hb, ns);
      NFFT4GP_HIP_CHECK(hipGetLastError());
      return 0;
   }
   const InterpFn fn = interp_fn(grad, d_dot != nullptr, small, P.det, P.rec);
   launch_ev(fn, dim3(P.nblocks), dim3(small ? 512 : kInterpThreads), interp_lds_bytes(P, grad), stream,
             P.kev ? P.kev + 4 : nullptr, P.dl.meta, P.dl.lo, P.dl.q, P.dl.tile_off, (const double*)P.d_H,
             (const double*)P.d_Hd, d_x, d_y, P.n, P.B, P.ngroups, alpha, beta, P.f, P.mu * P.diag, P.diag,
             P.d_dot_part, P.d_dot_ticket, d_dot, (const double*)P.d_hb, P.nw);
   NFFT4GP_HIP_CHECK(hipGetLastError());
   return 0;
}

static size_t fg_lds_bytes(int B, int nw)
{
   return sizeof(double) * ((size_t)B + kPad) + sizeof(double) * (size_t)nw * kFgLdsWin + kRedScratch;
}
constexpr int kFusedMaxBlocks = 256;
bool pick_fused_grid(const AdditivePlan& P)
{
   if (P.fused_grid == 0 || !P.cells33 || P.md.on || P.det || P.nblocks == 0 || P.n == 0) return false;
   if (P.row_begin != 0 || P.row_end != P.n_global) return false;
   if (!grid_atomic(P) || pick_interp_threads(P) != kInterpThreads || pick_interp_hl(P)) return false;
   if (fg_lds_bytes(P.B, P.nw) > kMaxDynamicLds) return false;
   return P.fused_grid > 0 || P.nblocks <= kFusedMaxBlocks;
}

int launch_matvec_fused(AdditivePlan& P, double alpha, const double* d_x, double beta, double* d_y, hipStream_t stream,
                        double* d_dot)
{
   if (!lds_ready()) return -1;
   if (d_dot && P.nblocks > kRedMaxBlocks) return -1;
   const size_t ns = (size_t)P.nw * kNos;
   if (!P.d_hsum) {
      NFFT4GP_HIP_CHECK(hipMalloc((void**)&P.d_hsum, sizeof(double) * 2 * ns));
      NFFT4GP_HIP_CHECK(hipMemsetAsync(P.d_hsum, 0, sizeof(double) * 2 * ns, stream));
      P.hsum_par = 0;
   }
   double* S = P.d_hsum + (size_t)P.hsum_par * ns;
   double* Sother = P.d_hsum + (size_t)(1 - P.hsum_par) * ns;
   if (launch_spread_to(P, d_x, nullptr, S, stream)) return -1;
   launch_ev(interp_fg_fn(d_dot != nullptr, P.rec), dim3(P.nblocks), dim3(kInterpThreads), fg_lds_bytes(P.B, P.nw),
             stream, P.kev ? P.kev + 4 : nullptr, P.dl.meta, P.dl.lo, P.dl.q, P.dl.tile_off, (const double*)S, Sother,
             (const double*)P.d_w, d_x, d_y, P.n, P.B, P.ngroups, alpha, beta, P.f, P.mu * P.diag, P.d_dot_part,
             P.d_dot_ticket, d_dot, P.nw);
   NFFT4GP_HIP_CHECK(hipGetLastError());
   P.hsum_par ^= 1;
   return 0;
}

int launch_interp_blocks(const AdditivePlan& P, double alpha, const double* d_x, double beta, double* d_y, int b0,
                         int b1, hipStream_t stream)
{
   if (P.n == 0 || b1 <= b0) return 0;
   if (!lds_ready()) return -1;
   const size_t off = (size_t)b0 * P.B;
   hipLaunchKernelGGL(interp_fn(false, false, false, P.det, P.rec), dim3(b1 - b0), dim3(kInterpThreads),
                      interp_lds_bytes(P, 0), stream, P.dl.meta, P.dl.lo, P.dl.q, P.dl.tile_off + (size_t)b0 * P.ngroups,
                      (const double*)P.d_H, (const double*)P.d_Hd, d_x + off, d_y + off, P.n - (int)off, P.B, P.ngroups,
                      alpha, beta, P.f, P.mu * P.diag, P.diag, (double*)nullptr, (unsigned int*)nullptr,
                      (double*)nullptr, (const double*)P.d_hb, P.nw);
   NFFT4GP_HIP_CHECK(hipGetLastError());
   return 0;
}

int launch_matvec2(AdditivePlan& P, double alpha, const double* x0, const double* x1, double beta, double* y0,
                   double* y1, hipStream_t stream)
{
   if (P.n == 0) return 0;
   if (P.md.on) return -1;
   if (!lds_ready()) return -1;
   const size_t part_rs = (size_t)std::max(1, P.nparts) * P.nw * kNos;
   const size_t h_rs = (size_t)P.nw * kNos * kNC;
   if (!P.d_part2) NFFT4GP_HIP_CHECK(hipMalloc((void**)&P.d_part2, sizeof(double) * 2 * part_rs));
   if (!P.d_H2) NFFT4GP_HIP_CHECK(hipMalloc((void**)&P.d_H2, sizeof(double) * 2 * h_rs));
   if (launch_spread(P, x0, P.d_part2, stream) || launch_spread(P, x1, P.d_part2 + part_rs, stream)) return -1;
   if (launch_k_grid(P, P.d_part2, P.nparts, 0, 0, 0, stream, P.d_H2, part_rs, h_rs)) return -1;
   const size_t lds_i = sizeof(double) * 2 * ((size_t)P.B + kPad);
   const bool small = pick_interp2_threads() == 512;
   hipLaunchKernelGGL(interp2_fn(P.det, small, P.rec), dim3(P.nblocks), dim3(small ? 512 : kInterp2Threads), lds_i, stream,
                      P.dl.meta, P.dl.lo,
                      P.dl.q, P.dl.tile_off, (const double*)P.d_H2, h_rs, x0, x1, y0, y1, P.n, P.B, P.ngroups, alpha,
                      beta, P.f, P.mu * P.diag, (const double*)P.d_hb, P.nw);
   NFFT4GP_HIP_CHECK(hipGetLastError());
   return 0;
}

}
```

preconditioned_additive_gaussian_processes_with_fourier_acceleration_amd/nfft.py:

```python
from __future__ import annotations

import ctypes as C

import numpy as np

from . import _lib

GAUSSIAN = 0
MATERN12 = 1


def _ptr(a):
    if isinstance(a, np.ndarray):
        if not a.flags.c_contiguous or a.dtype != np.float64:
            raise ValueError("numpy vectors must be C-contiguous float64")
        return a.ctypes.data, False
    if not a.is_contiguous() or str(a.dtype) != "torch.float64":
        raise ValueError("torch vectors must be contiguous float64")
    return a.data_ptr(), a.is_cuda


def _numel(a) -> int:
    return int(a.size) if isinstance(a, np.ndarray) else int(a.numel())


def _check_len(name, a, need, exact=True):
    got = _numel(a)
    if (got != need) if exact else (got < need):
        raise ValueError(f"{name} has {got} entries; this call needs {'exactly' if exact else 'at least'} {need}")


def _empty_like(x, n):
    if isinstance(x, np.ndarray):
        return np.zeros(n)
    import torch
    return torch.zeros(n, dtype=torch.float64, device=x.device)


class NFFTAdditiveKernel:

    def __init__(self, data, windows, nwindows: int, dwindows: int, shard: tuple[int, int] | None = None):
        data = np.asfortranarray(np.asarray(data, dtype=np.float64))
        if data.ndim != 2:
            raise ValueError("data must be n x d")
        self.n_global, self.d = data.shape
        self._data = data
        self._win = np.ascontiguousarray(np.asarray(windows, dtype=np.int32).ravel())
        if self._win.size != nwindows * dwindows:
            raise ValueError("windows must hold nwindows*dwindows entries")
        self.nwindows, self.dwindows = nwindows, dwindows
        L = _lib.lib()
        if shard is None:
            self.row_begin, self.row_end = 0, self.n_global
            self.h = L.Nfft4GPNFFTAdditiveKernelParamCreate(self._data.ctypes.data, self.n_global, self.n_global,
                                                            self.d, self._win.ctypes.data, nwindows, dwindows)
        else:
            self.row_begin, self.row_end = shard
            self.h = L.Nfft4GPAmdAdditiveShardCreate(self._data.ctypes.data, self.n_global, self.n_global, self.d,
                                                     self._win.ctypes.data, nwindows, dwindows, self.row_begin,
                                                     self.row_end)
        if not self.h:
            raise RuntimeError("Nfft4GPNFFTAdditiveKernelParamCreate failed")
        self.n = self.row_end - self.row_begin
        self._st = _lib.NfftKernelStruct.from_address(self.h)
        self._kernel = None

    @property
    def f(self):
        return self._st._params[0]

    @f.setter
    def f(self, v):
        self._st._params[0] = float(v)

    @property
    def l(self):
        return self._st._params[1]

    @l.setter
    def l(self, v):
        self._st._params[1] = float(v)

    @property
    def mu(self):
        return self._st._noise_level

    @mu.setter
    def mu(self, v):
        self._st._noise_level = float(v)

    @property
    def iparams(self):
        return tuple(self._st._iparams[:3])

    def setup(self, kernel: int = GAUSSIAN, f=None, l=None, mu=None) -> int:
        if f is not None:
            self.f = f
        if l is not None:
            self.l = l
        if mu is not None:
            self.mu = mu
        L = _lib.lib()
        fn = L.Nfft4GPNFFTAdditiveKernelGaussianKernel if kernel == GAUSSIAN else \
            L.Nfft4GPNFFTAdditiveKernelMatern12Kernel
        K = C.c_void_p()
        dK = C.c_void_p()
        rc = fn(self.h, self._data.ctypes.data, self.n_global, self.n_global, self.d, None, 0, None, 0,
                C.byref(K), C.byref(dK))
        if rc == 0:
            self._kernel = kernel
        return rc

    def _apply(self, fn, x, alpha, beta, y, mult):
        if self.row_begin != 0 or self.row_end != self.n_global:
            raise ValueError("a row-shard handle has no whole matvec: use shard_spread / shard_finish")
        _check_len("x", x, self.n)
        if y is None:
            y = _empty_like(x, mult * self.n)
        _check_len("y", y, mult * self.n)
        xp, xd = _ptr(x)
        yp, yd = _ptr(y)
        rc = fn(self.h, self.n, float(alpha), xp, float(beta), yp)
        if rc != 0:
            raise RuntimeError(f"matvec failed with status {rc}")
        return y

    def matsymv(self, x, alpha=1.0, beta=0.0, y=None):
        return self._apply(_lib.lib().Nfft4GPAdditiveNFFTMatSymv, x, alpha, beta, y, 1)

    def gradmatsymv(self, x, alpha=1.0, beta=0.0, y=None):
        return self._apply(_lib.lib().Nfft4GPAdditiveNFFTGradMatSymv, x, alpha, beta, y, 3)

    def shard_spread(self, x_local, grid):
        _check_len("x_local", x_local, self.n)
        size = self.shard_grid_size()
        if size < 0:
            raise RuntimeError("run the kernel setup before shard_spread")
        _check_len("grid", grid, size, exact=False)
        xp, _ = _ptr(x_local)
        gp, _ = _ptr(grid)
        if _lib.lib().Nfft4GPAmdShardSpread(self.h, xp, gp) != 0:
            raise RuntimeError("shard spread failed")
        return grid

    def shard_grid_size(self) -> int:
        return int(_lib.lib().Nfft4GPAmdShardGridSize(self.h))

    def shard_finish(self, grid, x_local, alpha=1.0, beta=0.0, y_local=None, grad=False):
        _check_len("x_local", x_local, self.n)
        if y_local is None:
            y_local = _empty_like(x_local, (3 if grad else 1) * self.n)
        _check_len("y_local", y_local, (3 if grad else 1) * self.n)
        size = self.shard_grid_size()
        if size < 0:
            raise RuntimeError("run the kernel setup before shard_finish")
        _check_len("grid", grid, size, exact=False)
        gp, _ = _ptr(grid)
        xp, _ = _ptr(x_local)
        yp, _ = _ptr(y_local)
        if _lib.lib().Nfft4GPAmdShardFinish(self.h, gp, int(grad), float(alpha), xp, float(beta), yp) != 0:
            raise RuntimeError("shard finish failed")
        return y_local

    def layout_info(self) -> dict:
        out = (C.c_longlong * 18)()
        _lib.lib().Nfft4GPAmdAdditiveLayoutInfo(self.h, out, 18)
        keys = ["n", "nwindows", "block", "nblocks", "ntiles", "slots", "R", "comps_per_group", "ngroups",
                "layout_bytes", "spread_variant", "grid_atomic", "interp_threads", "interp_hl", "hl_slots",
                "interp2_threads", "fused_grid", "shard_split"]
        return dict(zip(keys, [int(v) for v in out]))

    def set_deterministic(self, on: bool = True):
        if _lib.lib().Nfft4GPAmdSetDeterministic(self.h, int(bool(on))) != 0:
            raise RuntimeError("Nfft4GPAmdSetDeterministic failed")

    def set_precision(self, bits: int):
        if _lib.lib().Nfft4GPAmdSetPrecision(self.h, int(bits)) != 0:
            raise RuntimeError("Nfft4GPAmdSetPrecision failed")

    def timing(self, enable: bool):
        _lib.lib().Nfft4GPAmdTimingEnable(self.h, int(enable))

    def timing_query(self):
        ms = (C.c_double * 3)()
        cnt = (C.c_longlong * 3)()
        _lib.lib().Nfft4GPAmdTimingQuery(self.h, ms, cnt)
        names = ["spread", "grid", "interp"]
        return {nm: (ms[i], int(cnt[i])) for i, nm in enumerate(names)}

    KERNELS = ("spread", "grid", "interp")

    def kernel_bench(self, kernel: str, x, y, reps: int = 50, grad: bool = False) -> float:
        px, dx = _ptr(x)
        py, dy = _ptr(y)
        if not (dx and dy):
            raise ValueError("kernel_bench needs device vectors")
        ms = C.c_double()
        rc = _lib.lib().Nfft4GPAmdKernelBench(self.h, self.KERNELS.index(kernel), int(grad), reps, px, py,
                                               C.byref(ms))
        if rc != 0:
            raise RuntimeError("Nfft4GPAmdKernelBench failed")
        return ms.value

    @property
    def matvec_fnptr(self) -> int:
        return _lib.fnptr("Nfft4GPAdditiveNFFTMatSymv")

    @property
    def gradmatvec_fnptr(self) -> int:
        return _lib.fnptr("Nfft4GPAdditiveNFFTGradMatSymv")

    def free(self):
        if getattr(self, "h", None):
            _lib.lib().Nfft4GPAdditiveNFFTKernelFree(self.h)
            self.h = None

    def __del__(self):
        try:
            self.free()
        except Exception:
            pass


class NFFTKernel:

    def __init__(self, max_n: int, dim: int):
        L = _lib.lib()
        self.h = L.Nfft4GPNFFTKernelParamCreate(max_n, dim)
        self._st = _lib.NfftKernelStruct.from_address(self.h)
        self.dim = dim
        self.adj = None
        self.n = None

    def setup(self, data, kernel=GAUSSIAN, f=1.0, l=1.0, mu=0.0) -> int:
        data = np.asfortranarray(np.asarray(data, dtype=np.float64))
        n = data.shape[0]
        self._data = data
        self._st._params[0] = f
        self._st._params[1] = l
        self._st._noise_level = mu
        L = _lib.lib()
        fn = L.Nfft4GPNFFTKernelGaussianKernel if kernel == GAUSSIAN else L.Nfft4GPNFFTKernelMatern12Kernel
        K = C.c_void_p()
        dK = C.c_void_p()
        rc = fn(self.h, data.ctypes.data, n, n, self.dim, None, 0, None, 0, C.byref(K), C.byref(dK))
        if rc == 0:
            self.adj = K.value
            self.n = n
        return rc

    def matsymv(self, x, alpha=1.0, beta=0.0, y=None):
        _check_len("x", x, self.n)
        if y is None:
            y = _empty_like(x, self.n)
        _check_len("y", y, self.n)
        rc = _lib.lib().Nfft4GPNFFTMatSymv(self.adj, self.n, float(alpha), _ptr(x)[0], float(beta), _ptr(y)[0])
        if rc:
            raise RuntimeError("Nfft4GPNFFTMatSymv failed")
        return y

    def gradmatsymv(self, x, alpha=1.0, beta=0.0, y=None):
        _check_len("x", x, self.n)
        if y is None:
            y = _empty_like(x, 3 * self.n)
        _check_len("y", y, 3 * self.n)
        rc = _lib.lib().Nfft4GPNFFTGradMatSymv(self.adj, self.n, float(alpha), _ptr(x)[0], float(beta),
                                               _ptr(y)[0])
        if rc:
            raise RuntimeError("Nfft4GPNFFTGradMatSymv failed")
        return y

    def free(self):
        if getattr(self, "h", None):
            _lib.lib().Nfft4GPNFFTKernelParamFree(self.h)
            self.h = None

    def __del__(self):
        try:
            self.free()
        except Exception:
            pass
```

Before: 14740 matvecs/s.

## Add compact 48-column spread moment table when points fit the 33-cell span

Adds a new moment-table type (MOMT 2) holding 48 columns per window instead of 64. It is used when all points fall within the 33-cell span and the layout fits in the Infinity Cache. The smaller table cuts spread LDS use, which should let more workgroups share a CU and skip out-of-span fold work and atomics. The layout emit kernel is also reworked to handle tiles in LDS-bounded passes, and the CG choice and spread-round accounting are refactored. The cost is more template instantiations and more span-masking logic, which could introduce correctness risk.

```diff
diff --git a/include/nfft4gp_amd.h b/include/nfft4gp_amd.h
--- a/include/nfft4gp_amd.h
+++ b/include/nfft4gp_amd.h
@@ -484,6 +484,7 @@
                            unsigned short *meta, unsigned int *lo, unsigned int *q, int *tile_off);
 int Nfft4GPAmdDeviceLayoutRec(const unsigned int *qc, int n, int nw, int B, int CG, int rec, long long *counts,
                               unsigned short *meta, unsigned int *lo, unsigned int *q, int *tile_off);
+int Nfft4GPAmdDebugPickCG(long long n, int nw, int B, int cells33, int rec);
 int Nfft4GPAmdHostSymEig(const NFFT4GP_DOUBLE *A, int n, NFFT4GP_DOUBLE *w, NFFT4GP_DOUBLE *V);
 int Nfft4GPAmdHostCholInverse(const NFFT4GP_DOUBLE *A, int k, NFFT4GP_DOUBLE shift, NFFT4GP_DOUBLE *G);
 int Nfft4GPAmdHostLuSolve(const NFFT4GP_DOUBLE *A, int n, NFFT4GP_DOUBLE *B, int nrhs);
diff --git a/preconditioned_additive_gaussian_processes_with_fourier_acceleration_amd/csrc/internal.h b/preconditioned_additive_gaussian_processes_with_fourier_acceleration_amd/csrc/internal.h
--- a/preconditioned_additive_gaussian_processes_with_fourier_acceleration_amd/csrc/internal.h
+++ b/preconditioned_additive_gaussian_processes_with_fourier_acceleration_amd/csrc/internal.h
@@ -166,6 +166,9 @@
    int B = kMaxBlock, CG = 3, ngroups = 0, nblocks = 0;
    int rec = 5;
    int spread_variant = -1;
+   int spread_table = 64;
+   bool table64_forced = false;
+   int spread_rounds = 0;
    int spread_fold = 1;
    bool det = false;
    double* d_hb = nullptr;
@@ -225,6 +228,9 @@
 int launch_matvec2(AdditivePlan& P, double alpha, const double* x0, const double* x1, double beta, double* y0,
                    double* y1, hipStream_t stream);
 int pick_spread_variant(const AdditivePlan& P);
+int spread_table_cols(const AdditivePlan& P);
+int spread_momt(const AdditivePlan& P);
+size_t spread_lds_bytes(int B, int CG, int momt, bool det);
 bool grid_atomic(const AdditivePlan& P);
 int pick_interp_threads(const AdditivePlan& P);
 bool pick_interp_hl(const AdditivePlan& P);
diff --git a/preconditioned_additive_gaussian_processes_with_fourier_acceleration_amd/csrc/layout_gpu.hip b/preconditioned_additive_gaussian_processes_with_fourier_acceleration_amd/csrc/layout_gpu.hip
--- a/preconditioned_additive_gaussian_processes_with_fourier_acceleration_amd/csrc/layout_gpu.hip
+++ b/preconditioned_additive_gaussian_processes_with_fourier_acceleration_amd/csrc/layout_gpu.hip
@@ -51,8 +51,10 @@
 
 struct EmitLds {
    size_t off, run, cbase, sorted, sloc, sfr, smeta, cnt, total;
-   __host__ __device__ EmitLds(int CG, int B, int Tmax)
+   __host__ __device__ EmitLds(int CG, int B, int Tmax, int Tp)
    {
+      const bool one = Tp >= Tmax;
+      if (one) Tp = Tmax;
       size_t p = 0;
       auto take = [&](size_t bytes) {
          const size_t at = p;
@@ -62,24 +64,24 @@
       off = take(sizeof(int) * CG * (kNos + 1));
       run = take(sizeof(int) * CG * kNos);
       cbase = take(sizeof(int) * (CG * kNos + 1));
-      const size_t sorted_bytes = sizeof(uint16_t) * CG * B, cnt_bytes = sizeof(int) * Tmax * (2 * 32 + 4 * 16);
-      sorted = take(sorted_bytes > cnt_bytes ? sorted_bytes : cnt_bytes);
-      cnt = sorted;
-      sloc = take(sizeof(uint16_t) * Tmax * kWave * kR);
-      sfr = take(sizeof(uint32_t) * Tmax * kWave * kR);
-      smeta = take(sizeof(uint16_t) * Tmax * kWave);
+      const size_t sorted_bytes = sizeof(uint16_t) * CG * B, cnt_bytes = sizeof(int) * Tp * (2 * 32 + 4 * 16);
+      sorted = take(one && cnt_bytes > sorted_bytes ? cnt_bytes : sorted_bytes);
+      cnt = one ? sorted : take(cnt_bytes);
+      sloc = take(sizeof(uint16_t) * Tp * kWave * kR);
+      sfr = take(sizeof(uint32_t) * Tp * kWave * kR);
+      smeta = take(sizeof(uint16_t) * Tp * kWave);
       total = p;
    }
 };
 
 template <int REC>
 __global__ __launch_bounds__(kLT) void k_lay_emit(const uint32_t* __restrict__ qc, int n, int nw, int B, int CG,
-                                                  int ngroups, int Tmax, const int* __restrict__ tile_off,
+                                                  int ngroups, int Tmax, int Tp, const int* __restrict__ tile_off,
                                                   uint16_t* __restrict__ meta, uint32_t* __restrict__ lo,
                                                   uint32_t* __restrict__ q)
 {
    extern __shared__ __attribute__((aligned(16))) unsigned char lds[];
-   const EmitLds E(CG, B, Tmax);
+   const EmitLds E(CG, B, Tmax, Tp);
    int* s_off = reinterpret_cast<int*>(lds + E.off);
    int* s_run = reinterpret_cast<int*>(lds + E.run);
    int* s_cbase = reinterpret_cast<int*>(lds + E.cbase);
@@ -149,80 +151,87 @@
       }
       s_cbase[ncomp * kNos] = acc;
    }
-   for (int i = tid; i < T * kWave * kR; i += kLT) {
-      s_loc[i] = (uint16_t)(B + ((i / kR) % kWave & 31));
-      s_fr[i] = 0u;
-   }
-   for (int i = tid; i < T * kWave; i += kLT) s_meta[i] = (uint16_t)(c0 << 6);
    __syncthreads();
    const int nchunks = s_cbase[ncomp * kNos];
-   for (int k = tid; k < nchunks; k += kLT) {
-      int lo_i = 0, hi_i = ncomp * kNos;
-      while (hi_i - lo_i > 1) {
-         const int mid = (lo_i + hi_i) >> 1;
-         if (s_cbase[mid] <= k) lo_i = mid;
-         else hi_i = mid;
-      }
-      const int ci = lo_i / kNos, cell = lo_i % kNos;
-      const int* off = s_off + ci * (kNos + 1);
-      const int s = off[cell] + (k - s_cbase[lo_i]) * kR;
-      const int tile = k % T, ln = k / T;
-      s_meta[tile * kWave + ln] = (uint16_t)(((c0 + ci) << 6) | cell);
-      const uint32_t* qq = qc + (size_t)(c0 + ci) * n + base;
-      const uint16_t* sorted = s_sorted + (size_t)ci * B;
-      for (int r = 0; r < kR; r++) {
-         const int sidx = s + r;
-         if (sidx < off[cell + 1]) {
-            const int loc = sorted[sidx];
-            s_loc[(tile * kWave + ln) * kR + r] = (uint16_t)loc;
-            s_fr[(tile * kWave + ln) * kR + r] = qq[loc] & 0x3FFFFFFu;
-         }
-      }
-   }
-   __syncthreads();
-   if (tid < T) {
-      uint16_t* L = s_loc + (size_t)tid * kWave * kR;
-      uint32_t* F = s_fr + (size_t)tid * kWave * kR;
-      int* c32 = s_cnt + tid * 128;
-      int* c16 = c32 + 64;
-      for (int r = 0; r < kR; r++) {
-         for (int i = 0; i < 128; i++) c32[i] = 0;
-         for (int ln = 0; ln < kWave; ln++) {
-            int best = r, best_cost = 1 << 30;
-            for (int k = r; k < kR; k++) {
-               const int v = L[ln * kR + k];
-               const int cost = 2 * c32[(ln >> 5) * 32 + (v & 31)] + c16[(ln >> 4) * 16 + (v & 15)];
-               if (cost < best_cost) {
-                  best_cost = cost;
-                  best = k;
-                  if (cost == 0) break;
+   for (int tp0 = 0; tp0 < T; tp0 += Tp) {
+      const int Tn = min(Tp, T - tp0);
+      for (int i = tid; i < Tn * kWave * kR; i += kLT) {
+         s_loc[i] = (uint16_t)(B + ((i / kR) % kWave & 31));
+         s_fr[i] = 0u;
+      }
+      for (int i = tid; i < Tn * kWave; i += kLT) s_meta[i] = (uint16_t)(c0 << 6);
+      __syncthreads();
+      for (int idx = tid; idx < Tn * kWave; idx += kLT) {
+         const int tl = idx % Tn, ln = idx / Tn;
+         const int k = ln * T + tp0 + tl;
+         if (k >= nchunks) continue;
+         int lo_i = 0, hi_i = ncomp * kNos;
+         while (hi_i - lo_i > 1) {
+            const int mid = (lo_i + hi_i) >> 1;
+            if (s_cbase[mid] <= k) lo_i = mid;
+            else hi_i = mid;
+         }
+         const int ci = lo_i / kNos, cell = lo_i % kNos;
+         const int* off = s_off + ci * (kNos + 1);
+         const int s = off[cell] + (k - s_cbase[lo_i]) * kR;
+         s_meta[tl * kWave + ln] = (uint16_t)(((c0 + ci) << 6) | cell);
+         const uint32_t* qq = qc + (size_t)(c0 + ci) * n + base;
+         const uint16_t* sorted = s_sorted + (size_t)ci * B;
+         for (int r = 0; r < kR; r++) {
+            const int sidx = s + r;
+            if (sidx < off[cell + 1]) {
+               const int loc = sorted[sidx];
+               s_loc[(tl * kWave + ln) * kR + r] = (uint16_t)loc;
+               s_fr[(tl * kWave + ln) * kR + r] = qq[loc] & 0x3FFFFFFu;
+            }
+         }
+      }
+      __syncthreads();
+      if (tid < Tn) {
+         uint16_t* L = s_loc + (size_t)tid * kWave * kR;
+         uint32_t* F = s_fr + (size_t)tid * kWave * kR;
+         int* c32 = s_cnt + tid * 128;
+         int* c16 = c32 + 64;
+         for (int r = 0; r < kR; r++) {
+            for (int i = 0; i < 128; i++) c32[i] = 0;
+            for (int ln = 0; ln < kWave; ln++) {
+               int best = r, best_cost = 1 << 30;
+               for (int k = r; k < kR; k++) {
+                  const int v = L[ln * kR + k];
+                  const int cost = 2 * c32[(ln >> 5) * 32 + (v & 31)] + c16[(ln >> 4) * 16 + (v & 15)];
+                  if (cost < best_cost) {
+                     best_cost = cost;
+                     best = k;
+                     if (cost == 0) break;
+                  }
                }
+               const uint16_t tl = L[ln * kR + r];
+               L[ln * kR + r] = L[ln * kR + best];
+               L[ln * kR + best] = tl;
+               const uint32_t tf = F[ln * kR + r];
+               F[ln * kR + r] = F[ln * kR + best];
+               F[ln * kR + best] = tf;
+               const int v = L[ln * kR + r];
+               c32[(ln >> 5) * 32 + (v & 31)]++;
+               c16[(ln >> 4) * 16 + (v & 15)]++;
             }
-            const uint16_t tl = L[ln * kR + r];
-            L[ln * kR + r] = L[ln * kR + best];
-            L[ln * kR + best] = tl;
-            const uint32_t tf = F[ln * kR + r];
-            F[ln * kR + r] = F[ln * kR + best];
-            F[ln * kR + best] = tf;
-            const int v = L[ln * kR + r];
-            c32[(ln >> 5) * 32 + (v & 31)]++;
-            c16[(ln >> 4) * 16 + (v & 15)]++;
-         }
-      }
-   }
-   __syncthreads();
-   for (int i = tid; i < T * kWave; i += kLT) meta[(size_t)(t0 + i / kWave) * kWave + i % kWave] = s_meta[i];
-   for (int i = tid; i < T * kWave * kR; i += kLT) {
-      const int tile = i / (kWave * kR), ln = (i / kR) % kWave, r = i % kR;
-      const uint32_t loc = s_loc[i];
-      q[quad_index(t0 + tile, r, ln, kR)] = REC == 5 ? slot_word(loc, s_fr[i]) : slot_word4(loc, s_fr[i]);
-   }
-   if (REC != 5) return;
-   for (int i = tid; i < T * kWave * (kR / 4); i += kLT) {
-      const int tile = i / (kWave * (kR / 4)), ln = (i / (kR / 4)) % kWave, r4 = i % (kR / 4);
-      const uint16_t* l4 = s_loc + ((size_t)tile * kWave + ln) * kR + 4 * r4;
-      lo[quad_index(t0 + tile, r4, ln, kR / 4)] =
-          lo_byte(l4[0]) | (lo_byte(l4[1]) << 8) | (lo_byte(l4[2]) << 16) | (lo_byte(l4[3]) << 24);
+         }
+      }
+      __syncthreads();
+      const int tg0 = t0 + tp0;
+      for (int i = tid; i < Tn * kWave; i += kLT) meta[(size_t)(tg0 + i / kWave) * kWave + i % kWave] = s_meta[i];
+      for (int i = tid; i < Tn * kWave * kR; i += kLT) {
+         const int tile = i / (kWave * kR), ln = (i / kR) % kWave, r = i % kR;
+         const uint32_t loc = s_loc[i];
+         q[quad_index(tg0 + tile, r, ln, kR)] = REC == 5 ? slot_word(loc, s_fr[i]) : slot_word4(loc, s_fr[i]);
+      }
+      for (int i = tid; REC == 5 && i < Tn * kWave * (kR / 4); i += kLT) {
+         const int tile = i / (kWave * (kR / 4)), ln = (i / (kR / 4)) % kWave, r4 = i % (kR / 4);
+         const uint16_t* l4 = s_loc + ((size_t)tile * kWave + ln) * kR + 4 * r4;
+         lo[quad_index(tg0 + tile, r4, ln, kR / 4)] =
+             lo_byte(l4[0]) | (lo_byte(l4[1]) << 8) | (lo_byte(l4[2]) << 16) | (lo_byte(l4[3]) << 24);
+      }
+      __syncthreads();
    }
 }
 
@@ -232,7 +241,8 @@
 {
    const int ngroups = (nw + CG - 1) / CG, nblocks = (n + B - 1) / B, nbg = ngroups * nblocks;
    const int Tmax_bound = (CG * (B / kR + kNos) + kWave - 1) / kWave + 1;
-   if (EmitLds(CG, B, (CG * ((B + kR - 1) / kR) + kWave - 1) / kWave).total > 160 * 1024) return -1;
+   constexpr size_t kEmitLdsMax = 160 * 1024;
+   if (EmitLds(CG, B, 2, 1).total > kEmitLdsMax) return -1;
    int* d_tiles = nullptr;
    int* d_cmax = nullptr;
    NFFT4GP_HIP_CHECK(hipMalloc((void**)&d_tiles, sizeof(int) * (nbg + 1)));
@@ -252,7 +262,12 @@
       Tmax = std::max(Tmax, tiles[i]);
    }
    toff[nbg] = (int)acc;
-   if (Tmax > Tmax_bound || EmitLds(CG, B, Tmax).total > 160 * 1024) {
+   int Tp = Tmax;
+   if (EmitLds(CG, B, Tmax, Tmax).total > kEmitLdsMax) {
+      Tp = 1;
+      while (Tp + 1 < Tmax && EmitLds(CG, B, Tmax, Tp + 1).total <= kEmitLdsMax) Tp++;
+   }
+   if (Tmax > Tmax_bound || EmitLds(CG, B, Tmax, Tp).total > kEmitLdsMax) {
       (void)hipFree(d_tiles);
       (void)hipFree(d_cmax);
       return -1;
@@ -267,7 +282,7 @@
    NFFT4GP_HIP_CHECK(hipMalloc((void**)&P.dl.meta, sizeof(uint16_t) * nt * kWave));
    if (rec == 5) NFFT4GP_HIP_CHECK(hipMalloc((void**)&P.dl.lo, sizeof(uint32_t) * nt * (kR / 4) * kWave));
    NFFT4GP_HIP_CHECK(hipMalloc((void**)&P.dl.q, sizeof(uint32_t) * nt * kR * kWave));
-   const size_t lds = EmitLds(CG, B, Tmax).total;
+   const size_t lds = EmitLds(CG, B, Tmax, Tp).total;
    static const bool attr = []() {
       (void)hipFuncSetAttribute((const void*)k_lay_emit<5>, hipFuncAttributeMaxDynamicSharedMemorySize, 160 * 1024);
       (void)hipFuncSetAttribute((const void*)k_lay_emit<4>, hipFuncAttributeMaxDynamicSharedMemorySize, 160 * 1024);
@@ -277,7 +292,7 @@
    (void)attr;
    if (nbg > 0)
       hipLaunchKernelGGL(rec == 5 ? k_lay_emit<5> : k_lay_emit<4>, dim3(nbg), dim3(kLT), lds, s, d_qc, n, nw, B, CG,
-                         ngroups, Tmax, P.dl.tile_off, P.dl.meta, P.dl.lo, P.dl.q);
+                         ngroups, Tmax, Tp, P.dl.tile_off, P.dl.meta, P.dl.lo, P.dl.q);
    NFFT4GP_HIP_CHECK(hipGetLastError());
    NFFT4GP_HIP_CHECK(hipStreamSynchronize(s));
    (void)hipFree(d_tiles);
diff --git a/preconditioned_additive_gaussian_processes_with_fourier_acceleration_amd/csrc/nfft_api.cpp b/preconditioned_additive_gaussian_processes_with_fourier_acceleration_amd/csrc/nfft_api.cpp
--- a/preconditioned_additive_gaussian_processes_with_fourier_acceleration_amd/csrc/nfft_api.cpp
+++ b/preconditioned_additive_gaussian_processes_with_fourier_acceleration_amd/csrc/nfft_api.cpp
@@ -210,6 +210,8 @@
    const long long v = std::llround(x * 4294967296.0);
    return (uint32_t)(unsigned long long)v;
 }
+
+int spread_plan_rounds(const AdditivePlan& P);
 
 int plan_build_points(AdditivePlan& P, const double* buffer)
 {
@@ -266,6 +268,7 @@
          return -1;
       }
    P.cells33 = outside33 == 0;
+   P.spread_table = P.cells33 && !P.table64_forced && P.spread_variant != 2 ? 48 : 64;
    const auto t1 = std::chrono::steady_clock::now();
    free_layout(P);
    hipStream_t s = current_stream();
@@ -294,6 +297,7 @@
       fprintf(stderr, "nfft4gp_amd: layout setup: centre/scale/quantize %.1f ms, coordinate upload %.1f ms, "
                       "layout (%s) %.1f ms\n", ms(t0, t1), ms(t1, t2), rc_dev ? "host" : "GPU", ms(t2, t3));
    }
+   P.spread_rounds = spread_plan_rounds(P);
    P.nparts = P.nblocks;
    NFFT4GP_HIP_CHECK(hipMalloc((void**)&P.d_part, sizeof(double) * (size_t)std::max(1, P.nparts) * P.nw * kNos));
 
@@ -497,26 +501,48 @@
    return 1024;
 }
 
+constexpr int kCusPerXcd = 32;
+constexpr int kSpreadWgPerCu = 3;
+constexpr size_t kCuLdsBytes = 160 * 1024;
+
+int spread_plan_rounds(const AdditivePlan& P)
+{
+   const int momt = spread_momt(P);
+   const size_t lds = (spread_lds_bytes(P.B, P.CG, momt, P.det) + 511) & ~(size_t)511;
+   const size_t wg_per_cu = std::min<size_t>(kSpreadWgPerCu, kCuLdsBytes / lds);
+   const long long wgs = (long long)((P.nblocks + 7) / 8) * P.ngroups;
+   const long long slots = (long long)kCusPerXcd * (long long)std::max<size_t>(1, wg_per_cu);
+   return (int)((wgs + slots - 1) / slots);
+}
+
+int pick_spread_cg(long long n, int nw, int B)
+{
+   nw = std::max(nw, 1);
+   B = std::max(B, 1);
+   const int nblocks = (int)std::max<long long>(1, (n + B - 1) / B);
+   int cg = 1;
+   auto pick = [&](int cgmax) {
+      const int ngroups = (nw + cgmax - 1) / cgmax;
+      cg = (nw + ngroups - 1) / ngroups;
+      return ngroups;
+   };
+   if ((long long)pick(4) * nblocks < 384) pick(3);
+   return cg;
+}
+
 void env_layout(AdditivePlan& P)
 {
    P.B = default_block(P.n);
-   {
-      const int nw = std::max(P.nw, 1), nblocks = std::max(1, (P.n + P.B - 1) / P.B);
-      auto pick = [&](int cgmax) {
-         const int ngroups = (nw + cgmax - 1) / cgmax;
-         P.CG = (nw + ngroups - 1) / ngroups;
-         return ngroups;
-      };
-      if ((long long)pick(4) * nblocks < 384) pick(3);
-   }
    if (const char* e = getenv("NFFT4GP_AMD_BLOCK")) {
       const int v = atoi(e);
       if (v >= 256) P.B = std::min(v, kMaxBlock) & ~15;
    }
+   P.CG = pick_spread_cg(P.n, P.nw, default_block(P.n));
    if (const char* e = getenv("NFFT4GP_AMD_CG")) {
       const int v = atoi(e);
       if (v >= 1 && v <= 64) P.CG = v;
    }
+   if (const char* e = getenv("NFFT4GP_AMD_SPREAD_TABLE")) P.table64_forced = atoi(e) == 64;
    if (const char* e = getenv("NFFT4GP_AMD_SPREAD_VARIANT")) P.spread_variant = atoi(e);
    if (const char* e = getenv("NFFT4GP_AMD_SPREAD_FOLD")) P.spread_fold = atoi(e) != 0;
    if (const char* e = getenv("NFFT4GP_AMD_DET")) P.det = atoi(e) != 0;
@@ -867,15 +893,23 @@
    return X;
 }
 
+int Nfft4GPAmdDebugPickCG(long long n, int nw, int B, int cells33, int rec)
+{
+   if (n < 0 || nw < 1 || B < 16 || B > kMaxBlock || (rec != 4 && rec != 5)) return -1;
+   (void)cells33;
+   return pick_spread_cg(n, nw, B);
+}
+
 int Nfft4GPAmdAdditiveLayoutInfo(void* str, long long* out, int nout)
 {
    PlanExt* E = additive_plan(str);
    if (!E || !out) return -1;
    const AdditivePlan& P = E->P;
-   long long v[18] = {P.n, P.nw, P.B, P.nblocks, P.dl.ntiles, P.dl.ntiles * kWave * kR, kR, P.CG, P.ngroups,
+   long long v[20] = {P.n, P.nw, P.B, P.nblocks, P.dl.ntiles, P.dl.ntiles * kWave * kR, kR, P.CG, P.ngroups,
                       (long long)P.dl.bytes, pick_spread_variant(P), grid_atomic(P), pick_interp_threads(P),
-                      pick_interp_hl(P), pick_hl_slots(P), pick_interp2_threads(), pick_fused_grid(P), shard_split(P)};
-   for (int i = 0; i < nout && i < 18; i++) out[i] = v[i];
+                      pick_interp_hl(P), pick_hl_slots(P), pick_interp2_threads(), pick_fused_grid(P), shard_split(P),
+                      spread_table_cols(P), P.spread_rounds};
+   for (int i = 0; i < nout && i < 20; i++) out[i] = v[i];
    return 0;
 }
 
diff --git a/preconditioned_additive_gaussian_processes_with_fourier_acceleration_amd/csrc/nfft_kernels.hip b/preconditioned_additive_gaussian_processes_with_fourier_acceleration_amd/csrc/nfft_kernels.hip
--- a/preconditioned_additive_gaussian_processes_with_fourier_acceleration_amd/csrc/nfft_kernels.hip
+++ b/preconditioned_additive_gaussian_processes_with_fourier_acceleration_amd/csrc/nfft_kernels.hip
@@ -14,15 +14,18 @@
 constexpr int kGridThreads = 1024;
 constexpr int kMomStride = kNC + 1;
 constexpr int kMomWin = kNC * kNos + 4;
+constexpr int kMomCols = 48;
+constexpr int kMomWin48 = kNC * kMomCols + 4;
 template <int MOMT>
 __host__ __device__ constexpr int mom_doubles_per_window()
 {
-   return MOMT ? kMomWin : kNos * kMomStride;
+   return MOMT == 2 ? kMomWin48 : MOMT == 1 ? kMomWin : kNos * kMomStride;
 }
 template <int MOMT>
 __device__ __forceinline__ int mom_index(int cl, int cell, int d)
 {
-   return MOMT ? cl * kMomWin + d * kNos + cell : (cl * kNos + cell) * kMomStride + d;
+   if (MOMT == 2) return cl * kMomWin48 + d * kMomCols + ((cell + 16) & (kNos - 1));
+   return MOMT == 1 ? cl * kMomWin + d * kNos + cell : (cl * kNos + cell) * kMomStride + d;
 }
 
 __device__ __forceinline__ double q_to_s(uint32_t q) { return (double)(int)q; }
@@ -242,23 +245,26 @@
 #pragma unroll
    for (int ks = 0; ks < 2; ks++) a[ks] = i < kTaps ? ct[i * kNC + 4 * ks + k] : 0.0;
 }
+template <int NS = kNos>
 __device__ __forceinline__ double fold_window_mfma(const double (&a)[2], double* mrow, double* grow89, int lane)
 {
+   static_assert(NS == kNos || NS == kMomCols, "64 columns, or the 48 compact ones");
    typedef double f64x4 __attribute__((ext_vector_type(4)));
+   constexpr int NCB = NS / 16;
    const int i = lane & 15, k = lane >> 4;
-   double bm[2][4];
+   double bm[2][NCB];
 #pragma unroll
    for (int ks = 0; ks < 2; ks++)
 #pragma unroll
-      for (int cb = 0; cb < 4; cb++) bm[ks][cb] = mrow[(4 * ks + k) * kNos + 16 * cb + i];
-#pragma unroll
-   for (int cb = 0; cb < 4; cb++) {
+      for (int cb = 0; cb < NCB; cb++) bm[ks][cb] = mrow[(4 * ks + k) * NS + 16 * cb + i];
+#pragma unroll
+   for (int cb = 0; cb < NCB; cb++) {
       f64x4 acc = {0.0, 0.0, 0.0, 0.0};
       acc = __builtin_amdgcn_mfma_f64_16x16x4f64(a[0], bm[0][cb], acc, 0, 0, 0);
       acc = __builtin_amdgcn_mfma_f64_16x16x4f64(a[1], bm[1][cb], acc, 0, 0, 0);
-      mrow[k * kNos + 16 * cb + i] = acc[0];
-      mrow[(4 + k) * kNos + 16 * cb + i] = acc[1];
-      if (k < kTaps - 8) grow89[k * kNos + 16 * cb + i] = acc[2];
+      mrow[k * NS + 16 * cb + i] = acc[0];
+      mrow[(4 + k) * NS + 16 * cb + i] = acc[1];
+      if (k < kTaps - 8) grow89[k * NS + 16 * cb + i] = acc[2];
    }
    __builtin_amdgcn_fence(__ATOMIC_RELEASE, "wavefront");
    __builtin_amdgcn_wave_barrier();
@@ -266,8 +272,15 @@
    double v = 0.0;
 #pragma unroll
    for (int tp = 0; tp < kTaps; tp++) {
-      const int cell = (lane + kM - tp) & (kNos - 1);
-      v += tp < 8 ? mrow[tp * kNos + cell] : grow89[(tp - 8) * kNos + cell];
+      if constexpr (NS == kNos) {
+         const int cell = (lane + kM - tp) & (kNos - 1);
+         v += tp < 8 ? mrow[tp * kNos + cell] : grow89[(tp - 8) * kNos + cell];
+      } else {
+         const int ci = (lane + kM - tp + 16) & (kNos - 1);
+         const int col = min(ci, NS - 1);
+         const double gv = tp < 8 ? mrow[tp * NS + col] : grow89[(tp - 8) * NS + col];
+         v += ci < NS ? gv : 0.0;
+      }
    }
    return v;
 }
@@ -368,7 +381,7 @@
 #pragma unroll
       for (int d = 0; d < kNC; d++) {
          const double a = DET ? det_round(acc[d], Cd[d]) : acc[d];
-         atomicAdd(dst + mom_index<MOMT>(0, 0, d), a);
+         atomicAdd(dst + (MOMT == 2 ? d * kMomCols : mom_index<MOMT>(0, 0, d)), a);
       }
       if (PIPE)
          cur = nxt;
@@ -376,19 +389,28 @@
          load_tile<REC>(cur, meta, lo, qarr, t + nwaves, lane);
    }
    const int ncomp = min(CG, nw - c0);
-   constexpr bool kMfold = MOMT == 1 && kFoldMfmaOk;
+   constexpr bool kMfold = MOMT >= 1 && kFoldMfmaOk;
    const bool mfold = kMfold && fold && 128 * ncomp <= Bp;
    double tapa[2] = {0.0, 0.0};
    if (mfold && wave < ncomp) fold_tap_operand<REC>(tapa, lane);
    __syncthreads();
    if (TIMELINE) stamp(2);
 
+   auto in_span = [](int gi) { return ((gi - kFgSpan0) & (kNos - 1)) < kFgSpan; };
    for (int cl = wave; kMfold && mfold && cl < ncomp; cl += nwaves) {
-      const double v = fold_window_mfma(tapa, s_mom + mom_index<1>(cl, 0, 0), s_alpha + cl * 128, lane);
-      if (gsum)
-         atomicAdd(gsum + (size_t)(c0 + cl) * kNos + lane, v);
-      else
-         part[((size_t)(c0 + cl) * nblocks + b) * kNos + lane] = v;
+      if constexpr (MOMT == 2) {
+         const double v = fold_window_mfma<kMomCols>(tapa, s_mom + cl * kMomWin48, s_alpha + cl * 128, lane);
+         if (gsum) {
+            if (in_span(lane)) atomicAdd(gsum + (size_t)(c0 + cl) * kNos + lane, v);
+         } else
+            part[((size_t)(c0 + cl) * nblocks + b) * kNos + lane] = v;
+      } else {
+         const double v = fold_window_mfma(tapa, s_mom + mom_index<1>(cl, 0, 0), s_alpha + cl * 128, lane);
+         if (gsum)
+            atomicAdd(gsum + (size_t)(c0 + cl) * kNos + lane, v);
+         else
+            part[((size_t)(c0 + cl) * nblocks + b) * kNos + lane] = v;
+      }
    }
    for (int idx = tid; !mfold && idx < ncomp * kNos; idx += THREADS) {
       const int cl = idx / kNos;
@@ -396,14 +418,22 @@
       double v = 0.0;
 #pragma unroll 1
       for (int tp = 0; tp < kTaps; tp++) {
-         const double* mrow = s_mom + mom_index<MOMT>(cl, (gi + kM - tp) & (kNos - 1), 0);
-#pragma unroll
-         for (int d = 0; d < kNC; d++)
-            v = fma((REC == 4 ? c_taps_u : c_taps)[tp * kNC + d], mrow[mom_index<MOMT>(0, 0, d)], v);
-      }
-      if (gsum)
-         atomicAdd(gsum + (size_t)(c0 + cl) * kNos + gi, v);
-      else
+         if constexpr (MOMT == 2) {
+            const int cell = (gi + kM - tp) & (kNos - 1);
+            if (((cell + 16) & (kNos - 1)) >= kMomCols) continue;
+            const double* mrow = s_mom + mom_index<2>(cl, cell, 0);
+#pragma unroll
+            for (int d = 0; d < kNC; d++) v = fma((REC == 4 ? c_taps_u : c_taps)[tp * kNC + d], mrow[d * kMomCols], v);
+         } else {
+            const double* mrow = s_mom + mom_index<MOMT>(cl, (gi + kM - tp) & (kNos - 1), 0);
+#pragma unroll
+            for (int d = 0; d < kNC; d++)
+               v = fma((REC == 4 ? c_taps_u : c_taps)[tp * kNC + d], mrow[mom_index<MOMT>(0, 0, d)], v);
+         }
+      }
+      if (gsum) {
+         if (MOMT != 2 || in_span(gi)) atomicAdd(gsum + (size_t)(c0 + cl) * kNos + gi, v);
+      } else
          part[((size_t)(c0 + cl) * nblocks + b) * kNos + gi] = v;
    }
    if (TIMELINE) {
@@ -1122,13 +1152,19 @@
       hipLaunchKernelGGL(fn, grid, block, lds, s, args...);
 }
 
-static int spread_momt(const AdditivePlan& P) { return P.spread_variant == 2 ? 0 : 1; }
-
-static size_t spread_lds_bytes(const AdditivePlan& P)
-{
-   const size_t per = spread_momt(P) ? mom_doubles_per_window<1>() : mom_doubles_per_window<0>();
-   return sizeof(double) * ((size_t)P.B + kPad + (size_t)P.CG * per) + (P.det ? 64 : 0);
-}
+constexpr size_t kInfinityCacheBytes = 256ull << 20;
+int spread_table_cols(const AdditivePlan& P)
+{
+   return P.spread_variant != 2 && P.spread_table == 48 && P.dl.bytes <= kInfinityCacheBytes ? 48 : 64;
+}
+int spread_momt(const AdditivePlan& P) { return P.spread_variant == 2 ? 0 : spread_table_cols(P) == 48 ? 2 : 1; }
+
+size_t spread_lds_bytes(int B, int CG, int momt, bool det)
+{
+   const size_t per = momt == 2 ? mom_doubles_per_window<2>() : momt ? mom_doubles_per_window<1>() : mom_doubles_per_window<0>();
+   return sizeof(double) * ((size_t)B + kPad + (size_t)CG * per) + (det ? 64 : 0);
+}
+static size_t spread_lds_bytes(const AdditivePlan& P) { return spread_lds_bytes(P.B, P.CG, spread_momt(P), P.det); }
 
 constexpr size_t kRedScratch = sizeof(double) * (2 * (1024 / 64) + 1);
 
@@ -1157,17 +1193,19 @@
 typedef void (*SpreadFn)(const uint16_t*, const uint32_t*, const uint32_t*, const int*, const int*, const double*, int,
                          int, int, int, int, int, double*, double*, int);
 constexpr int kSpreadThreads = 512;
-static const SpreadFn kSpreadFns[2][2][4] = {
-    {{k_spread<kSpreadThreads>, k_spread<kSpreadThreads, true>, k_spread<kSpreadThreads, false, 0>,
-      k_spread<kSpreadThreads, false, 1, false, 5, true>},
-     {k_spread<kSpreadThreads, false, 1, true>, k_spread<kSpreadThreads, true, 1, true>,
-      k_spread<kSpreadThreads, false, 0, true>, k_spread<kSpreadThreads, false, 1, true, 5, true>}},
-    {{k_spread<kSpreadThreads, false, 1, false, 4>, k_spread<kSpreadThreads, true, 1, false, 4>,
-      k_spread<kSpreadThreads, false, 0, false, 4>, k_spread<kSpreadThreads, false, 1, false, 4, true>},
-     {k_spread<kSpreadThreads, false, 1, true, 4>, k_spread<kSpreadThreads, true, 1, true, 4>,
-      k_spread<kSpreadThreads, false, 0, true, 4>, k_spread<kSpreadThreads, false, 1, true, 4, true>}}};
+template <int MT, bool DET, int REC>
+struct SpreadVariants {
+   static constexpr SpreadFn fns[4] = {k_spread<kSpreadThreads, false, MT, DET, REC>,
+                                       k_spread<kSpreadThreads, true, MT, DET, REC>,
+                                       k_spread<kSpreadThreads, false, 0, DET, REC>,
+                                       k_spread<kSpreadThreads, false, MT, DET, REC, true>};
+};
+static const SpreadFn* const kSpreadFns[2][2][2] = {
+    {{SpreadVariants<1, false, 5>::fns, SpreadVariants<1, true, 5>::fns},
+     {SpreadVariants<1, false, 4>::fns, SpreadVariants<1, true, 4>::fns}},
+    {{SpreadVariants<2, false, 5>::fns, SpreadVariants<2, true, 5>::fns},
+     {SpreadVariants<2, false, 4>::fns, SpreadVariants<2, true, 4>::fns}}};
 constexpr int kNumSpreadVariants = 4;
-constexpr size_t kInfinityCacheBytes = 256ull << 20;
 int pick_spread_variant(const AdditivePlan& P)
 {
    int v = P.spread_variant;
@@ -1176,7 +1214,7 @@
 }
 static SpreadFn spread_fn(const AdditivePlan& P)
 {
-   return kSpreadFns[P.rec == 4 ? 1 : 0][P.det ? 1 : 0][pick_spread_variant(P)];
+   return kSpreadFns[spread_momt(P) == 2 ? 1 : 0][P.rec == 4 ? 1 : 0][P.det ? 1 : 0][pick_spread_variant(P)];
 }
 
 constexpr int kInterpThreads = 1024;
@@ -1278,9 +1316,10 @@
 static std::vector<const void*> spread_kernels()
 {
    std::vector<const void*> v;
-   for (const auto& byrec : kSpreadFns)
-      for (const auto& bydet : byrec)
-         for (const SpreadFn f : bydet) v.push_back((const void*)f);
+   for (const auto& bytable : kSpreadFns)
+      for (const auto& byrec : bytable)
+         for (const SpreadFn* bydet : byrec)
+            for (int i = 0; i < kNumSpreadVariants; i++) v.push_back((const void*)bydet[i]);
    return v;
 }
 
diff --git a/preconditioned_additive_gaussian_processes_with_fourier_acceleration_amd/nfft.py b/preconditioned_additive_gaussian_processes_with_fourier_acceleration_amd/nfft.py
--- a/preconditioned_additive_gaussian_processes_with_fourier_acceleration_amd/nfft.py
+++ b/preconditioned_additive_gaussian_processes_with_fourier_acceleration_amd/nfft.py
@@ -163,11 +163,11 @@
         return y_local
 
     def layout_info(self) -> dict:
-        out = (C.c_longlong * 18)()
-        _lib.lib().Nfft4GPAmdAdditiveLayoutInfo(self.h, out, 18)
+        out = (C.c_longlong * 20)()
+        _lib.lib().Nfft4GPAmdAdditiveLayoutInfo(self.h, out, 20)
         keys = ["n", "nwindows", "block", "nblocks", "ntiles", "slots", "R", "comps_per_group", "ngroups",
                 "layout_bytes", "spread_variant", "grid_atomic", "interp_threads", "interp_hl", "hl_slots",
-                "interp2_threads", "fused_grid", "shard_split"]
+                "interp2_threads", "fused_grid", "shard_split", "spread_table", "spread_rounds"]
         return dict(zip(keys, [int(v) for v in out]))
 
     def set_deterministic(self, on: bool = True):
```

After: 14750 matvecs/s, median of 3. Within noise of the previous version (+0.1%).
